# rosinality/vision-transformers-pytorch

Hardware: AMD Instinct MI355X
Metric: images/sec training (fwd+bwd+step) (higher is better)
Workload: dtype bf16; 1 GPU; swin_s 224x224 train step, batch 128/GPU, drop_path 0.3, MixLoss(eps 0.1), clip 5.0, AdamW(lr 1e-3, wd 0.05), grad_accum 1; global_batch=128, parallelism=dp1

## Files before the change

include/vtx.h:

```cpp
#ifndef VTX_H_
#define VTX_H_

#include <stddef.h>
#include <stdint.h>

#ifdef __cplusplus
extern "C" {
#endif

#define VTX_F32 0
#define VTX_BF16 1

#define VTX_OK 0
#define VTX_ERR_SHAPE (-1)
#define VTX_ERR_DTYPE (-2)
#define VTX_ERR_ALIGN (-3)
#define VTX_ERR_LAUNCH (-4)
#define VTX_ERR_WORKSPACE (-5)
#define VTX_ERR_NULL (-6)
#define VTX_ERR_JPEG (-7)

const char* vtx_strerror(int code);
#define VTX_ABI_VERSION 30
int vtx_abi_version(void);
int vtx_cu_count(void);
int vtx_debug_lds_poison(unsigned pattern, int rounds, void* stream);
int vtx_debug_mfma_peak(int iters, int waves_per_cu, void* sink, double* flops, void* stream);
int vtx_debug_spin(int microseconds, void* stream);
int vtx_sattn_waves(int L);

int vtx_option_count(void);
const char* vtx_option_name(int id);
int vtx_get_option(int id);
int vtx_set_option(int id, int value);

int vtx_layernorm_fwd(const void* x, const float* gamma, const float* beta, void* y, float* mean, float* rstd,
                      int64_t rows, int C, float eps, int dtype, int merge, int H, int W, void* stream);
int vtx_layernorm_fwd_mapped(const void* x, const float* gamma, const float* beta, void* y, float* mean, float* rstd,
                             int64_t rows, int C, float eps, int dtype, const int* perm, int T, void* stream);
int vtx_layernorm_bwd_mapped(const void* dy, const void* x, const float* mean, const float* rstd, const float* gamma,
                             const void* dres, void* dx, void* workspace, size_t ws_bytes, int64_t rows, int64_t live, int C,
                             int dtype, const int* perm, int T, void* stream);
size_t vtx_layernorm_bwd_workspace(int64_t rows, int C);
int vtx_layernorm_bwd_blocks(int64_t rows, int C);
int vtx_colreduce_multi(int n, const float* const* part, float* const* out0, float* const* out1, const int* nb,
                        const int* C, const int* ld, void* stream);
int vtx_layernorm_bwd(const void* dy, const void* x, const float* mean, const float* rstd, const float* gamma,
                      const void* dres, void* dx, float* dgamma, float* dbeta, void* workspace, size_t ws_bytes,
                      int64_t rows, int C, int dtype, int merge, int H, int W, void* stream);

int vtx_gemm(int mode, int dtype, const void* A, const void* B, void* C, int M, int N, int K, int64_t lda,
             int64_t ldb, int64_t ldc, const float* bias, const void* resid, const float* rowscale,
             int rows_per_scale, void* aux_out, const void* aux_in, int act, void* stream);
typedef struct VtxRoute {
  int family;
  int tile_m, tile_n, tile_k, stages, waves;
  int wmf, nf, ktiles;
  int mapped, act, resid, aux;
  int wide_j, tiles;
  int reserved;
  char label[96];
} VtxRoute;
#define VTX_Q_RESID 1
#define VTX_Q_AUXOUT 2
#define VTX_Q_AUXIN 4
#define VTX_Q_MAPPED 8
#define VTX_Q_BIAS 16
#define VTX_Q_ROWSCALE 32
#define VTX_Q_INPLACE 64
typedef struct VtxGemmQuery {
  int mode, dtype, M, N, K, act;
  int flags;
  int Mk, map_T;
  int rows_per_scale;
} VtxGemmQuery;
int vtx_gemm_route(const VtxGemmQuery* q, VtxRoute* out);
int vtx_wgrad_route(int dtype, int nprob, const int* N, const int* Kin, int64_t mtok, int flags, int rows_per_scale,
                    float scale_const, VtxRoute* out);
int vtx_wattn_route(int dtype, int bwd, int masked, int problems_per_head, int inverse_map, VtxRoute* out);
int vtx_gemm_glds_ok(int N, int K);

int vtx_mlp_fused_ok(int dtype, int64_t M, int C, int ff);
int vtx_mlp_fwd(int dtype, const void* ln2, const void* w1, const float* b1, const void* w2, const float* b2, const void* resid,
                const float* rowscale, int rows_per_scale, void* y, void* z, void* h, int64_t M, int C, int ff, void* stream);
int vtx_mlp_bwd(int dtype, const void* ln2, const void* dy, const void* w1, const float* b1, const void* w2, const float* rowscale,
                int rows_per_scale, void* h, void* dz, void* dln2, int64_t M, int C, int ff, void* stream);
int vtx_mlp_bwd_ln(int dtype, const void* ln2, const void* dy, const void* w1, const float* b1, const void* w2, const float* rowscale,
                   int rows_per_scale, void* h, void* dz, const void* x1, const float* mean, const float* rstd, const float* gamma,
                   void* dx1, float* part, int part_rows, int64_t M, int C, int ff, void* stream);
int vtx_dgrad_ln(int dtype, const void* dy, const void* wt, const void* x, const float* mean, const float* rstd, const float* gamma,
                 const void* dres, void* dx, float* part, int part_rows, int64_t M, int C, int K, void* stream);
int vtx_mlp_fwd_ln(int dtype, const void* x1, const float* gamma, const float* beta, float eps, void* ln2, float* mean, float* rstd,
                   const void* w1, const float* b1, const void* w2, const float* b2, const float* rowscale, int rows_per_scale, void* y,
                   int64_t M, int C, int ff, void* stream);
int vtx_ln_gemm(int dtype, const void* x, const float* gamma, const float* beta, float eps, void* ln_out, float* mean, float* rstd,
                const void* w, const float* bias, void* y, int64_t M, int C, int N, void* stream);
size_t vtx_wgrad_workspace(int64_t mtok, int N, int Kin);
int vtx_wgrad(int dtype, const void* dy, const void* x, float* dW, float* dbias, int64_t mtok, int N, int Kin,
              int64_t ld_dy, int64_t ld_x, const float* rowscale, int rows_per_scale, float scale_const,
              void* workspace, size_t ws_bytes, void* stream);
int vtx_wgrad_group_max(void);
int vtx_wgrad_group_ok(int dtype, int nprob, const int* N, const int* Kin, int64_t mtok, int has_rowscale,
                       int rows_per_scale, float scale_const);
size_t vtx_wgrad_group_workspace(int nprob, const int* N, const int* Kin, int64_t mtok);
int vtx_wgrad_group(int dtype, int nprob, const void* const* dy, const void* const* x, float* const* dW,
                    float* const* dbias, const int* N, const int* Kin, const int64_t* ld_dy, const int64_t* ld_x,
                    const float* const* rowscale, int rows_per_scale, float scale_const, int64_t mtok,
                    void* workspace, size_t ws_bytes, int ncol, const float* const* col_part, float* const* col_out0,
                    float* const* col_out1, const int* col_nb, const int* col_C, const int* col_ld, int accumulate,
                    void* stream);
int vtx_wgrad_group_mapped(int dtype, int nprob, const void* const* dy, const void* const* x, float* const* dW,
                           float* const* dbias, const int* N, const int* Kin, const int64_t* ld_dy, const int64_t* ld_x,
                           const float* const* rowscale, const int* const* perm, const int* mtok_kept, const float* scale,
                           int rows_per_scale, float scale_const, int64_t mtok, void* workspace, size_t ws_bytes, int ncol,
                           const float* const* col_part, float* const* col_out0, float* const* col_out1, const int* col_nb,
                           const int* col_C, const int* col_ld, int accumulate, void* stream);
int vtx_wgrad_group_slices(int nprob, const int* N, const int* Kin, int64_t mtok);

int vtx_relpos_bias(const float* rel_pos, const int64_t* pos, float* bias, int L, int nH, void* stream);
int vtx_attention_fwd(const void* qkv, void* o, float* lse, const float* bias, const uint8_t* mask, int B, int L,
                      int nH, int D, int swin, int H, int W, int win, int shift, int dtype, void* stream);
size_t vtx_attention_bwd_workspace(int B, int L, int nH, int swin, int H, int W, int win);
int vtx_attention_fwd_mapped(const void* qkv, void* o, float* lse, const int* perm, int Bk, int L, int nH, int D, int dtype,
                             void* stream);
int vtx_attention_bwd_mapped(const void* qkv, const void* o, const void* dout, const float* lse, void* dqkv, const int* perm,
                             int Bk, int L, int nH, int D, int dtype, void* stream);
int vtx_attention_bwd(const void* qkv, const void* o, const void* dout, const float* lse, const float* bias,
                      const uint8_t* mask, const int* csr_order, const int* csr_offsets, void* dqkv,
                      float* drel_pos, int ntab, void* workspace, size_t ws_bytes, int B, int L, int nH, int D,
                      int swin, int H, int W, int win, int shift, int dtype, void* stream);

int vtx_attention_fwd_drop(const void* qkv, void* o, float* lse, const float* bias, const uint8_t* mask, int B, int L,
                           int nH, int D, int swin, int H, int W, int win, int shift, int dtype, float drop_p, uint64_t seed,
                           const uint8_t* keep, void* stream);
int vtx_attention_bwd_drop(const void* qkv, const void* o, const void* dout, const float* lse, const float* bias,
                           const uint8_t* mask, const int* csr_order, const int* csr_offsets, void* dqkv,
                           float* drel_pos, int ntab, void* workspace, size_t ws_bytes, int B, int L, int nH, int D,
                           int swin, int H, int W, int win, int shift, int dtype, float drop_p, uint64_t seed,
                           const uint8_t* keep, void* stream);
int vtx_attn_keep_mask(uint8_t* out, int64_t nprob, int Lq, int Lk, float drop_p, uint64_t seed, void* stream);

int vtx_wattn_fwd(const void* qkv, void* o, float* lse, const float* rel_pos, const int64_t* pos,
                  const uint8_t* region, int B, int L, int nH, int H, int W, int win, int shift, int dtype,
                  void* stream);
int vtx_wattn_fwd_mapped(const void* qkv, void* o, float* lse, const float* rel_pos, const int64_t* pos,
                         const uint8_t* region, const int* perm, int Bk, int L, int nH, int H, int W, int win, int shift,
                         int dtype, void* stream);
int vtx_wattn_bwd_mapped(const void* qkv, const void* o, const void* dout, const float* lse, const float* rel_pos,
                         const int64_t* pos, const uint8_t* region, void* dqkv, void* workspace, size_t ws_bytes,
                         const int* inv_cells, int inv_count, const int* perm, int Bk, int L, int nH, int H, int W, int win,
                         int shift, int dtype, void* stream);
size_t vtx_wattn_bwd_workspace(int B, int nH, int H, int W, int win);
int vtx_wattn_bwd_parts(int B, int nH, int H, int W, int win);
int vtx_wattn_bwd_part_ld(int nH);
int vtx_wattn_bwd(const void* qkv, const void* o, const void* dout, const float* lse, const float* rel_pos,
                  const int64_t* pos, const uint8_t* region, void* dqkv, float* drel_pos, void* workspace,
                  size_t ws_bytes, const int* inv_cells, int inv_count, int B, int L, int nH, int H, int W, int win,
                  int shift, int dtype, void* stream);

#define VTX_ATTN_WINDOW 1
#define VTX_ATTN_GLOBAL 2
typedef struct VtxLayerFwd {
  int dtype, attn_kind;
  int64_t M;
  int C, ff, nH, L, B, rows_per_scale;
  int H, W, win, shift;
  float eps;
  const void* x;
  const float *ln1_w, *ln1_b, *ln2_w, *ln2_b;
  const void *wq, *wo, *w1, *w2;
  const float *bq, *bo, *b1, *b2;
  const float* rel_pos; const int64_t* pos; const uint8_t* region;
  const float *s1, *s2;
  void *ln1, *qkv, *o, *x1, *ln2, *z, *h, *y;
  float *mean1, *rstd1, *mean2, *rstd2, *lse;
  const int *perm1, *perm2;
  int Bk1, Bk2;
} VtxLayerFwd;
int vtx_layer_fwd(const VtxLayerFwd* a, void* stream);
typedef struct VtxLayerBwd {
  int dtype, attn_kind;
  int64_t M;
  int C, ff, nH, L, B, rows_per_scale;
  int H, W, win, shift;
  float scale_const;
  int accumulate, inv_count;
  const void *dy, *x, *ln1, *qkv, *o, *x1, *ln2, *z, *h;
  const float *mean1, *rstd1, *mean2, *rstd2, *lse;
  const float *ln1_w, *ln2_w;
  const void *wq, *wo, *w1, *w2, *wqt, *wot, *w1t, *w2t;
  const float* rel_pos; const int64_t* pos; const uint8_t* region; const int* inv_cells;
  const float *s1, *s2;
  void *dz, *dln2, *dx1, *dout, *dqkv, *dln1, *dx;
  void *ln1_ws, *ln2_ws, *attn_ws, *wgrad_ws;
  size_t ln_ws_bytes, attn_ws_bytes, wgrad_ws_bytes;
  float *dWq, *dbq, *dWo, *dbo, *dW1, *db1, *dW2, *db2, *dg1, *dbe1, *dg2, *dbe2, *drel;
  const int *perm1, *perm2;
  int Bk1, Bk2;
  const float* b1;
} VtxLayerBwd;
int vtx_layer_bwd(const VtxLayerBwd* a, void* stream, void* side_stream);
int vtx_layer_desc_bytes(int which);
typedef struct VtxSrLayerFwd {
  int dtype, twins;
  int64_t M;
  int C, ff, nH, L, B, rows_per_scale, H, W, r, skip, Lk, splitk;
  float eps;
  const void* x;
  const float *ln1_w, *ln1_b, *ln2_w, *ln2_b, *srn_w, *srn_b;
  const void *wq, *wkv, *wsr, *wsr_t, *wo, *w1, *w2;
  const float *bsr, *bo, *b1, *b2;
  const float *s1, *s2;
  void *ln1, *q, *patches, *patches_t, *red32, *red, *kvin, *kv, *o, *x1, *ln2, *z, *h, *y;
  float *mean1, *rstd1, *mean2, *rstd2, *means, *rstds, *lse;
  void* splitk_ws;
  size_t splitk_ws_bytes;
} VtxSrLayerFwd;
int vtx_srlayer_fwd(const VtxSrLayerFwd* a, void* stream);
typedef struct VtxSrLayerBwd {
  int dtype, twins;
  int64_t M;
  int C, ff, nH, L, B, rows_per_scale, H, W, r, skip, Lk, reserved;
  float scale_const;
  const void *dy, *x, *ln1, *q, *patches, *red, *kvin, *kv, *o, *x1, *ln2, *z, *h;
  const float *mean1, *rstd1, *mean2, *rstd2, *means, *rstds, *lse;
  const float *ln1_w, *ln2_w, *srn_w;
  const void *wq, *wkv, *wsr, *wo, *w1, *w2, *wqt, *wkvt, *wsrt, *wot, *w1t, *w2t;
  const float *s1, *s2;
  void *dz, *dln2, *dx1, *dout, *dq, *dkv, *dkvin, *dred, *dpatches, *dln1, *dx;
  void *ln1_ws, *ln2_ws, *lns_ws, *attn_ws, *wgrad_ws, *wgrad2_ws;
  size_t ln_ws_bytes, lns_ws_bytes, attn_ws_bytes, wgrad_ws_bytes, wgrad2_ws_bytes;
  float *dWq, *dWkv, *dWsr, *dbsr, *dWo, *dbo, *dW1, *db1, *dW2, *db2, *dg1, *dbe1, *dg2, *dbe2, *dgs, *dbs;
  const float* b1;
} VtxSrLayerBwd;
int vtx_srlayer_bwd(const VtxSrLayerBwd* a, void* stream, void* side_stream);
enum { VTX_T_LN_FWD = 1, VTX_T_GEMM = 2, VTX_T_WATTN_FWD = 3, VTX_T_ATTN_FWD = 4, VTX_T_LN_BWD = 5, VTX_T_WATTN_BWD = 6,
       VTX_T_ATTN_BWD = 7, VTX_T_WGRAD = 8,
       VTX_T_SRATTN_FWD = 9, VTX_T_SRATTN_BWD = 10, VTX_T_WGRAD_SR_A = 11, VTX_T_WGRAD_SR_B = 12, VTX_T_WGRAD_SPLITK = 13,
       VTX_T_GATHER = 14,
       VTX_T_MLP_FWD = 15, VTX_T_MLP_BWD = 16,
       VTX_T_DGRAD_LN = 17,
       VTX_T_LN_GEMM = 18 };
typedef struct VtxTimerRec { int tag, n, k, flags; int64_t rows; float ms; } VtxTimerRec;
int vtx_timer_start(void);
int vtx_timer_stop(VtxTimerRec* out, int cap);

int vtx_srattn_fwd(const void* q, const void* kv, void* o, float* lse, int B, int Lq, int Lk, int nH, int D, int dtype,
                   void* stream);
int vtx_srattn_scores(const void* q, const void* kv, void* score, int B, int Lq, int Lk, int nH, int D, int dtype,
                      void* stream);
size_t vtx_srattn_bwd_workspace(int B, int Lq, int Lk, int nH, int D);
int vtx_srattn_bwd(const void* q, const void* kv, const void* o, const void* dout, const float* lse, void* dq, void* dkv,
                   void* workspace, size_t ws_bytes, int B, int Lq, int Lk, int nH, int D, int dtype, void* stream);

int vtx_srattn_fwd_drop(const void* q, const void* kv, void* o, float* lse, int B, int Lq, int Lk, int nH, int D, int dtype,
                        float drop_p, uint64_t seed, const uint8_t* keep, void* stream);
int vtx_srattn_bwd_drop(const void* q, const void* kv, const void* o, const void* dout, const float* lse, void* dq, void* dkv,
                        void* workspace, size_t ws_bytes, int B, int Lq, int Lk, int nH, int D, int dtype, float drop_p,
                        uint64_t seed, const uint8_t* keep, void* stream);

int vtx_window_gather(const void* map, void* dst, int B, int H, int W, int64_t ld, int c0, int nc, int win, int halo, int dtype,
                      void* stream);
int vtx_window_scatter(const void* src, void* map, int B, int H, int W, int64_t ld, int c0, int nc, int win, int halo, int dtype,
                       void* stream);
int vtx_table_bias(const float* table, const int64_t* pos, float* bias, int64_t cells, int nH, void* stream);
int vtx_table_bias_bwd(const float* full, const int* csr_order, const int* csr_offsets, float* dtable, int64_t cells, int nH, int ntab,
                       void* stream);
int vtx_xattn_fwd(const void* q, const void* kv, void* o, float* lse, const float* bias, int B, int Lq, int Lk, int nH, int D, int dtype,
                  void* stream);
size_t vtx_xattn_bwd_workspace(int B, int Lq, int nH);
int vtx_xattn_bwd(const void* q, const void* kv, const void* o, const void* dout, const float* lse, const float* bias, void* dq,
                  void* dkv, float* dbias, void* workspace, size_t ws_bytes, int B, int Lq, int Lk, int nH, int D, int dtype,
                  void* stream);

int vtx_xattn_fwd_drop(const void* q, const void* kv, void* o, float* lse, const float* bias, int B, int Lq, int Lk, int nH, int D,
                       int dtype, float drop_p, uint64_t seed, const uint8_t* keep, void* stream);
int vtx_xattn_bwd_drop(const void* q, const void* kv, const void* o, const void* dout, const float* lse, const float* bias, void* dq,
                       void* dkv, float* dbias, void* workspace, size_t ws_bytes, int B, int Lq, int Lk, int nH, int D, int dtype,
                       float drop_p, uint64_t seed, const uint8_t* keep, void* stream);

int vtx_attn_hd_fwd(const void* q, const void* k, const void* v, int64_t ldq, int64_t ldkv, void* o, float* lse, int B, int Lq, int Lk,
                    int nH, int D, int dtype, float drop_p, uint64_t seed, const uint8_t* keep, int64_t keep_cells, void* stream);
size_t vtx_attn_hd_bwd_workspace(int B, int Lq, int nH);
int vtx_attn_hd_bwd(const void* q, const void* k, const void* v, int64_t ldq, int64_t ldkv, const void* o, const void* dout,
                    const float* lse, void* dq, void* dk, void* dv, int64_t lddq, int64_t lddkv, void* workspace, size_t ws_bytes, int B,
                    int Lq, int Lk, int nH, int D, int dtype, float drop_p, uint64_t seed, const uint8_t* keep, int64_t keep_cells,
                    void* stream);

int vtx_attn_hdw_fwd(const void* q, const void* k, const void* v, int64_t ldq, int64_t ldkv, void* o, float* lse, const float* bias,
                     const uint8_t* mask, int B, int Lq, int Lk, int nH, int D, int H, int W, int win, int shift, int dtype, float drop_p,
                     uint64_t seed, const uint8_t* keep, int64_t keep_cells, void* stream);
size_t vtx_attn_hdw_bwd_workspace(int B, int Lq, int Lk, int nH, int H, int W, int win, int has_bias);
int vtx_attn_hdw_bwd(const void* q, const void* k, const void* v, int64_t ldq, int64_t ldkv, const void* o, const void* dout,
                     const float* lse, const float* bias, const uint8_t* mask, void* dq, void* dk, void* dv, int64_t lddq, int64_t lddkv,
                     float* dbias, void* workspace, size_t ws_bytes, int B, int Lq, int Lk, int nH, int D, int H, int W, int win, int shift,
                     int dtype, float drop_p, uint64_t seed, const uint8_t* keep, int64_t keep_cells, void* stream);

int vtx_dwconv3_fwd(const void* x, const float* w, void* y, int B, int H, int W, int C, int adjoint, int dtype, void* stream);
size_t vtx_dwconv3_wgrad_workspace(int B, int H, int W, int C);
int vtx_dwconv3_wgrad(const void* x, const void* dy, float* dw, void* workspace, size_t ws_bytes, int B, int H, int W, int C,
                      int dtype, void* stream);

int vtx_twins_subsample_fwd(const void* x, void* out, void* out_t, int B, int H, int W, int C, int r, int dtype, void* stream);
int vtx_bias_cast(const float* x, const float* bias, void* out, int64_t rows, int C, int dtype, void* stream);
int vtx_twins_subsample_bwd(const void* dout, void* dx, int B, int H, int W, int C, int r, int accumulate, int dtype,
                            void* stream);

int vtx_patchify_fwd(const void* x, void* out, int B, int H, int W, int C, int p, int skip, int dtype, void* stream);
int vtx_patchify_bwd(const void* dout, void* dx, int B, int H, int W, int C, int p, int skip, int accumulate, int dtype,
                     void* stream);

int vtx_add_pos_fwd(const void* x, const float* cls, const float* pos, void* out, int B, int T, int C, int dtype,
                    void* stream);
int vtx_add_pos_bwd(const void* dout, void* dx, float* dcls, float* dpos, int B, int T, int C, int dtype, void* stream);

int vtx_l2norm_fwd(const void* x, void* y, float* nrm, int64_t rows, int C, float eps, int dtype, void* stream);
int vtx_l2norm_bwd(const void* dy, const void* y, const float* nrm, void* dx, int64_t rows, int C, float eps, int dtype,
                   void* stream);

size_t vtx_mix_plan_bytes(void);
int vtx_mix_max_rects(void);
int vtx_mix_normalize_erase(const void* x, int in_u8, const void* plan, const float* mean, const float* stdv,
                            const float* fills, void* out, int out_nhwc_bf16, int N, int C, int H, int W, void* stream);

size_t vtx_randaug_plan_bytes(void);
int vtx_randaug_max_ops(void);
int vtx_randaug_apply(const void* x, const void* plan, void* scratch, void* out, int N, int C, int H, int W, void* stream);

size_t vtx_resample_plan_bytes(void);
int vtx_resample_max_taps(void);
size_t vtx_resample_workspace_bytes(int M, int S_h, int S_w);
int vtx_resample_coeffs(int L, int S, int first, int n, void* table, void* stream);
int vtx_resized_crop(const void* buf, size_t buf_bytes, const void* table, void* ws, size_t ws_bytes, void* out, int M, int S_h,
                     int S_w, void* stream);

size_t vtx_resample_long_workspace_bytes(int L, int S_h, int S_w, int max_taps);
int vtx_resized_crop_long(const void* buf, size_t buf_bytes, const void* table, const void* idx, int L, int max_taps, void* ws,
                          size_t ws_bytes, void* out, int M, int S_h, int S_w, void* stream);

int vtx_jpeg_info(const void* data, size_t len, void* info);
size_t vtx_jpeg_plan_bytes(void);
size_t vtx_jpeg_coef_bytes(const void* info, const int* window);
size_t vtx_jpeg_plane_bytes(const void* info, const int* window);
size_t vtx_jpeg_workspace_bytes(int n, size_t plane_bytes);
int vtx_jpeg_entropy_decode(const void* data, size_t len, const int* window, void* coef, size_t coef_bytes, const long long* offs,
                            void* plan, int* reason);
int vtx_jpeg_decode(const void* coef, size_t coef_bytes, const void* plans, int n, void* ws, size_t ws_bytes, void* out,
                    size_t out_bytes, void* stream);

int vtx_jpeg_info_ex(const void* data, size_t len, void* info, int flags);
size_t vtx_jpeg_scratch_bytes(const void* info);
int vtx_jpeg_entropy_decode_ms(const void* data, size_t len, const int* window, void* coef, size_t coef_bytes, const long long* offs,
// ... 113 lines not shown
```

vision-transformers-pytorch_amd/csrc/attention_win.hip:

```cpp
#include <stdlib.h>

#include <type_traits>

#include "options.h"
#include "vtx_common.h"

#define WA_D 32
#define WA_LP 64
#define WA_STR 72
#define WA_NBIN 172
#define WA_BSTR 68
#define WA_WAVES 4
#ifndef WA_ABLATE
#define WA_ABLATE 0
#endif

struct WinGeom {
  int L, nH, hd, nW, H, W, win, shift, nWx;
  float scale;
  const int* perm;
};

struct WaTok {
  int ay[4], ax[4];
  bool val[4];
};
__device__ __forceinline__ void wa_tok_init(WaTok& k, const WinGeom& g, int c) {
#pragma unroll
  for (int t4 = 0; t4 < 4; ++t4) {
    const int tok = 16 * t4 + c;
    k.val[t4] = tok < g.L;
    const int t = k.val[t4] ? tok : 0;
    k.ay[t4] = t / g.win;
    k.ax[t4] = t - k.ay[t4] * g.win;
  }
}
__device__ __forceinline__ int wa_row(const WinGeom& g, const WaTok& k, int t4, int b, int wi, int wj) {
  int y = wi * g.win + k.ay[t4] + g.shift;
  y -= y >= g.H ? g.H : 0;
  int x = wj * g.win + k.ax[t4] + g.shift;
  x -= x >= g.W ? g.W : 0;
  return (b * g.H + y) * g.W + x;
}
template <typename T> __device__ __forceinline__ Vec8<T> wa_frag_acc(const f32x4& lo, const f32x4& hi) {
  Vec8<T> f;
#pragma unroll
  for (int j = 0; j < 4; ++j) { f.set(j, lo[j]); f.set(4 + j, hi[j]); }
  return f;
}
template <typename T> __device__ __forceinline__ Vec8<T> wa_frag_t(const T* p, int g) {
  Vec8<T> f;
  if constexpr (sizeof(T) == 2) {
    bf16x4 a = *reinterpret_cast<const bf16x4*>(p + 4 * g);
    bf16x4 b = *reinterpret_cast<const bf16x4*>(p + 16 + 4 * g);
#pragma unroll
    for (int j = 0; j < 4; ++j) { f.v[j] = a[j]; f.v[4 + j] = b[j]; }
  } else {
    f32x4 a = *reinterpret_cast<const f32x4*>(p + 4 * g);
    f32x4 b = *reinterpret_cast<const f32x4*>(p + 16 + 4 * g);
#pragma unroll
    for (int j = 0; j < 4; ++j) { f.v[j] = a[j]; f.v[4 + j] = b[j]; }
  }
  return f;
}
template <typename T> __device__ __forceinline__ void wa_store_t(T* xt, const Vec8<T> (&f)[4], int c, int g) {
#pragma unroll
  for (int t4 = 0; t4 < 4; ++t4)
#pragma unroll
    for (int e = 0; e < 8; ++e) xt[(16 * (e >> 2) + 4 * g + (e & 3)) * WA_STR + 16 * t4 + c] = f[t4].v[e];
}
template <typename T> __device__ __forceinline__ Vec8<T> wa_out8(const f32x4& a0, const f32x4& a1, float scale) {
  Vec8<T> f;
#pragma unroll
  for (int j = 0; j < 4; ++j) { f.set(j, a0[j] * scale); f.set(4 + j, a1[j] * scale); }
  return f;
}


__device__ __forceinline__ void wa_wave_sync() {
  __builtin_amdgcn_fence(__ATOMIC_RELEASE, "wavefront");
  __builtin_amdgcn_wave_barrier();
  __builtin_amdgcn_fence(__ATOMIC_ACQUIRE, "wavefront");
}

__device__ __forceinline__ bool wa_uniform(uint8_t reg, bool live) {
  const int first = __builtin_amdgcn_readfirstlane((int)reg);
  return __ballot(live && (int)reg != first) == 0ull;
}
__device__ __forceinline__ float group_max16(float v) {
  v = fmaxf(v, dpp_f<0xB1>(v));
  v = fmaxf(v, dpp_f<0x4E>(v));
  v = fmaxf(v, dpp_f<0x141>(v));
  v = fmaxf(v, dpp_f<0x140>(v));
  return v;
}

__device__ __forceinline__ void wa_build_bias(float* bias_s, float* relh, const float* __restrict__ rel_pos,
                                              const int64_t* __restrict__ pos, int L, int nH, int h, int ntab,
                                              int qrows = 64) {
  constexpr int PER = 64 * 64 / (64 * WA_WAVES);
  if (WA_ABLATE & 16) return;
  int pidx[PER];
#pragma unroll
  for (int i = 0; i < PER; ++i) {
    const int idx = threadIdx.x + i * 64 * WA_WAVES;
    const int k = idx & 63, q = idx >> 6;
    pidx[i] = (k < L && q < L) ? (int)pos[q * L + k] : -1;
  }
  if ((int)threadIdx.x < ntab) relh[threadIdx.x] = rel_pos[threadIdx.x * nH + h];
  __syncthreads();
#pragma unroll
  for (int i = 0; i < PER; ++i) {
    const int idx = threadIdx.x + i * 64 * WA_WAVES;
    const int k = idx & 63, q = idx >> 6;
    if (q < qrows) bias_s[q * WA_BSTR + k] = k >= L ? -INFINITY : (pidx[i] >= 0 ? relh[pidx[i]] : 0.f);
  }
}

template <typename T> struct WaSmem {
  static constexpr int kImg = WA_D * WA_STR * (int)sizeof(T);
  static constexpr int kBias = 64 * WA_BSTR * 4;
  static constexpr int kFwdWave = kImg + 64 + 64 * (int)sizeof(T);
  static constexpr int kBwdWave = 3 * kImg + 2 * WA_LP * 4 + WA_NBIN * 4 + 64;
  static constexpr int kFwd = kBias + WA_WAVES * kFwdWave;
  static constexpr int kBwd = kBias + WA_WAVES * kBwdWave;
};

__device__ __forceinline__ void wa_block_map(int nblk, int nH, int xcd_major, int& blk, int& h) {
  const int b = blockIdx.x;
  if (xcd_major) {
    const int xcd = b & 7, slot = b >> 3;
    h = slot % nH;
    blk = (slot / nH) * 8 + xcd;
  } else {
    blk = b % nblk;
    h = b / nblk;
  }
}

template <typename T, bool MASKED>
__global__ __launch_bounds__(64 * WA_WAVES) void wattn_fwd_kernel(const T* __restrict__ qkv, T* __restrict__ o,
                                                                  float* __restrict__ lse,
                                                                  const float* __restrict__ rel_pos,
                                                                  const int64_t* __restrict__ pos,
                                                                  const uint8_t* __restrict__ region, int nbn,
                                                                  int nblk, int xcd_major, int fast, WinGeom g) {
  extern __shared__ __attribute__((aligned(16))) unsigned char wa_smem[];
  float* bias_s = reinterpret_cast<float*>(wa_smem);
  const int wave = __builtin_amdgcn_readfirstlane(threadIdx.x >> 6);
  unsigned char* wbase = wa_smem + WaSmem<T>::kBias + wave * WaSmem<T>::kFwdWave;
  T* vt = reinterpret_cast<T*>(wbase);
  uint8_t* reg_s = wbase + WaSmem<T>::kImg;
  T* prow = reinterpret_cast<T*>(wbase + WaSmem<T>::kImg + 64);
  int blk, h;
  wa_block_map(nblk, g.nH, xcd_major, blk, h);
  const int lane = threadIdx.x & 63, c_ = lane & 15, g_ = lane >> 4;
  const int64_t ld = 3 * (int64_t)g.hd;
  wa_build_bias(bias_s, reinterpret_cast<float*>(wa_smem + WaSmem<T>::kBias), rel_pos, pos, g.L, g.nH, h,
                (2 * g.win - 1) * (2 * g.win - 1));
  __syncthreads();
  WaTok tk;
  wa_tok_init(tk, g, c_);
  const bool w7 = g.L == 49;
  const bool row48 = w7 && (fast & 1);
  if (row48) tk.ay[3] = tk.ax[3] = 6;

  for (int bn = blk * WA_WAVES + wave; bn < nbn; bn += nblk * WA_WAVES) {
    const int n = bn % g.nW, b = g.perm ? g.perm[bn / g.nW] : bn / g.nW;
    const int wi = n / g.nWx, wj = n - wi * g.nWx;
    const int prob = bn * g.nH + h;
    int row[4];
    const bool (&val)[4] = tk.val;
    Vec8<T> qf[4], kf[4], vf[4];
#pragma unroll
    for (int t4 = 0; t4 < 4; ++t4) {
      row[t4] = wa_row(g, tk, t4, b, wi, wj);
      const T* p = qkv + (int64_t)row[t4] * ld + h * WA_D + g_ * 8;
      qf[t4] = load8<T>(p);
      kf[t4] = load8<T>(p + g.hd);
      vf[t4] = load8<T>(p + 2 * g.hd);
    }
    uint8_t myreg = 0;
    if (MASKED) myreg = region[(int64_t)n * 64 + lane];
    wa_wave_sync();
    wa_store_t<T>(vt, vf, c_, g_);
    if (MASKED) reg_s[lane] = myreg;
    wa_wave_sync();

    if (WA_ABLATE & 32) {
#pragma unroll
      for (int qt = 0; qt < 4; ++qt)
        if (val[qt]) store8<T>(o + (int64_t)row[qt] * g.hd + h * WA_D + g_ * 8, qf[qt]);
      continue;
    }
    auto pv_store = [&](int qt, const Vec8<T>& p0, const Vec8<T>& p1) {
      f32x4 oacc[2] = {f32x4{0.f, 0.f, 0.f, 0.f}, f32x4{0.f, 0.f, 0.f, 0.f}};
#pragma unroll
      for (int ks = 0; ks < 2; ++ks)
#pragma unroll
        for (int dt = 0; dt < 2; ++dt) mma16(wa_frag_t<T>(vt + (dt * 16 + c_) * WA_STR + ks * 32, g_), ks ? p1 : p0, oacc[dt]);
      if (val[qt]) store8<T>(o + (int64_t)row[qt] * g.hd + h * WA_D + g_ * 8, wa_out8<T>(oacc[0], oacc[1], 1.f));
    };
    auto tiles = [&](auto mk) {
      constexpr bool MK = decltype(mk)::value;
#pragma unroll
      for (int qt = 0; qt < 4; ++qt) {
        if (qt * 16 >= g.L) break;
        if (qt == 3 && row48) {
          float sv[4], m = -INFINITY;
          const uint8_t r48 = MK ? reg_s[48] : 0;
#pragma unroll
          for (int kt = 0; kt < 4; ++kt) {
            f32x4 s = f32x4{0.f, 0.f, 0.f, 0.f};
            mma16(qf[3], kf[kt], s);
            sv[kt] = s[0] * g.scale + bias_s[48 * WA_BSTR + kt * 16 + c_];
            if (MK && reg_s[kt * 16 + c_] != r48) sv[kt] = -INFINITY;
            m = fmaxf(m, sv[kt]);
          }
          m = group_max16(m);
          float l = 0.f;
#pragma unroll
          for (int kt = 0; kt < 4; ++kt) {
            sv[kt] = __expf(sv[kt] - m);
            l += sv[kt];
          }
          l = group_sum<16>(l);
          const float inv = 1.f / l;
          if (lane == 0) lse[(int64_t)prob * g.L + 48] = m + __logf(l);
          Vec8<T> one;
#pragma unroll
          for (int kt = 0; kt < 4; ++kt) {
            one.set(0, sv[kt] * inv);
            prow[kt * 16 + c_] = one.v[0];
          }
          wa_wave_sync();
          pv_store(3, wa_frag_t<T>(prow, g_), wa_frag_t<T>(prow + 32, g_));
          break;
        }
        const int q = qt * 16 + c_;
        f32x4 st[4];
        float m = -INFINITY;
        const unsigned rq = MK ? reg_s[q] * 0x01010101u : 0u;
#pragma unroll
        for (int kt = 0; kt < 4; ++kt) {
          st[kt] = f32x4{0.f, 0.f, 0.f, 0.f};
          mma16(kf[kt], qf[qt], st[kt]);
          const f32x4 bb = *reinterpret_cast<const f32x4*>(bias_s + q * WA_BSTR + kt * 16 + g_ * 4);
          unsigned rx = 0u;
          if (MK) rx = *reinterpret_cast<const unsigned*>(reg_s + kt * 16 + g_ * 4) ^ rq;
#pragma unroll
          for (int r = 0; r < 4; ++r) {
            if (kt == 3 && r > 0 && w7) continue;
            float sv = st[kt][r] * g.scale + bb[r];
            if (MK && (rx & (0xffu << (8 * r))) != 0u) sv = -INFINITY;
            st[kt][r] = sv;
            m = fmaxf(m, sv);
          }
        }
        m = fmaxf(m, shfl_xor_f(m, 16));
        m = fmaxf(m, shfl_xor_f(m, 32));
        float l = 0.f;
#pragma unroll
        for (int kt = 0; kt < 4; ++kt)
#pragma unroll
          for (int r = 0; r < 4; ++r) {
            if (kt == 3 && r > 0 && w7) { st[kt][r] = 0.f; continue; }
            st[kt][r] = __expf(st[kt][r] - m);
            l += st[kt][r];
          }
        l += shfl_xor_f(l, 16);
        l += shfl_xor_f(l, 32);
        const float inv = 1.f / l;
        if (val[qt] && g_ == 0) lse[(int64_t)prob * g.L + q] = m + __logf(l);
        pv_store(qt, wa_frag_acc<T>(st[0] * inv, st[1] * inv), wa_frag_acc<T>(st[2] * inv, st[3] * inv));
      }
    };
    if (MASKED && !((fast & 2) && wa_uniform(myreg, lane < g.L)))
      tiles(std::true_type{});
    else
      tiles(std::false_type{});
  }
}

template <typename T, bool MASKED>
__global__ __launch_bounds__(64 * WA_WAVES, 2) void wattn_bwd_kernel(
    const T* __restrict__ qkv, const T* __restrict__ oin, const T* __restrict__ dout, const float* __restrict__ lse,
    const float* __restrict__ rel_pos, const int64_t* __restrict__ pos, const uint8_t* __restrict__ region,
    T* __restrict__ dqkv, float* __restrict__ bins_part, const int* __restrict__ inv_cells, int inv_count, int nbn,
    int nblk, int xcd_major, WinGeom g) {
  extern __shared__ __attribute__((aligned(16))) unsigned char wa_smem[];
  float* bias_s = reinterpret_cast<float*>(wa_smem);
  const int wave = __builtin_amdgcn_readfirstlane(threadIdx.x >> 6);
  unsigned char* wbase = wa_smem + WaSmem<T>::kBias + wave * WaSmem<T>::kBwdWave;
  T* kt_s = reinterpret_cast<T*>(wbase);
  T* qt_s = reinterpret_cast<T*>(wbase + WaSmem<T>::kImg);
  T* dot_s = reinterpret_cast<T*>(wbase + 2 * WaSmem<T>::kImg);
  float* dq_s = reinterpret_cast<float*>(wbase + 3 * WaSmem<T>::kImg);
  float* lse_s = dq_s + WA_LP;
  float* bins = lse_s + WA_LP;
  uint8_t* reg_s = reinterpret_cast<uint8_t*>(bins + WA_NBIN);
  int blk, h;
  wa_block_map(nblk, g.nH, xcd_major, blk, h);
  const int lane = threadIdx.x & 63, c_ = lane & 15, g_ = lane >> 4;
  const int64_t ld = 3 * (int64_t)g.hd;
  wa_build_bias(bias_s, reinterpret_cast<float*>(wa_smem + WaSmem<T>::kBias), rel_pos, pos, g.L, g.nH, h,
                (2 * g.win - 1) * (2 * g.win - 1));
  __syncthreads();
  for (int i = lane; i < WA_NBIN; i += 64) bins[i] = 0.f;
  f32x4 dsacc[4][4];
#pragma unroll
  for (int i = 0; i < 4; ++i)
#pragma unroll
    for (int j = 0; j < 4; ++j) dsacc[i][j] = f32x4{0.f, 0.f, 0.f, 0.f};
  WaTok tk;
  wa_tok_init(tk, g, c_);

  for (int bn = blk * WA_WAVES + wave; bn < nbn; bn += nblk * WA_WAVES) {
    const int n = bn % g.nW, b = g.perm ? g.perm[bn / g.nW] : bn / g.nW;
    const int wi = n / g.nWx, wj = n - wi * g.nWx;
    const int prob = bn * g.nH + h;

    int row[4];
    const bool (&val)[4] = tk.val;
    Vec8<T> qf[4], kf[4], vf[4], dof[4];
    float dsum[4], lq[4];
#pragma unroll
    for (int t4 = 0; t4 < 4; ++t4) {
      row[t4] = wa_row(g, tk, t4, b, wi, wj);
      const T* p = qkv + (int64_t)row[t4] * ld + h * WA_D + g_ * 8;
      const int64_t ro = (int64_t)row[t4] * g.hd + h * WA_D + g_ * 8;
      qf[t4] = load8<T>(p);
      kf[t4] = load8<T>(p + g.hd);
      vf[t4] = load8<T>(p + 2 * g.hd);
      dof[t4] = load8<T>(dout + ro);
      Vec8<T> of = load8<T>(oin + ro);
      const float lv = lse[(int64_t)prob * g.L + (val[t4] ? 16 * t4 + c_ : 0)];
      lq[t4] = val[t4] ? lv : INFINITY;
      float s = 0.f;
#pragma unroll
      for (int e = 0; e < 8; ++e) s += of.get(e) * dof[t4].get(e);
      s += shfl_xor_f(s, 16);
      s += shfl_xor_f(s, 32);
      dsum[t4] = s;
    }
    uint8_t myreg = 0;
    if (MASKED) myreg = region[(int64_t)n * 64 + lane];
    wa_wave_sync();
    wa_store_t<T>(kt_s, kf, c_, g_);
    wa_store_t<T>(qt_s, qf, c_, g_);
    wa_store_t<T>(dot_s, dof, c_, g_);
    if (g_ == 0) {
#pragma unroll
      for (int t4 = 0; t4 < 4; ++t4) { dq_s[16 * t4 + c_] = dsum[t4]; lse_s[16 * t4 + c_] = lq[t4]; }
    }
    if (MASKED) reg_s[lane] = myreg;
    wa_wave_sync();

    constexpr bool MK = MASKED;
#pragma unroll
    for (int qt = 0; qt < 4; ++qt) {
      if (qt * 16 >= g.L || (WA_ABLATE & 4)) break;
      const int q = qt * 16 + c_;
      const unsigned rq = MK ? reg_s[q] * 0x01010101u : 0u;
      f32x4 dqacc[2] = {f32x4{0.f, 0.f, 0.f, 0.f}, f32x4{0.f, 0.f, 0.f, 0.f}};
#pragma unroll
      for (int ks = 0; ks < 2; ++ks) {
        f32x4 dsv[2];
#pragma unroll
        for (int half = 0; half < 2; ++half) {
          const int kt = 2 * ks + half;
          f32x4 pt = f32x4{0.f, 0.f, 0.f, 0.f}, dpt = f32x4{0.f, 0.f, 0.f, 0.f};
          mma16(kf[kt], qf[qt], pt);
          mma16(vf[kt], dof[qt], dpt);
          const f32x4 bb = *reinterpret_cast<const f32x4*>(bias_s + q * WA_BSTR + kt * 16 + g_ * 4);
          unsigned rx = 0u;
          if (MK) rx = *reinterpret_cast<const unsigned*>(reg_s + kt * 16 + g_ * 4) ^ rq;
#pragma unroll
          for (int r = 0; r < 4; ++r) {
            float p = __expf(pt[r] * g.scale + bb[r] - lq[qt]);
            if (MK && (rx & (0xffu << (8 * r))) != 0u) p = 0.f;
            dsv[half][r] = p * (dpt[r] - dsum[qt]);
          }
        }
        Vec8<T> dsf = wa_frag_acc<T>(dsv[0], dsv[1]);
#pragma unroll
        for (int dt = 0; dt < 2; ++dt) mma16(wa_frag_t<T>(kt_s + (dt * 16 + c_) * WA_STR + ks * 32, g_), dsf, dqacc[dt]);
      }
      if (val[qt]) store8<T>(dqkv + (int64_t)row[qt] * ld + h * WA_D + g_ * 8, wa_out8<T>(dqacc[0], dqacc[1], g.scale));
      __builtin_amdgcn_sched_barrier(0);
    }

#pragma unroll
    for (int kt = 0; kt < 4; ++kt) {
      if (kt * 16 >= g.L || (WA_ABLATE & 8)) break;
      const int key = kt * 16 + c_;
      const unsigned rk = MK ? reg_s[key] * 0x01010101u : 0u;
      f32x4 dkacc[2] = {f32x4{0.f, 0.f, 0.f, 0.f}, f32x4{0.f, 0.f, 0.f, 0.f}};
      f32x4 dvacc[2] = {f32x4{0.f, 0.f, 0.f, 0.f}, f32x4{0.f, 0.f, 0.f, 0.f}};
#pragma unroll
      for (int qs = 0; qs < 2; ++qs) {
        f32x4 pp[2], dss[2];
#pragma unroll
        for (int half = 0; half < 2; ++half) {
          const int qt = 2 * qs + half;
          f32x4 s = f32x4{0.f, 0.f, 0.f, 0.f}, dp = f32x4{0.f, 0.f, 0.f, 0.f};
          mma16(qf[qt], kf[kt], s);
          mma16(dof[qt], vf[kt], dp);
          const int q0 = qt * 16 + g_ * 4;
          const f32x4 ls = *reinterpret_cast<const f32x4*>(lse_s + q0);
          const f32x4 dd = *reinterpret_cast<const f32x4*>(dq_s + q0);
          unsigned rx = 0u;
          if (MK) rx = *reinterpret_cast<const unsigned*>(reg_s + q0) ^ rk;
#pragma unroll
          for (int r = 0; r < 4; ++r) {
            const float bb = bias_s[(q0 + r) * WA_BSTR + key];
            float p = __expf(s[r] * g.scale + bb - ls[r]);
            if (MK && (rx & (0xffu << (8 * r))) != 0u) p = 0.f;
            pp[half][r] = p;
            dss[half][r] = p * (dp[r] - dd[r]);
          }
          dsacc[kt][qt] += dss[half];
        }
        Vec8<T> pf = wa_frag_acc<T>(pp[0], pp[1]);
        Vec8<T> dsf = wa_frag_acc<T>(dss[0], dss[1]);
#pragma unroll
        for (int dt = 0; dt < 2; ++dt) {
          mma16(wa_frag_t<T>(dot_s + (dt * 16 + c_) * WA_STR + qs * 32, g_), pf, dvacc[dt]);
          mma16(wa_frag_t<T>(qt_s + (dt * 16 + c_) * WA_STR + qs * 32, g_), dsf, dkacc[dt]);
        }
      }
      if (val[kt]) {
        T* p = dqkv + (int64_t)row[kt] * ld + h * WA_D + g_ * 8;
        store8<T>(p + g.hd, wa_out8<T>(dkacc[0], dkacc[1], g.scale));
        store8<T>(p + 2 * g.hd, wa_out8<T>(dvacc[0], dvacc[1], 1.f));
      }
      __builtin_amdgcn_sched_barrier(0);
    }
  }
  const int ntab = (2 * g.win - 1) * (2 * g.win - 1);
  if (inv_cells != nullptr && (g.L + 1) * 64 * 4 <= 3 * WaSmem<T>::kImg && !(WA_ABLATE & 1)) {
    float* ds_s = reinterpret_cast<float*>(wbase);
    wa_wave_sync();
#pragma unroll
    for (int kt = 0; kt < 4; ++kt) {
      const int key = kt * 16 + c_;
#pragma unroll
      for (int qt = 0; qt < 4; ++qt) {
#pragma unroll
        for (int r = 0; r < 4; ++r) {
          const int q = qt * 16 + g_ * 4 + r;
          if (key < g.L && q < g.L) ds_s[q * 64 + key] = dsacc[kt][qt][r];
        }
      }
    }
    if (lane == 0) ds_s[g.L * 64] = 0.f;
    wa_wave_sync();
    for (int b = lane; b < ntab; b += 64) {
      float sum = 0.f;
      const int* __restrict__ ic = inv_cells + b;
#pragma unroll 7
      for (int t = 0; t < inv_count; ++t) sum += ds_s[ic[t * ntab]];
      bins[b] = sum;
    }
  } else {
#pragma unroll
    for (int kt = 0; kt < 4; ++kt) {
      const int key = kt * 16 + c_;
#pragma unroll
      for (int qt = 0; qt < 4; ++qt) {
#pragma unroll
        for (int r = 0; r < 4; ++r) {
          const int q = qt * 16 + g_ * 4 + r;
          if (key < g.L && q < g.L && !(WA_ABLATE & 1)) atomicAdd(&bins[(int)pos[q * g.L + key]], dsacc[kt][qt][r]);
        }
      }
    }
  }
  wa_wave_sync();
  float* out = bins_part + ((int64_t)blk * WA_WAVES + wave) * WA_NBIN * g.nH + h;
  if (!(WA_ABLATE & 2))
    for (int i = lane; i < WA_NBIN; i += 64) out[(int64_t)i * g.nH] = bins[i];
}

#define WA4_PSTR 40
#ifndef WA4_OCC
#define WA4_OCC 3
#endif
#define WA4_BROWS 50
#define WA4_MSTR 72
struct Wa4Smem {
  static constexpr int kBias = WA4_BROWS * WA_BSTR * 4;
  static constexpr int kPlain = WA_LP * WA4_PSTR * 2;
  static constexpr int kMat = WA_LP * WA4_MSTR * 2;
  static constexpr int kSmall = 64;
  static constexpr int kTotal = kBias + 4 * kPlain + 2 * kMat + kSmall;
};
static_assert((WA_LP + 1) * 64 * 4 <= 4 * Wa4Smem::kPlain, "the dS spill must fit the images");
static_assert(3 * Wa4Smem::kTotal <= 160 * 1024, "three workgroups per CU");

typedef __attribute__((ext_vector_type(4))) short wa_s16x4;
typedef __attribute__((ext_vector_type(8))) short wa_s16x8;
typedef __attribute__((address_space(3))) wa_s16x4 wa_lds_s16x4;
__device__ __forceinline__ Vec8<bf16> wa4_frag_trp(const bf16* img, int t0, int dt, int lane) {
  const int p = lane & 15, g = lane >> 4;
  const int n = ((p & 3) << 3) + 4 * dt;
  wa_s16x4 v[2];
#pragma unroll
  for (int half = 0; half < 2; ++half) {
    const int r = t0 + half * 16 + g * 4 + (p >> 2);
    v[half] = __builtin_amdgcn_ds_read_tr16_b64_v4i16((wa_lds_s16x4*)(img + r * WA4_PSTR + n));
  }
  wa_s16x8 wv = __builtin_shufflevector(v[0], v[1], 0, 1, 2, 3, 4, 5, 6, 7);
  Vec8<bf16> f;
  f.v = __builtin_bit_cast(bf16x8, wv);
  return f;
}

__device__ __forceinline__ void wa_wg_sync() {
  asm volatile("s_waitcnt lgkmcnt(0)" ::: "memory");
  __builtin_amdgcn_s_barrier();
  asm volatile("" ::: "memory");
}

__device__ __forceinline__ Vec8<bf16> wa4_frag_tr(const bf16* mat, int t0, int key0, int lane) {
  const int p = lane & 15, g = lane >> 4;
  const int n = key0 + ((p & 3) << 2);
  wa_s16x4 v[2];
#pragma unroll
  for (int half = 0; half < 2; ++half) {
    const int r = t0 + half * 16 + g * 4 + (p >> 2);
    v[half] = __builtin_amdgcn_ds_read_tr16_b64_v4i16((wa_lds_s16x4*)(mat + r * WA4_MSTR + n));
  }
  wa_s16x8 wv = __builtin_shufflevector(v[0], v[1], 0, 1, 2, 3, 4, 5, 6, 7);
  Vec8<bf16> f;
  f.v = __builtin_bit_cast(bf16x8, wv);
  return f;
}

template <bool MASKED>
__global__ __launch_bounds__(64 * WA_WAVES, WA4_OCC) void wattn_bwd4_kernel(
    const bf16* __restrict__ qkv, const bf16* __restrict__ oin, const bf16* __restrict__ dout, const float* __restrict__ lse,
    const float* __restrict__ rel_pos, const int64_t* __restrict__ pos, const uint8_t* __restrict__ region,
    bf16* __restrict__ dqkv, float* __restrict__ bins_part, const int* __restrict__ inv_cells, int inv_count, int nbn,
    int nblk, int rows_total, int xcd_major, WinGeom g) {
  using T = bf16;
  extern __shared__ __attribute__((aligned(16))) unsigned char wa_smem[];
  float* bias_s = reinterpret_cast<float*>(wa_smem);
  unsigned char* base = wa_smem + Wa4Smem::kBias;
  T* pk = reinterpret_cast<T*>(base);
  T* pv = reinterpret_cast<T*>(base + Wa4Smem::kPlain);
  T* pq = reinterpret_cast<T*>(base + 2 * Wa4Smem::kPlain);
  T* pdo = reinterpret_cast<T*>(base + 3 * Wa4Smem::kPlain);
  T* pm_s = reinterpret_cast<T*>(base + 4 * Wa4Smem::kPlain);
  T* dm_s = reinterpret_cast<T*>(base + 4 * Wa4Smem::kPlain + Wa4Smem::kMat);
  uint8_t* reg_s = base + 4 * Wa4Smem::kPlain + 2 * Wa4Smem::kMat;
  const int w = __builtin_amdgcn_readfirstlane(threadIdx.x >> 6);
  const int lane = threadIdx.x & 63, c_ = lane & 15, g_ = lane >> 4;
  int blk, h;
  wa_block_map(nblk, g.nH, xcd_major, blk, h);
  const int64_t ld = 3 * (int64_t)g.hd;
  const int ntab = (2 * g.win - 1) * (2 * g.win - 1);
  wa_build_bias(bias_s, reinterpret_cast<float*>(base), rel_pos, pos, g.L, g.nH, h, ntab, WA4_BROWS);
  __syncthreads();

  const int tok = 16 * w + c_;
  const bool val = tok < g.L;
  const int tcl = val ? tok : 0;
  const int ay = tcl / g.win, ax = tcl - ay * g.win;
  const bool tile_live = 16 * w < g.L;
  const bool w7 = g.L == 49;

  f32x4 dsacc[4];
#pragma unroll
  for (int j = 0; j < 4; ++j) dsacc[j] = f32x4{0.f, 0.f, 0.f, 0.f};

  Vec8<T> nq, nk, nv, ndo, no;
  float nl = 0.f;
  int nrow = 0;
  auto request = [&](int bn) {
    const int n = bn % g.nW, b = g.perm ? g.perm[bn / g.nW] : bn / g.nW;
    const int wi = n / g.nWx, wj = n - wi * g.nWx;
    int y = wi * g.win + ay + g.shift;
    y -= y >= g.H ? g.H : 0;
    int x = wj * g.win + ax + g.shift;
    x -= x >= g.W ? g.W : 0;
    nrow = (b * g.H + y) * g.W + x;
    const T* p = qkv + (int64_t)nrow * ld + h * WA_D + g_ * 8;
    const int64_t ro = (int64_t)nrow * g.hd + h * WA_D + g_ * 8;
    nq = load8<T>(p);
    nk = load8<T>(p + g.hd);
    nv = load8<T>(p + 2 * g.hd);
    ndo = load8<T>(dout + ro);
    no = load8<T>(oin + ro);
    nl = lse[((int64_t)bn * g.nH + h) * g.L + tcl];
  };
  if (blk < nbn) request(blk);

  for (int bn = blk; bn < nbn; bn += nblk) {
    const Vec8<T> qf = nq, kf = nk, vf = nv, dof = ndo;
    const int row = nrow;
    const float lq = val ? nl : INFINITY;
    float dsum = 0.f;
#pragma unroll
    for (int e = 0; e < 8; ++e) dsum += no.get(e) * dof.get(e);
    dsum += shfl_xor_f(dsum, 16);
    dsum += shfl_xor_f(dsum, 32);
    uint8_t myreg = 0;
    if (MASKED && w == 0) myreg = region[(int64_t)(bn % g.nW) * 64 + lane];
    if (bn != blk) wa_wg_sync();
    *reinterpret_cast<Vec8<T>*>(pk + tok * WA4_PSTR + g_ * 8) = kf;
    *reinterpret_cast<Vec8<T>*>(pv + tok * WA4_PSTR + g_ * 8) = vf;
    *reinterpret_cast<Vec8<T>*>(pq + tok * WA4_PSTR + g_ * 8) = qf;
    *reinterpret_cast<Vec8<T>*>(pdo + tok * WA4_PSTR + g_ * 8) = dof;
    if (MASKED && w == 0) reg_s[lane] = myreg;
    wa_wg_sync();
    if (bn + nblk < nbn) request(bn + nblk);

    constexpr bool MK = MASKED;
    if (tile_live) {
      const int q = tok;
      const unsigned rq = MK ? reg_s[q] * 0x01010101u : 0u;
      f32x4 dqacc[2] = {f32x4{0.f, 0.f, 0.f, 0.f}, f32x4{0.f, 0.f, 0.f, 0.f}};
#pragma unroll
      for (int ks = 0; ks < 2; ++ks) {
        f32x4 dsv[2], pv2[2];
#pragma unroll
        for (int half = 0; half < 2; ++half) {
          const int kt = 2 * ks + half;
          const Vec8<T> kk = *reinterpret_cast<const Vec8<T>*>(pk + (16 * kt + c_) * WA4_PSTR + g_ * 8);
          const Vec8<T> vv = *reinterpret_cast<const Vec8<T>*>(pv + (16 * kt + c_) * WA4_PSTR + g_ * 8);
          f32x4 pt = f32x4{0.f, 0.f, 0.f, 0.f}, dpt = f32x4{0.f, 0.f, 0.f, 0.f};
          mma16(kk, qf, pt);
          mma16(vv, dof, dpt);
          const f32x4 bb = *reinterpret_cast<const f32x4*>(bias_s + tcl * WA_BSTR + kt * 16 + g_ * 4);
          unsigned rx = 0u;
          if (MK) rx = *reinterpret_cast<const unsigned*>(reg_s + kt * 16 + g_ * 4) ^ rq;
#pragma unroll
          for (int r = 0; r < 4; ++r) {
            if (kt == 3 && r > 0 && w7) { pv2[half][r] = 0.f; dsv[half][r] = 0.f; continue; }
            float p = __expf(pt[r] * g.scale + bb[r] - lq);
            if (MK && (rx & (0xffu << (8 * r))) != 0u) p = 0.f;
            pv2[half][r] = p;
            dsv[half][r] = p * (dpt[r] - dsum);
          }
          dsacc[kt] += dsv[half];
        }
        const Vec8<T> pf = wa_frag_acc<T>(pv2[0], pv2[1]);
        const Vec8<T> dsf = wa_frag_acc<T>(dsv[0], dsv[1]);
        bf16x4 plo, phi, dlo, dhi;
#pragma unroll
        for (int j = 0; j < 4; ++j) { plo[j] = pf.v[j]; phi[j] = pf.v[4 + j]; dlo[j] = dsf.v[j]; dhi[j] = dsf.v[4 + j]; }
        *reinterpret_cast<bf16x4*>(pm_s + q * WA4_MSTR + 32 * ks + 4 * g_) = plo;
        *reinterpret_cast<bf16x4*>(pm_s + q * WA4_MSTR + 32 * ks + 16 + 4 * g_) = phi;
        *reinterpret_cast<bf16x4*>(dm_s + q * WA4_MSTR + 32 * ks + 4 * g_) = dlo;
        *reinterpret_cast<bf16x4*>(dm_s + q * WA4_MSTR + 32 * ks + 16 + 4 * g_) = dhi;
#pragma unroll
        for (int dt = 0; dt < 2; ++dt) mma16(wa4_frag_trp(pk, ks * 32, dt, lane), dsf, dqacc[dt]);
      }
      if (val) store8<T>(dqkv + (int64_t)row * ld + h * WA_D + g_ * 8, wa_out8<T>(dqacc[0], dqacc[1], g.scale));
    } else {
      const bf16x4 z = {(bf16)0.f, (bf16)0.f, (bf16)0.f, (bf16)0.f};
#pragma unroll
      for (int j = 0; j < 4; ++j) {
        *reinterpret_cast<bf16x4*>(pm_s + tok * WA4_MSTR + 16 * j + 4 * g_) = z;
        *reinterpret_cast<bf16x4*>(dm_s + tok * WA4_MSTR + 16 * j + 4 * g_) = z;
      }
    }
    wa_wg_sync();
    if (tile_live) {
      f32x4 dkacc[2] = {f32x4{0.f, 0.f, 0.f, 0.f}, f32x4{0.f, 0.f, 0.f, 0.f}};
      f32x4 dvacc[2] = {f32x4{0.f, 0.f, 0.f, 0.f}, f32x4{0.f, 0.f, 0.f, 0.f}};
#pragma unroll
      for (int qs = 0; qs < 2; ++qs) {
        const Vec8<T> pf = wa4_frag_tr(pm_s, qs * 32, 16 * w, lane);
        const Vec8<T> dsf = wa4_frag_tr(dm_s, qs * 32, 16 * w, lane);
#pragma unroll
        for (int dt = 0; dt < 2; ++dt) {
          mma16(wa4_frag_trp(pdo, qs * 32, dt, lane), pf, dvacc[dt]);
          mma16(wa4_frag_trp(pq, qs * 32, dt, lane), dsf, dkacc[dt]);
        }
      }
      if (val) {
        T* p = dqkv + (int64_t)row * ld + h * WA_D + g_ * 8;
        store8<T>(p + g.hd, wa_out8<T>(dkacc[0], dkacc[1], g.scale));
        store8<T>(p + 2 * g.hd, wa_out8<T>(dvacc[0], dvacc[1], 1.f));
      }
    }
  }

  wa_wg_sync();
  float* ds_s = reinterpret_cast<float*>(base);
  {
    const int q = tok;
#pragma unroll
    for (int kt = 0; kt < 4; ++kt)
#pragma unroll
      for (int r = 0; r < 4; ++r) {
        const int key = kt * 16 + g_ * 4 + r;
        if (key < g.L && q < g.L) ds_s[q * 64 + key] = dsacc[kt][r];
      }
    if (threadIdx.x == 0) ds_s[g.L * 64] = 0.f;
  }
  wa_wg_sync();
  for (int b = threadIdx.x; b < WA_NBIN; b += 64 * WA_WAVES) {
    float sum = 0.f;
    if (b < ntab) {
      const int* __restrict__ ic = inv_cells + b;
#pragma unroll 7
      for (int t = 0; t < inv_count; ++t) sum += ds_s[ic[t * ntab]];
    }
    bins_part[((int64_t)blk * WA_NBIN + b) * g.nH + h] = sum;
    for (int r = nblk + blk; r < rows_total; r += nblk) bins_part[((int64_t)r * WA_NBIN + b) * g.nH + h] = 0.f;
  }
}

#ifndef WF4_OCC
#define WF4_OCC 5
#endif
#ifndef WF4_PF
#define WF4_PF 1
#endif
#ifndef WF4_COAL
#define WF4_COAL 0
#endif
#ifndef WF4_DB
#define WF4_DB 0
#endif
struct Wf4Smem {
  static constexpr int kBias = WA4_BROWS * WA_BSTR * 4;
  static constexpr int kPlain = WA_LP * WA4_PSTR * 2;
  static constexpr int kRow = 64 * 2;
  static constexpr int kSmall = 64;
  static constexpr int kSet = (2 + WF4_COAL) * kPlain + kSmall;
  static constexpr int kTotal = kBias + kRow + (1 + WF4_DB) * kSet;
};
static_assert(WF4_OCC * Wf4Smem::kTotal <= 160 * 1024, "WF4_OCC workgroups per CU");
static_assert(WA_NBIN * 4 <= Wf4Smem::kPlain, "the rel_pos column scratch of the table build must fit the K image");

template <bool MASKED>
__global__ __launch_bounds__(64 * WA_WAVES, WF4_OCC) void wattn_fwd4_kernel(
    const bf16* __restrict__ qkv, bf16* __restrict__ o, float* __restrict__ lse, const float* __restrict__ rel_pos,
    const int64_t* __restrict__ pos, const uint8_t* __restrict__ region, int nbn, int nblk, int xcd_major, int fast, WinGeom g) {
  using T = bf16;
  extern __shared__ __attribute__((aligned(16))) unsigned char wa_smem[];
  float* bias_s = reinterpret_cast<float*>(wa_smem);
  unsigned char* base = wa_smem + Wf4Smem::kBias;
  T* prow = reinterpret_cast<T*>(base);
  base += Wf4Smem::kRow;
  const int w = __builtin_amdgcn_readfirstlane(threadIdx.x >> 6);
  const int lane = threadIdx.x & 63, c_ = lane & 15, g_ = lane >> 4;
  const int lt = WF4_COAL ? lane >> 2 : c_, lp = WF4_COAL ? lane & 3 : g_;
  int blk, h;
  wa_block_map(nblk, g.nH, xcd_major, blk, h);
  const int64_t ld = 3 * (int64_t)g.hd;
  wa_build_bias(bias_s, reinterpret_cast<float*>(base), rel_pos, pos, g.L, g.nH, h, (2 * g.win - 1) * (2 * g.win - 1), WA4_BROWS);
  __syncthreads();
  const bool w7 = g.L == 49;
  const bool row48 = w7 && (fast & 1);
  auto tok_pack = [&](int t4) {
    const int tok = 16 * t4 + lt;
    const bool live = tok < g.L;
    const int tc = (t4 == 3 && row48) ? 48 : (live ? tok : 0);
    const int ay = tc / g.win;
    return ay | ((tc - ay * g.win) << 8) | ((int)live << 16);
  };
  const int tp0 = tok_pack(0), tp1 = tok_pack(1), tp2 = tok_pack(2), tp3 = tok_pack(3);

  struct Rows { Vec8<T> q, k, v; int row; uint8_t reg; };
  auto request = [&](int bn, int t, Rows& s) __attribute__((always_inline)) {
    const int n = bn % g.nW, b = g.perm ? g.perm[bn / g.nW] : bn / g.nW;
    const int wi = n / g.nWx, wj = n - wi * g.nWx;
    const int tp = t == 0 ? tp0 : t == 1 ? tp1 : t == 2 ? tp2 : tp3;
    const int ay = tp & 0xff, ax = (tp >> 8) & 0xff;
    int y = wi * g.win + ay + g.shift;
    y -= y >= g.H ? g.H : 0;
    int x = wj * g.win + ax + g.shift;
    x -= x >= g.W ? g.W : 0;
    s.row = (b * g.H + y) * g.W + x;
    const T* p = qkv + (int64_t)s.row * ld + h * WA_D + lp * 8;
    s.q = load8<T>(p);
    s.k = load8<T>(p + g.hd);
    s.v = load8<T>(p + 2 * g.hd);
    if (MASKED && w == 0) s.reg = region[(int64_t)n * 64 + lane];
  };
  Rows rs[WF4_PF];
#pragma unroll
  for (int u = 0; u < WF4_PF; ++u) {
    rs[u].reg = 0;
    if (blk + u * nblk < nbn) request(blk + u * nblk, (w + u) & 3, rs[u]);
  }
  for (int bn = blk, it = 0; bn < nbn;) {
#pragma unroll
  for (int u = 0; u < WF4_PF; ++u, bn += nblk, ++it) {
    if (bn >= nbn) break;
    Rows& nx = rs[u];
    const int t = (w + it) & 3;
    const Vec8<T> qg = nx.q, kf = nx.k, vf = nx.v;
    const int row = nx.row;
    const uint8_t myreg = nx.reg;
    const int tok = 16 * t + c_, ltok = 16 * t + lt;
    const bool val = tok < g.L;
    const bool gval = ((t == 0 ? tp0 : t == 1 ? tp1 : t == 2 ? tp2 : tp3) >> 16) != 0;
    const int prob = bn * g.nH + h;
    unsigned char* set = base + (WF4_DB ? (it & 1) * Wf4Smem::kSet : 0);
    T* pk = reinterpret_cast<T*>(set);
    T* pv = reinterpret_cast<T*>(set + Wf4Smem::kPlain);
    T* pq = reinterpret_cast<T*>(set + 2 * Wf4Smem::kPlain);
    uint8_t* reg_s = set + (2 + WF4_COAL) * Wf4Smem::kPlain;
    if (!WF4_DB && bn != blk) wa_wg_sync();
    *reinterpret_cast<Vec8<T>*>(pk + ltok * WA4_PSTR + lp * 8) = kf;
    *reinterpret_cast<Vec8<T>*>(pv + ltok * WA4_PSTR + lp * 8) = vf;
    if (WF4_COAL) *reinterpret_cast<Vec8<T>*>(pq + ltok * WA4_PSTR + lp * 8) = qg;
    if (MASKED && w == 0) reg_s[lane] = myreg;
    wa_wg_sync();
    if (bn + WF4_PF * nblk < nbn) request(bn + WF4_PF * nblk, (w + it + WF4_PF) & 3, nx);
    if (WA_ABLATE & 32) {
      if (gval) store8<T>(o + (int64_t)row * g.hd + h * WA_D + lp * 8, qg);
      continue;
    }
    if (16 * t >= g.L) continue;
    Vec8<T> qf = qg;
    if (WF4_COAL) qf = *reinterpret_cast<const Vec8<T>*>(pq + tok * WA4_PSTR + g_ * 8);

    auto pv_store = [&](const Vec8<T>& p0, const Vec8<T>& p1) {
      f32x4 oacc[2] = {f32x4{0.f, 0.f, 0.f, 0.f}, f32x4{0.f, 0.f, 0.f, 0.f}};
#pragma unroll
      for (int ks = 0; ks < 2; ++ks)
#pragma unroll
        for (int dt = 0; dt < 2; ++dt) mma16(wa4_frag_trp(pv, ks * 32, dt, lane), ks ? p1 : p0, oacc[dt]);
      Vec8<T> ov = wa_out8<T>(oacc[0], oacc[1], 1.f);
      if (WF4_COAL) {
        wa_wave_sync();
        *reinterpret_cast<Vec8<T>*>(pq + tok * WA4_PSTR + g_ * 8) = ov;
        wa_wave_sync();
        ov = *reinterpret_cast<const Vec8<T>*>(pq + ltok * WA4_PSTR + lp * 8);
      }
      if (gval) store8<T>(o + (int64_t)row * g.hd + h * WA_D + lp * 8, ov);
    };
    auto tile = [&](auto mk) {
      constexpr bool MK = decltype(mk)::value;
      if (t == 3 && row48) {
        float sv[4], m = -INFINITY;
        const uint8_t r48 = MK ? reg_s[48] : 0;
#pragma unroll
        for (int kt = 0; kt < 4; ++kt) {
          const Vec8<T> kk = *reinterpret_cast<const Vec8<T>*>(pk + (16 * kt + c_) * WA4_PSTR + g_ * 8);
          f32x4 s = f32x4{0.f, 0.f, 0.f, 0.f};
          mma16(qf, kk, s);
          sv[kt] = s[0] * g.scale + bias_s[48 * WA_BSTR + kt * 16 + c_];
          if (MK && reg_s[kt * 16 + c_] != r48) sv[kt] = -INFINITY;
          m = fmaxf(m, sv[kt]);
        }
        m = group_max16(m);
        float l = 0.f;
#pragma unroll
        for (int kt = 0; kt < 4; ++kt) {
          sv[kt] = __expf(sv[kt] - m);
          l += sv[kt];
        }
        l = group_sum<16>(l);
        const float inv = 1.f / l;
        if (lane == 0) lse[(int64_t)prob * g.L + 48] = m + __logf(l);
        Vec8<T> one;
#pragma unroll
        for (int kt = 0; kt < 4; ++kt) {
          one.set(0, sv[kt] * inv);
          prow[kt * 16 + c_] = one.v[0];
        }
        wa_wave_sync();
        pv_store(wa_frag_t<T>(prow, g_), wa_frag_t<T>(prow + 32, g_));
        return;
      }
      const int q = val ? tok : 0;
      f32x4 st[4];
      float m = -INFINITY;
      const unsigned rq = MK ? reg_s[tok] * 0x01010101u : 0u;
#pragma unroll
      for (int kt = 0; kt < 4; ++kt) {
        const Vec8<T> kk = *reinterpret_cast<const Vec8<T>*>(pk + (16 * kt + c_) * WA4_PSTR + g_ * 8);
        st[kt] = f32x4{0.f, 0.f, 0.f, 0.f};
        mma16(kk, qf, st[kt]);
        const f32x4 bb = *reinterpret_cast<const f32x4*>(bias_s + q * WA_BSTR + kt * 16 + g_ * 4);
        unsigned rx = 0u;
        if (MK) rx = *reinterpret_cast<const unsigned*>(reg_s + kt * 16 + g_ * 4) ^ rq;
#pragma unroll
        for (int r = 0; r < 4; ++r) {
          if (kt == 3 && r > 0 && w7) continue;
          float sv = st[kt][r] * g.scale + bb[r];
          if (MK && (rx & (0xffu << (8 * r))) != 0u) sv = -INFINITY;
          st[kt][r] = sv;
          m = fmaxf(m, sv);
        }
      }
      m = fmaxf(m, shfl_xor_f(m, 16));
      m = fmaxf(m, shfl_xor_f(m, 32));
      float l = 0.f;
#pragma unroll
      for (int kt = 0; kt < 4; ++kt)
#pragma unroll
        for (int r = 0; r < 4; ++r) {
          if (kt == 3 && r > 0 && w7) { st[kt][r] = 0.f; continue; }
          st[kt][r] = __expf(st[kt][r] - m);
          l += st[kt][r];
        }
      l += shfl_xor_f(l, 16);
      l += shfl_xor_f(l, 32);
      const float inv = 1.f / l;
      if (val && g_ == 0) lse[(int64_t)prob * g.L + tok] = m + __logf(l);
      pv_store(wa_frag_acc<T>(st[0] * inv, st[1] * inv), wa_frag_acc<T>(st[2] * inv, st[3] * inv));
    };
    bool masked = MASKED;
    if (MASKED && (fast & 2)) masked = !wa_uniform(reg_s[lane], lane < g.L);
    if (masked)
      tile(std::true_type{});
    else
      tile(std::false_type{});
  }
  }
}

static int win_geom(WinGeom& g, int L, int nH, int H, int W, int win, int shift) {
  if (win <= 0 || H % win || W % win || L != win * win || L > WA_LP) return VTX_ERR_SHAPE;
  if ((2 * win - 1) * (2 * win - 1) > WA_NBIN) return VTX_ERR_SHAPE;
  g.L = L; g.nH = nH; g.hd = nH * WA_D; g.H = H; g.W = W; g.win = win;
  g.nWx = W / win; g.nW = (H / win) * (W / win); g.shift = shift ? win / 2 : 0;
  g.scale = 1.0f / sqrtf((float)WA_D);
  g.perm = nullptr;
  return VTX_OK;
}

static int wattn_blocks(int nbn, int nH, int cap) {
  int per_head = cap / nH;
  if (per_head < WA_WAVES) per_head = WA_WAVES;
  const int ppw = (nbn + per_head - 1) / per_head;
  const int waves = (nbn + ppw - 1) / ppw;
  int blocks = (waves + WA_WAVES - 1) / WA_WAVES;
  if (blocks >= 8 && vtx_opt(VTX_OPT_WATTN_XCD_MAJOR)) blocks = (blocks + 7) / 8 * 8;
  return blocks;
}
static int wattn_xcd_major(int nblk) { return (nblk % 8 == 0 && vtx_opt(VTX_OPT_WATTN_XCD_MAJOR)) ? 1 : 0; }
static int wattn_fwd_blocks(int nbn, int nH) {
  const int cap = vtx_opt(VTX_OPT_WATTN_FWD_WAVES);
  return wattn_blocks(nbn, nH, cap > 0 ? cap : 4096);
}
static int wattn_bwd_blocks(int nbn, int nH) {
  const int cap = vtx_opt(VTX_OPT_WATTN_BWD_WAVES);
  return wattn_blocks(nbn, nH, cap > 0 ? cap : 2048);
}
static int wattn_bwd4_blocks(int nbn, int nH) {
  int per_head = 256 * WA4_OCC / nH;
  if (per_head < 1) per_head = 1;
  const int ppw = (nbn + per_head - 1) / per_head;
  int blocks = (nbn + ppw - 1) / ppw;
  if (blocks >= 8 && vtx_opt(VTX_OPT_WATTN_XCD_MAJOR)) blocks = (blocks + 7) / 8 * 8;
  return blocks;
}
static int wattn_fwd4_blocks(int nbn, int nH) {
  int per_head = 256 * WF4_OCC / nH;
  if (per_head < 1) per_head = 1;
  const int ppw = (nbn + per_head - 1) / per_head;
  int blocks = (nbn + ppw - 1) / ppw;
  if (blocks >= 8 && vtx_opt(VTX_OPT_WATTN_XCD_MAJOR)) blocks = (blocks + 7) / 8 * 8;
  return blocks;
}
static int wattn_bwd_rows(int nbn, int nH) {
  const int a = wattn_bwd_blocks(nbn, nH) * WA_WAVES, b = wattn_bwd4_blocks(nbn, nH);
  return a > b ? a : b;
}

template <typename K> static int wa_smem_attr(K kern, int bytes) {
  if (bytes > 64 * 1024 &&
      hipFuncSetAttribute((const void*)kern, hipFuncAttributeMaxDynamicSharedMemorySize, bytes) != hipSuccess)
    return VTX_ERR_LAUNCH;
  return VTX_OK;
}

struct WattnRoute { int four, masked, dtype, bwd; };
static WattnRoute wattn_route(int dtype, bool bwd, bool masked, int nbn, bool inverse_map) {
  WattnRoute r;
  r.dtype = dtype; r.bwd = bwd; r.masked = masked; r.four = 0;
  if (dtype != VTX_BF16) return r;
  if (bwd) {
    r.four = inverse_map && vtx_opt(VTX_OPT_WATTN_BWD4) != 0;
  } else {
    const int f4 = vtx_opt(VTX_OPT_WATTN_FWD4);
    r.four = f4 >= 2 || (f4 == 1 && nbn >= 4096);
  }
  return r;
}
static void wattn_route_label(const WattnRoute& r, char* buf, size_t n) {
  const char* d = r.bwd ? "bwd" : "fwd";
  const char* m = r.masked ? "true" : "false";
  if (r.four) snprintf(buf, n, "wattn_%s4_kernel<%s>", d, m);
  else snprintf(buf, n, "wattn_%s_kernel<%s, %s>", d, r.dtype == VTX_BF16 ? "__bf16" : "float", m);
}

template <typename T, bool MASKED>
static int wattn_fwd_launch(const WattnRoute& r, const void* qkv, void* o, float* lse, const float* rel_pos, const int64_t* pos,
                            const uint8_t* region, int nbn, const WinGeom& g, hipStream_t st) {
  if constexpr (sizeof(T) == 2) {
    if (r.four) {
      const int nb4 = wattn_fwd4_blocks(nbn, g.nH);
      hipLaunchKernelGGL(wattn_fwd4_kernel<MASKED>, dim3(nb4 * g.nH), dim3(64 * WA_WAVES), Wf4Smem::kTotal, st,
                         (const bf16*)qkv, (bf16*)o, lse, rel_pos, pos, region, nbn, nb4, wattn_xcd_major(nb4),
                         vtx_opt(VTX_OPT_WATTN_FAST), g);
      return vtx_check_launch();
    }
  }
  auto kern = wattn_fwd_kernel<T, MASKED>;
  int rc = wa_smem_attr(kern, WaSmem<T>::kFwd);
  if (rc) return rc;
  const int nblk = wattn_fwd_blocks(nbn, g.nH);
  hipLaunchKernelGGL(kern, dim3(nblk * g.nH), dim3(64 * WA_WAVES), WaSmem<T>::kFwd, st,
                     (const T*)qkv, (T*)o, lse, rel_pos, pos, region, nbn, nblk, wattn_xcd_major(nblk), vtx_opt(VTX_OPT_WATTN_FAST), g);
  return vtx_check_launch();
}
static int wattn_fwd_routed(int dtype, const void* qkv, void* o, float* lse, const float* rel_pos, const int64_t* pos,
                            const uint8_t* region, int nbn, const WinGeom& g, hipStream_t st) {
  const WattnRoute r = wattn_route(dtype, false, region != nullptr, nbn, false);
  if (dtype == VTX_BF16)
    return r.masked ? wattn_fwd_launch<bf16, true>(r, qkv, o, lse, rel_pos, pos, region, nbn, g, st)
                    : wattn_fwd_launch<bf16, false>(r, qkv, o, lse, rel_pos, pos, region, nbn, g, st);
  if (dtype == VTX_F32)
    return r.masked ? wattn_fwd_launch<float, true>(r, qkv, o, lse, rel_pos, pos, region, nbn, g, st)
                    : wattn_fwd_launch<float, false>(r, qkv, o, lse, rel_pos, pos, region, nbn, g, st);
  return VTX_ERR_DTYPE;
}

template <typename T, bool MASKED>
static int wattn_bwd_launch(const WattnRoute& r, const void* qkv, const void* o, const void* dout, const float* lse, const float* rel_pos,
                            const int64_t* pos, const uint8_t* region, void* dqkv, float* part, const int* inv_cells,
                            int inv_count, int nbn, const WinGeom& g, hipStream_t st) {
  const int rows = wattn_bwd_rows(nbn, g.nH);
  if constexpr (sizeof(T) == 2) {
    if (r.four) {
      auto kern4 = wattn_bwd4_kernel<MASKED>;
      int rc4 = wa_smem_attr(kern4, Wa4Smem::kTotal);
      if (rc4) return rc4;
      const int nb4 = wattn_bwd4_blocks(nbn, g.nH);
      hipLaunchKernelGGL(kern4, dim3(nb4 * g.nH), dim3(64 * WA_WAVES), Wa4Smem::kTotal, st,
                         (const bf16*)qkv, (const bf16*)o, (const bf16*)dout, lse, rel_pos, pos, region, (bf16*)dqkv, part,
                         inv_cells, inv_count, nbn, nb4, rows, wattn_xcd_major(nb4), g);
      return vtx_check_launch();
    }
  }
  auto kern = wattn_bwd_kernel<T, MASKED>;
  int rc = wa_smem_attr(kern, WaSmem<T>::kBwd);
  if (rc) return rc;
  const int nblk = wattn_bwd_blocks(nbn, g.nH);
  if (rows > nblk * WA_WAVES &&
      hipMemsetAsync(part + (size_t)nblk * WA_WAVES * WA_NBIN * g.nH, 0,
                     (size_t)(rows - nblk * WA_WAVES) * WA_NBIN * g.nH * sizeof(float), st) != hipSuccess)
    return VTX_ERR_LAUNCH;
  hipLaunchKernelGGL(kern, dim3(nblk * g.nH), dim3(64 * WA_WAVES), WaSmem<T>::kBwd, st,
                     (const T*)qkv, (const T*)o, (const T*)dout, lse, rel_pos, pos, region, (T*)dqkv, part, inv_cells,
                     inv_count, nbn, nblk, wattn_xcd_major(nblk), g);
  return vtx_check_launch();
}

static int wattn_bwd_routed(int dtype, const void* qkv, const void* o, const void* dout, const float* lse, const float* rel_pos,
                            const int64_t* pos, const uint8_t* region, void* dqkv, float* part, const int* inv_cells,
                            int inv_count, int nbn, const WinGeom& g, hipStream_t st) {
  const WattnRoute r = wattn_route(dtype, true, region != nullptr, nbn, inv_cells != nullptr);
  if (dtype == VTX_BF16)
    return r.masked ? wattn_bwd_launch<bf16, true>(r, qkv, o, dout, lse, rel_pos, pos, region, dqkv, part, inv_cells, inv_count, nbn, g, st)
                    : wattn_bwd_launch<bf16, false>(r, qkv, o, dout, lse, rel_pos, pos, region, dqkv, part, inv_cells, inv_count, nbn, g, st);
  if (dtype == VTX_F32)
    return r.masked ? wattn_bwd_launch<float, true>(r, qkv, o, dout, lse, rel_pos, pos, region, dqkv, part, inv_cells, inv_count, nbn, g, st)
                    : wattn_bwd_launch<float, false>(r, qkv, o, dout, lse, rel_pos, pos, region, dqkv, part, inv_cells, inv_count, nbn, g, st);
  return VTX_ERR_DTYPE;
}

extern "C" {

int vtx_wattn_fwd(const void* qkv, void* o, float* lse, const float* rel_pos, const int64_t* pos,
                  const uint8_t* region, int B, int L, int nH, int H, int W, int win, int shift, int dtype,
                  void* stream) {
  if (!qkv || !o || !lse || !rel_pos || !pos) return VTX_ERR_NULL;
  WinGeom g;
  int rc = win_geom(g, L, nH, H, W, win, shift);
  if (rc) return rc;
  const int nbn = B * g.nW;
  if (nbn <= 0) return VTX_OK;
  hipStream_t st = (hipStream_t)stream;
  return wattn_fwd_routed(dtype, qkv, o, lse, rel_pos, pos, region, nbn, g, st);
}

int vtx_wattn_fwd_mapped(const void* qkv, void* o, float* lse, const float* rel_pos, const int64_t* pos,
                         const uint8_t* region, const int* perm, int Bk, int L, int nH, int H, int W, int win, int shift,
                         int dtype, void* stream) {
  if (!qkv || !o || !lse || !rel_pos || !pos || !perm) return VTX_ERR_NULL;
  WinGeom g;
  int rc = win_geom(g, L, nH, H, W, win, shift);
  if (rc) return rc;
  g.perm = perm;
  const int nbn = Bk * g.nW;
  if (nbn <= 0) return VTX_OK;
  hipStream_t st = (hipStream_t)stream;
  return wattn_fwd_routed(dtype, qkv, o, lse, rel_pos, pos, region, nbn, g, st);
}

int vtx_wattn_bwd_parts(int B, int nH, int H, int W, int win) {
  if (win <= 0 || H % win || W % win) return 0;
  return wattn_bwd_rows(B * (H / win) * (W / win), nH);
}
int vtx_wattn_bwd_part_ld(int nH) { return WA_NBIN * nH; }

size_t vtx_wattn_bwd_workspace(int B, int nH, int H, int W, int win) {
  const int nbn = B * (H / win) * (W / win);
  return (size_t)wattn_bwd_rows(nbn, nH) * nH * WA_NBIN * sizeof(float);
}

int vtx_wattn_bwd(const void* qkv, const void* o, const void* dout, const float* lse, const float* rel_pos,
                  const int64_t* pos, const uint8_t* region, void* dqkv, float* drel_pos, void* workspace,
                  size_t ws_bytes, const int* inv_cells, int inv_count, int B, int L, int nH, int H, int W, int win,
                  int shift, int dtype, void* stream) {
  if (!qkv || !o || !dout || !lse || !rel_pos || !pos || !dqkv || !workspace) return VTX_ERR_NULL;
  WinGeom g;
  int rc = win_geom(g, L, nH, H, W, win, shift);
  if (rc) return rc;
  const int nbn = B * g.nW;
  if (nbn <= 0) return VTX_OK;
  if (ws_bytes < vtx_wattn_bwd_workspace(B, nH, H, W, win)) return VTX_ERR_WORKSPACE;
  if (inv_cells != nullptr && (inv_count <= 0 || inv_count > L * L)) return VTX_ERR_SHAPE;
  hipStream_t st = (hipStream_t)stream;
  float* part = (float*)workspace;
  rc = wattn_bwd_routed(dtype, qkv, o, dout, lse, rel_pos, pos, region, dqkv, part, inv_cells, inv_count, nbn, g, st);
  if (rc || drel_pos == nullptr) return rc;
  const int ntab = (2 * win - 1) * (2 * win - 1);
  const int nwaves = wattn_bwd_rows(nbn, nH);
  hipLaunchKernelGGL(colreduce_kernel, colreduce_grid(ntab * nH), dim3(1024), 0, st, (const float*)part, drel_pos,
                     (float*)nullptr, nwaves, ntab * nH, WA_NBIN * nH);
  return vtx_check_launch();
}

int vtx_wattn_bwd_mapped(const void* qkv, const void* o, const void* dout, const float* lse, const float* rel_pos,
                         const int64_t* pos, const uint8_t* region, void* dqkv, void* workspace, size_t ws_bytes,
                         const int* inv_cells, int inv_count, const int* perm, int Bk, int L, int nH, int H, int W, int win,
                         int shift, int dtype, void* stream) {
  if (!qkv || !o || !dout || !lse || !rel_pos || !pos || !dqkv || !workspace || !perm) return VTX_ERR_NULL;
  WinGeom g;
  int rc = win_geom(g, L, nH, H, W, win, shift);
  if (rc) return rc;
  g.perm = perm;
  const int nbn = Bk * g.nW;
  if (nbn <= 0) return VTX_ERR_SHAPE;
  if (ws_bytes < vtx_wattn_bwd_workspace(Bk, nH, H, W, win)) return VTX_ERR_WORKSPACE;
  if (inv_cells != nullptr && (inv_count <= 0 || inv_count > L * L)) return VTX_ERR_SHAPE;
  hipStream_t st = (hipStream_t)stream;
  float* part = (float*)workspace;
  return wattn_bwd_routed(dtype, qkv, o, dout, lse, rel_pos, pos, region, dqkv, part, inv_cells, inv_count, nbn, g, st);
}

int vtx_wattn_route(int dtype, int bwd, int masked, int problems_per_head, int inverse_map, VtxRoute* out) {
  if (!out) return VTX_ERR_NULL;
  if (dtype != VTX_BF16 && dtype != VTX_F32) return VTX_ERR_DTYPE;
  const WattnRoute r = wattn_route(dtype, bwd != 0, masked != 0, problems_per_head, inverse_map != 0);
  *out = VtxRoute{};
  out->family = r.four ? 2 : 1;
  out->waves = r.four ? 4 : 1;
  wattn_route_label(r, out->label, sizeof(out->label));
  return VTX_OK;
}

}
```

vision-transformers-pytorch_amd/csrc/cast.hip:

```cpp
#include "vtx_common.h"

struct CastDesc {
  const float* src;
  int64_t off;
  int rows, cols;
  int tile0;
  int tiles_c;
};

__global__ __launch_bounds__(256) void cast_weights_kernel(const CastDesc* __restrict__ desc, int nmat,
                                                          bf16* __restrict__ dst, bf16* __restrict__ dst_t) {
  __shared__ float tile[64][65];
  const int t = blockIdx.x;
  int lo = 0, hi = nmat - 1;
  while (lo < hi) {
    const int mid = (lo + hi + 1) >> 1;
    if (desc[mid].tile0 <= t) lo = mid; else hi = mid - 1;
  }
  const CastDesc d = desc[lo];
  const int lt = t - d.tile0;
  const int r0 = (lt / d.tiles_c) * 64, c0 = (lt % d.tiles_c) * 64;
  const int tx = threadIdx.x & 63, ty = threadIdx.x >> 6;
  bf16* out = dst + d.off;
  bf16* out_t = dst_t + d.off;
#pragma unroll 4
  for (int i = 0; i < 16; ++i) {
    const int r = r0 + ty + 4 * i, c = c0 + tx;
    float v = 0.f;
    if (r < d.rows && c < d.cols) {
      v = d.src[(int64_t)r * d.cols + c];
      out[(int64_t)r * d.cols + c] = from_f32<bf16>(v);
    }
    tile[ty + 4 * i][tx] = v;
  }
  __syncthreads();
#pragma unroll 4
  for (int i = 0; i < 16; ++i) {
    const int c = c0 + ty + 4 * i, r = r0 + tx;
    if (r < d.rows && c < d.cols) out_t[(int64_t)c * d.rows + r] = from_f32<bf16>(tile[tx][ty + 4 * i]);
  }
}

extern "C" {

size_t vtx_cast_desc_bytes(void) { return sizeof(CastDesc); }

int vtx_cast_weights(const void* desc, int nmat, int ntiles, void* dst, void* dst_t, void* stream) {
  if (!desc || !dst || !dst_t) return VTX_ERR_NULL;
  if (nmat <= 0 || ntiles <= 0) return VTX_OK;
  hipLaunchKernelGGL(cast_weights_kernel, dim3(ntiles), dim3(256), 0, (hipStream_t)stream, (const CastDesc*)desc, nmat,
                     (bf16*)dst, (bf16*)dst_t);
  return vtx_check_launch();
}

}
```

vision-transformers-pytorch_amd/csrc/layer.hip:

```cpp
#include <hip/hip_runtime.h>

#include <vector>

#include "gemm_common.h"

namespace {

struct EventRing {
  hipEvent_t ev[64];
  int n = 0, next = 0;
  hipEvent_t get() {
    if (n < 64) {
      if (hipEventCreateWithFlags(&ev[n], hipEventDisableTiming) != hipSuccess) return nullptr;
      return ev[n++];
    }
    hipEvent_t e = ev[next];
    next = (next + 1) & 63;
    return e;
  }
};
thread_local EventRing g_events;

struct TimerEntry { int tag, n, k, flags; int64_t rows; hipEvent_t e0, e1; };
std::vector<TimerEntry>* g_timer = nullptr;
int g_timer_base = 0;
struct TimerScope {
  TimerEntry e; hipStream_t st; bool on;
  TimerScope(int tag, int64_t rows, int n, int k, int flags, void* stream) : st((hipStream_t)stream), on(g_timer != nullptr) {
    if (!on) return;
    e.tag = tag; e.rows = rows; e.n = n; e.k = k; e.flags = flags | g_timer_base;
    on = hipEventCreate(&e.e0) == hipSuccess && hipEventCreate(&e.e1) == hipSuccess && hipEventRecord(e.e0, st) == hipSuccess;
  }
  ~TimerScope() {
    if (on && hipEventRecord(e.e1, st) == hipSuccess) g_timer->push_back(e);
  }
};
#define TCALL(tag, rows, n, k, flags, st, expr) ([&]() -> int { TimerScope ts_(tag, rows, n, k, flags, st); return (expr); }())
enum { F_RESID = 1, F_AUXOUT = 2, F_AUXIN = 4, F_MAPPED = 8, F_MASKED = 16, F_BF16 = 32, F_TWINS = 64 };

int layer_dgrad(int dtype, const void* dy, const void* w, const void* wt, void* dx, int64_t M, int n_in, int k_out,
                const void* resid, const float* rowscale, int rps, const void* aux_in, int act, void* st) {
  if (dtype == VTX_BF16 && wt != nullptr && gemm_glds_ok(n_in, k_out))
    return vtx_gemm(0, dtype, dy, wt, dx, (int)M, n_in, k_out, k_out, k_out, n_in, nullptr, resid, rowscale, rps, nullptr,
                    aux_in, act, st);
  return vtx_gemm(1, dtype, dy, w, dx, (int)M, n_in, k_out, k_out, n_in, n_in, nullptr, resid, rowscale, rps, nullptr,
                  aux_in, act, st);
}

int layer_gemm_mapped(const void* A, const void* W, void* Cc, int M, int Mk, int N, int K, const float* bias, const void* resid,
                      const float* rowscale, int T, void* aux_out, const void* aux_in, int act, const int* perm, void* st) {
  GemmArgs a;
  a.A = A; a.B = W; a.C = Cc; a.M = M; a.N = N; a.K = K; a.lda = K; a.ldb = K; a.ldc = N;
  a.bias = bias; a.resid = resid; a.rowscale = rowscale; a.rows_per_scale = T; a.aux_out = aux_out; a.aux_in = aux_in;
  a.act = act; a.kscale = nullptr; a.k_per_scale = 1; a.kscale_const = 0.f; a.kchunk = ((K + 127) / 128) * 128;
  a.ksum_out = nullptr; a.perm = perm; a.map_T = T; a.Mk = Mk; a.map_magic = vtx_div_magic(T);
  if (!A || !W || !Cc || !perm) return VTX_ERR_NULL;
  if ((act == 2 || act == 4) && !aux_in) return VTX_ERR_NULL;
  int rc = gemm_mapped_validate(a);
  if (rc) return rc;
  GemmRoute r;
  rc = gemm_route(a, 0, VTX_BF16, r);
  return rc ? rc : gemm_route_launch(a, r, 1, (hipStream_t)st);
}

}

extern "C" {

int vtx_layer_desc_bytes(int which) {
  switch (which) {
    case 0: return (int)sizeof(VtxLayerFwd);
    case 1: return (int)sizeof(VtxLayerBwd);
    case 2: return (int)sizeof(VtxSrLayerFwd);
    case 3: return (int)sizeof(VtxSrLayerBwd);
    case 4: return (int)sizeof(VtxRoute);
    case 5: return (int)sizeof(VtxGemmQuery);
    default: return 0;
  }
}

int vtx_timer_start(void) {
  if (g_timer == nullptr) g_timer = new std::vector<TimerEntry>();
  g_timer->clear();
  return VTX_OK;
}
int vtx_timer_stop(VtxTimerRec* out, int cap) {
  if (g_timer == nullptr) return 0;
  int n = 0;
  for (TimerEntry& e : *g_timer) {
    float ms = 0.f;
    if (hipEventSynchronize(e.e1) == hipSuccess && hipEventElapsedTime(&ms, e.e0, e.e1) == hipSuccess && out && n < cap) {
      out[n].tag = e.tag; out[n].n = e.n; out[n].k = e.k; out[n].flags = e.flags; out[n].rows = e.rows; out[n].ms = ms;
      ++n;
    }
    hipEventDestroy(e.e0); hipEventDestroy(e.e1);
  }
  delete g_timer;
  g_timer = nullptr;
  return n;
}

int vtx_layer_fwd(const VtxLayerFwd* a, void* stream) {
  if (!a || !a->x || !a->y || !a->ln1 || !a->qkv || !a->o || !a->x1 || !a->ln2 || !a->h) return VTX_ERR_NULL;
  if (a->M <= 0 || a->M > 0x7fffffff || a->C <= 0 || a->ff <= 0 || a->nH <= 0) return VTX_ERR_SHAPE;
  const int dt = a->dtype, M = (int)a->M, C = a->C, ff = a->ff;
  g_timer_base = (dt == VTX_BF16 ? F_BF16 : 0) | ((C / a->nH) << 8);
  if (a->perm1 != nullptr || a->perm2 != nullptr) {
    const int T = a->rows_per_scale;
    if (!a->perm1 || !a->perm2 || dt != VTX_BF16 || T <= 0 || M != a->B * T ||
        a->Bk1 <= 0 || a->Bk1 > a->B || a->Bk2 <= 0 || a->Bk2 > a->B)
      return VTX_ERR_SHAPE;
    const int M1 = a->Bk1 * T, M2 = a->Bk2 * T;
    int rc = TCALL(VTX_T_LN_FWD, M1, C, 0, F_MAPPED, stream, vtx_layernorm_fwd_mapped(a->x, a->ln1_w, a->ln1_b, a->ln1, a->mean1, a->rstd1, M1, C, a->eps, dt, a->perm1, T, stream));
    if (rc) return rc;
    rc = TCALL(VTX_T_GEMM, M1, 3 * C, C, F_MAPPED, stream, layer_gemm_mapped(a->ln1, a->wq, a->qkv, M1, M1, 3 * C, C, a->bq, nullptr, nullptr, T, nullptr, nullptr, 0, a->perm1, stream));
    if (rc) return rc;
    if (a->attn_kind == VTX_ATTN_WINDOW)
      rc = TCALL(VTX_T_WATTN_FWD, M1, a->nH, a->L, F_MAPPED | (a->region ? F_MASKED : 0), stream,
                 vtx_wattn_fwd_mapped(a->qkv, a->o, a->lse, a->rel_pos, a->pos, a->region, a->perm1, a->Bk1, a->L, a->nH, a->H, a->W,
                                      a->win, a->shift, dt, stream));
    else
      rc = TCALL(VTX_T_ATTN_FWD, M1, a->nH, a->L, F_MAPPED, stream,
                 vtx_attention_fwd_mapped(a->qkv, a->o, a->lse, a->perm1, a->Bk1, a->L, a->nH, C / a->nH, dt, stream));
    if (rc) return rc;
    rc = TCALL(VTX_T_GEMM, M1, C, C, F_MAPPED | F_RESID, stream, layer_gemm_mapped(a->o, a->wo, a->x1, M, M1, C, C, a->bo, a->x, a->s1, T, nullptr, nullptr, 0, a->perm1, stream));
    if (rc) return rc;
    rc = TCALL(VTX_T_LN_FWD, M2, C, 0, F_MAPPED, stream, vtx_layernorm_fwd_mapped(a->x1, a->ln2_w, a->ln2_b, a->ln2, a->mean2, a->rstd2, M2, C, a->eps, dt, a->perm2, T, stream));
    if (rc) return rc;
    rc = TCALL(VTX_T_GEMM, M2, ff, C, F_MAPPED | (a->z ? F_AUXOUT : 0), stream, layer_gemm_mapped(a->ln2, a->w1, a->h, M2, M2, ff, C, a->b1, nullptr, nullptr, T, a->z, nullptr, 1, a->perm2, stream));
    if (rc) return rc;
    return TCALL(VTX_T_GEMM, M2, C, ff, F_MAPPED | F_RESID, stream, layer_gemm_mapped(a->h, a->w2, a->y, M, M2, C, ff, a->b2, a->x1, a->s2, T, nullptr, nullptr, 0, a->perm2, stream));
  }
  int rc;
  if (ln_gemm_ok(dt, M, C, 3 * C)) {
    rc = TCALL(VTX_T_LN_GEMM, M, 3 * C, C, 0, stream,
               ln_gemm_launch(a->x, a->ln1_w, a->ln1_b, a->eps, a->ln1, a->mean1, a->rstd1, a->wq, a->bq, a->qkv, M, C, 3 * C, (hipStream_t)stream));
    if (rc) return rc;
  } else {
    rc = TCALL(VTX_T_LN_FWD, M, C, 0, 0, stream, vtx_layernorm_fwd(a->x, a->ln1_w, a->ln1_b, a->ln1, a->mean1, a->rstd1, a->M, C, a->eps, dt, 0, 0, 0, stream));
    if (rc) return rc;
    rc = TCALL(VTX_T_GEMM, M, 3 * C, C, 0, stream, vtx_gemm(0, dt, a->ln1, a->wq, a->qkv, M, 3 * C, C, C, C, 3 * C, a->bq, nullptr, nullptr, 1, nullptr, nullptr, 0, stream));
    if (rc) return rc;
  }
  if (a->attn_kind == VTX_ATTN_WINDOW)
    rc = TCALL(VTX_T_WATTN_FWD, M, a->nH, a->L, a->region ? F_MASKED : 0, stream,
               vtx_wattn_fwd(a->qkv, a->o, a->lse, a->rel_pos, a->pos, a->region, a->B, a->L, a->nH, a->H, a->W, a->win, a->shift, dt, stream));
  else if (a->attn_kind == VTX_ATTN_GLOBAL)
    rc = TCALL(VTX_T_ATTN_FWD, M, a->nH, a->L, 0, stream,
               vtx_attention_fwd(a->qkv, a->o, a->lse, nullptr, nullptr, a->B, a->L, a->nH, C / a->nH, 0, 0, 0, 0, 0, dt, stream));
  else
    return VTX_ERR_SHAPE;
  if (rc) return rc;
  rc = TCALL(VTX_T_GEMM, M, C, C, F_RESID, stream, vtx_gemm(0, dt, a->o, a->wo, a->x1, M, C, C, C, C, C, a->bo, a->x, a->s1, a->rows_per_scale, nullptr, nullptr, 0, stream));
  if (rc) return rc;
  if (mlp_fused_lnf_ok(dt, M, C, ff))
    return TCALL(VTX_T_MLP_FWD, M, C, ff, F_RESID | F_AUXOUT, stream,
                 mlp_fused_fwd_ln(a->x1, a->ln2_w, a->ln2_b, a->eps, a->ln2, a->mean2, a->rstd2, a->w1, a->b1, a->w2, a->b2, a->s2, a->rows_per_scale,
                                  a->y, M, C, ff, (hipStream_t)stream));
  rc = TCALL(VTX_T_LN_FWD, M, C, 0, 0, stream, vtx_layernorm_fwd(a->x1, a->ln2_w, a->ln2_b, a->ln2, a->mean2, a->rstd2, a->M, C, a->eps, dt, 0, 0, 0, stream));
  if (rc) return rc;
  if (mlp_fused_ok(dt, M, C, ff))
    return TCALL(VTX_T_MLP_FWD, M, C, ff, F_RESID, stream,
                 mlp_fused_fwd(a->ln2, a->w1, a->b1, a->w2, a->b2, a->x1, a->s2, a->rows_per_scale, a->y, nullptr, nullptr, M, C, ff, (hipStream_t)stream));
  rc = TCALL(VTX_T_GEMM, M, ff, C, a->z ? F_AUXOUT : 0, stream, vtx_gemm(0, dt, a->ln2, a->w1, a->h, M, ff, C, C, C, ff, a->b1, nullptr, nullptr, 1, a->z, nullptr, 1, stream));
  if (rc) return rc;
  return TCALL(VTX_T_GEMM, M, C, ff, F_RESID, stream,
               vtx_gemm(0, dt, a->h, a->w2, a->y, M, C, ff, ff, ff, C, a->b2, a->x1, a->s2, a->rows_per_scale, nullptr, nullptr, 0, stream));
}

int vtx_layer_bwd(const VtxLayerBwd* a, void* stream, void* side_stream) {
  if (!a || !a->dy || !a->dx || !a->x || !a->z || !a->dz || !a->dln2 || !a->dx1 || !a->dout || !a->dqkv || !a->dln1)
    return VTX_ERR_NULL;
  if (a->M <= 0 || a->M > 0x7fffffff || a->C <= 0 || a->ff <= 0 || a->nH <= 0) return VTX_ERR_SHAPE;
  const int dt = a->dtype, C = a->C, ff = a->ff, rps = a->rows_per_scale;
  const int64_t M = a->M;
  const bool mapped = a->perm1 != nullptr || a->perm2 != nullptr;
  g_timer_base = (dt == VTX_BF16 ? F_BF16 : 0) | ((C / a->nH) << 8);
  if (mapped) {
    const int T = rps;
    if (!a->perm1 || !a->perm2 || dt != VTX_BF16 || T <= 0 || M != (int64_t)a->B * T ||
        a->Bk1 <= 0 || a->Bk1 > a->B || a->Bk2 <= 0 || a->Bk2 > a->B || !a->w2t || !a->w1t || !a->wot || !a->wqt ||
        !a->s1 || !a->s2)
      return VTX_ERR_SHAPE;
    const int M1 = a->Bk1 * T, M2 = a->Bk2 * T;
    int rc = TCALL(VTX_T_GEMM, M2, ff, C, F_MAPPED | F_AUXIN, stream, layer_gemm_mapped(a->dy, a->w2t, a->dz, M2, M2, ff, C, nullptr, nullptr, a->s2, T, nullptr, a->z, 2, a->perm2, stream));
    if (rc) return rc;
    rc = TCALL(VTX_T_GEMM, M2, C, ff, F_MAPPED, stream, layer_gemm_mapped(a->dz, a->w1t, a->dln2, M2, M2, C, ff, nullptr, nullptr, nullptr, T, nullptr, nullptr, 0, a->perm2, stream));
    if (rc) return rc;
    rc = TCALL(VTX_T_LN_BWD, M, C, 0, F_MAPPED, stream,
               vtx_layernorm_bwd_mapped(a->dln2, a->x1, a->mean2, a->rstd2, a->ln2_w, a->dy, a->dx1, a->ln2_ws, a->ln_ws_bytes, M, M2, C, dt,
                                        a->perm2, T, stream));
    if (rc) return rc;
    rc = TCALL(VTX_T_GEMM, M1, C, C, F_MAPPED, stream, layer_gemm_mapped(a->dx1, a->wot, a->dout, M1, M1, C, C, nullptr, nullptr, a->s1, T, nullptr, nullptr, 0, a->perm1, stream));
    if (rc) return rc;
    if (a->attn_kind == VTX_ATTN_WINDOW)
      rc = TCALL(VTX_T_WATTN_BWD, M1, a->nH, a->L, F_MAPPED | (a->region ? F_MASKED : 0), stream,
                 vtx_wattn_bwd_mapped(a->qkv, a->o, a->dout, a->lse, a->rel_pos, a->pos, a->region, a->dqkv, a->attn_ws, a->attn_ws_bytes,
                                      a->inv_cells, a->inv_count, a->perm1, a->Bk1, a->L, a->nH, a->H, a->W, a->win, a->shift, dt, stream));
    else
      rc = TCALL(VTX_T_ATTN_BWD, M1, a->nH, a->L, F_MAPPED, stream,
                 vtx_attention_bwd_mapped(a->qkv, a->o, a->dout, a->lse, a->dqkv, a->perm1, a->Bk1, a->L, a->nH, C / a->nH, dt, stream));
    if (rc) return rc;
    rc = TCALL(VTX_T_GEMM, M1, C, 3 * C, F_MAPPED, stream, layer_gemm_mapped(a->dqkv, a->wqt, a->dln1, M1, M1, C, 3 * C, nullptr, nullptr, nullptr, T, nullptr, nullptr, 0, a->perm1, stream));
    if (rc) return rc;
    rc = TCALL(VTX_T_LN_BWD, M, C, 0, F_MAPPED, stream,
               vtx_layernorm_bwd_mapped(a->dln1, a->x, a->mean1, a->rstd1, a->ln1_w, a->dx1, a->dx, a->ln1_ws, a->ln_ws_bytes, M, M1, C, dt,
                                        a->perm1, T, stream));
    if (rc) return rc;
  }
  if (!mapped) {
    int rc;
    bool ln2_folded = false;
    if (mlp_fused_ok(dt, M, C, ff)) {
      if (!a->h || !a->b1) return VTX_ERR_NULL;
      if (mlp_fused_ln_ok(dt, M, C, ff)) {
        if (a->ln_ws_bytes < vtx_layernorm_bwd_workspace(M, C)) return VTX_ERR_WORKSPACE;
        rc = TCALL(VTX_T_MLP_BWD, M, C, ff, F_RESID, stream,
                   mlp_fused_bwd_ln(a->ln2, a->dy, a->w1, a->b1, a->w2, a->s2, rps, const_cast<void*>(a->h), a->dz, a->x1, a->mean2, a->rstd2,
                                    a->ln2_w, a->dx1, (float*)a->ln2_ws, vtx_layernorm_bwd_blocks(M, C), M, C, ff, (hipStream_t)stream));
        if (rc) return rc;
        ln2_folded = true;
      } else {
        rc = TCALL(VTX_T_MLP_BWD, M, C, ff, 0, stream,
                   mlp_fused_bwd(a->ln2, a->dy, a->w1, a->b1, a->w2, a->s2, rps, const_cast<void*>(a->h), a->dz, a->dln2, M, C, ff, (hipStream_t)stream));
        if (rc) return rc;
      }
    } else {
      rc = TCALL(VTX_T_GEMM, M, ff, C, F_AUXIN, stream, layer_dgrad(dt, a->dy, a->w2, a->w2t, a->dz, M, ff, C, nullptr, a->s2, rps, a->z, 2, stream));
      if (rc) return rc;
      rc = TCALL(VTX_T_GEMM, M, C, ff, 0, stream, layer_dgrad(dt, a->dz, a->w1, a->w1t, a->dln2, M, C, ff, nullptr, nullptr, 1, nullptr, 0, stream));
      if (rc) return rc;
    }
    if (!ln2_folded) {
      rc = TCALL(VTX_T_LN_BWD, M, C, 0, 0, stream,
                 vtx_layernorm_bwd(a->dln2, a->x1, a->mean2, a->rstd2, a->ln2_w, a->dy, a->dx1, nullptr, nullptr, a->ln2_ws, a->ln_ws_bytes,
                                   M, C, dt, 0, 0, 0, stream));
      if (rc) return rc;
    }
    rc = TCALL(VTX_T_GEMM, M, C, C, 0, stream, layer_dgrad(dt, a->dx1, a->wo, a->wot, a->dout, M, C, C, nullptr, a->s1, rps, nullptr, 0, stream));
    if (rc) return rc;
    if (a->attn_kind == VTX_ATTN_WINDOW)
      rc = TCALL(VTX_T_WATTN_BWD, M, a->nH, a->L, a->region ? F_MASKED : 0, stream,
                 vtx_wattn_bwd(a->qkv, a->o, a->dout, a->lse, a->rel_pos, a->pos, a->region, a->dqkv, nullptr, a->attn_ws, a->attn_ws_bytes,
                               a->inv_cells, a->inv_count, a->B, a->L, a->nH, a->H, a->W, a->win, a->shift, dt, stream));
    else if (a->attn_kind == VTX_ATTN_GLOBAL)
      rc = TCALL(VTX_T_ATTN_BWD, M, a->nH, a->L, 0, stream,
                 vtx_attention_bwd(a->qkv, a->o, a->dout, a->lse, nullptr, nullptr, nullptr, nullptr, a->dqkv, nullptr, 0, a->attn_ws,
                                   a->attn_ws_bytes, a->B, a->L, a->nH, C / a->nH, 0, 0, 0, 0, 0, dt, stream));
    else
      return VTX_ERR_SHAPE;
    if (rc) return rc;
    if (a->wqt != nullptr && dgrad_ln_ok(dt, M, C, 3 * C)) {
      if (a->ln_ws_bytes < vtx_layernorm_bwd_workspace(M, C)) return VTX_ERR_WORKSPACE;
      rc = TCALL(VTX_T_DGRAD_LN, M, C, 3 * C, 0, stream,
                 dgrad_ln_launch(a->dqkv, a->wqt, a->x, a->mean1, a->rstd1, a->ln1_w, a->dx1, a->dx, (float*)a->ln1_ws, vtx_layernorm_bwd_blocks(M, C),
                                 M, C, 3 * C, (hipStream_t)stream));
    } else {
      rc = TCALL(VTX_T_GEMM, M, C, 3 * C, 0, stream, layer_dgrad(dt, a->dqkv, a->wq, a->wqt, a->dln1, M, C, 3 * C, nullptr, nullptr, 1, nullptr, 0, stream));
      if (rc) return rc;
      rc = TCALL(VTX_T_LN_BWD, M, C, 0, 0, stream,
                 vtx_layernorm_bwd(a->dln1, a->x, a->mean1, a->rstd1, a->ln1_w, a->dx1, a->dx, nullptr, nullptr, a->ln1_ws, a->ln_ws_bytes,
                                   M, C, dt, 0, 0, 0, stream));
    }
    if (rc) return rc;
  }
  void* ws = stream;
  if (side_stream != nullptr && side_stream != stream) {
    hipEvent_t e = g_events.get();
    if (!e || hipEventRecord(e, (hipStream_t)stream) != hipSuccess ||
        hipStreamWaitEvent((hipStream_t)side_stream, e, 0) != hipSuccess)
      return VTX_ERR_LAUNCH;
    ws = side_stream;
  }
  const void* dys[4] = {a->dy, a->dz, a->dx1, a->dqkv};
  const void* xs[4] = {a->h, a->ln2, a->o, a->ln1};
  float* dWs[4] = {a->dW2, a->dW1, a->dWo, a->dWq};
  float* dbs[4] = {a->db2, a->db1, a->dbo, a->dbq};
  const int Ns[4] = {C, ff, C, 3 * C}, Ks[4] = {ff, C, C, C};
  const int64_t ldy[4] = {C, ff, C, 3 * C}, ldx[4] = {ff, C, C, C};
  const float* rs[4] = {mapped ? nullptr : a->s2, nullptr, mapped ? nullptr : a->s1, nullptr};
  const int* perms[4] = {a->perm2, a->perm2, a->perm1, a->perm1};
  const int kept[4] = {a->Bk2 * rps, a->Bk2 * rps, a->Bk1 * rps, a->Bk1 * rps};
  const float scl[4] = {a->scale_const, 1.f, a->scale_const, 1.f};
  const int ncol = a->attn_kind == VTX_ATTN_WINDOW ? 3 : 2;
  const float* cpart[4] = {(const float*)a->ln2_ws, (const float*)a->ln1_ws, (const float*)a->attn_ws, nullptr};
  float* cout0[4] = {a->dg2, a->dg1, a->drel, nullptr};
  float* cout1[4] = {a->dbe2, a->dbe1, nullptr, nullptr};
  const int ntab = (2 * a->win - 1) * (2 * a->win - 1);
  const int cnb[4] = {vtx_layernorm_bwd_blocks(M, C), vtx_layernorm_bwd_blocks(M, C),
                      ncol == 3 ? vtx_wattn_bwd_parts(mapped ? a->Bk1 : a->B, a->nH, a->H, a->W, a->win) : 0, 0};
  const int cC[4] = {C, C, ncol == 3 ? ntab * a->nH : 0, 0};
  const int cld[4] = {2 * C, 2 * C, ncol == 3 ? vtx_wattn_bwd_part_ld(a->nH) : 0, 0};
  return TCALL(VTX_T_WGRAD, mapped ? (int64_t)(kept[0] > kept[2] ? kept[0] : kept[2]) : M, C, ff, mapped ? F_MAPPED : 0, ws,
               vtx_wgrad_group_mapped(dt, 4, dys, xs, dWs, dbs, Ns, Ks, ldy, ldx, rs, mapped ? perms : nullptr, kept, scl, rps,
                                      a->scale_const, M, a->wgrad_ws, a->wgrad_ws_bytes, ncol, cpart, cout0, cout1, cnb, cC, cld,
                                      a->accumulate, ws));
}

int vtx_srlayer_fwd(const VtxSrLayerFwd* a, void* stream) {
  if (!a || !a->x || !a->y || !a->ln1 || !a->q || !a->kv || !a->o || !a->x1 || !a->ln2 || !a->h) return VTX_ERR_NULL;
  if (a->M <= 0 || a->M > 0x7fffffff || a->C <= 0 || a->ff <= 0 || a->nH <= 0 || a->B <= 0 || a->L <= 0 || a->Lk <= 0 || a->r < 1)
    return VTX_ERR_SHAPE;
  const int dt = a->dtype, M = (int)a->M, C = a->C, ff = a->ff, r = a->r;
  g_timer_base = (dt == VTX_BF16 ? F_BF16 : 0) | ((C / a->nH) << 8);
  int rc;
  if (ln_gemm_ok(dt, M, C, C)) {
    rc = TCALL(VTX_T_LN_GEMM, M, C, C, 0, stream,
               ln_gemm_launch(a->x, a->ln1_w, a->ln1_b, a->eps, a->ln1, a->mean1, a->rstd1, a->wq, nullptr, a->q, M, C, C, (hipStream_t)stream));
    if (rc) return rc;
  } else {
    rc = TCALL(VTX_T_LN_FWD, M, C, 0, 0, stream, vtx_layernorm_fwd(a->x, a->ln1_w, a->ln1_b, a->ln1, a->mean1, a->rstd1, a->M, C, a->eps, dt, 0, 0, 0, stream));
    if (rc) return rc;
    rc = TCALL(VTX_T_GEMM, M, C, C, 0, stream, vtx_gemm(0, dt, a->ln1, a->wq, a->q, M, C, C, C, C, C, nullptr, nullptr, nullptr, 1, nullptr, nullptr, 0, stream));
    if (rc) return rc;
  }
  const void* kvin = a->ln1;
  const int rows = a->B * a->Lk;
  if (r > 1) {
    if (!a->patches || !a->red || !a->wsr) return VTX_ERR_NULL;
    const int K = r * r * C;
    if (a->twins) rc = TCALL(VTX_T_GATHER, rows, K, 0, F_TWINS, stream, vtx_twins_subsample_fwd(a->ln1, a->patches, a->splitk ? a->patches_t : nullptr, a->B, a->H, a->W, C, r, dt, stream));
    else rc = TCALL(VTX_T_GATHER, rows, K, 0, 0, stream, vtx_patchify_fwd(a->ln1, a->patches, a->B, a->H, a->W, C, r, a->skip, dt, stream));
    if (rc) return rc;
    if (a->splitk) {
      if (!a->twins || !a->patches_t || !a->wsr_t || !a->red32 || !a->splitk_ws) return VTX_ERR_NULL;
      rc = TCALL(VTX_T_WGRAD_SPLITK, K, rows, C, 0, stream,
                 vtx_wgrad(dt, a->patches_t, a->wsr_t, (float*)a->red32, nullptr, K, rows, C, rows, C, nullptr, 1, 0.f, a->splitk_ws,
                           a->splitk_ws_bytes, stream));
      if (rc) return rc;
      rc = vtx_bias_cast((const float*)a->red32, a->bsr, a->red, rows, C, dt, stream);
    } else {
      rc = TCALL(VTX_T_GEMM, rows, C, K, 0, stream, vtx_gemm(0, dt, a->patches, a->wsr, a->red, rows, C, K, K, K, C, a->bsr, nullptr, nullptr, 1, nullptr, nullptr, 0, stream));
    }
    if (rc) return rc;
    kvin = a->red;
    if (a->srn_w != nullptr) {
      if (!a->kvin || !a->means || !a->rstds) return VTX_ERR_NULL;
      rc = TCALL(VTX_T_LN_FWD, rows, C, 0, 0, stream, vtx_layernorm_fwd(a->red, a->srn_w, a->srn_b, a->kvin, a->means, a->rstds, rows, C, a->eps, dt, 0, 0, 0, stream));
      if (rc) return rc;
      kvin = a->kvin;
    }
  }
  rc = TCALL(VTX_T_GEMM, rows, 2 * C, C, 0, stream, vtx_gemm(0, dt, kvin, a->wkv, a->kv, rows, 2 * C, C, C, C, 2 * C, nullptr, nullptr, nullptr, 1, nullptr, nullptr, 0, stream));
  if (rc) return rc;
  rc = TCALL(VTX_T_SRATTN_FWD, M, a->nH, a->Lk, 0, stream, vtx_srattn_fwd(a->q, a->kv, a->o, a->lse, a->B, a->L, a->Lk, a->nH, C / a->nH, dt, stream));
  if (rc) return rc;
  rc = TCALL(VTX_T_GEMM, M, C, C, F_RESID, stream, vtx_gemm(0, dt, a->o, a->wo, a->x1, M, C, C, C, C, C, a->bo, a->x, a->s1, a->rows_per_scale, nullptr, nullptr, 0, stream));
  if (rc) return rc;
  if (mlp_fused_lnf_ok(dt, M, C, ff))
    return TCALL(VTX_T_MLP_FWD, M, C, ff, F_RESID | F_AUXOUT, stream,
                 mlp_fused_fwd_ln(a->x1, a->ln2_w, a->ln2_b, a->eps, a->ln2, a->mean2, a->rstd2, a->w1, a->b1, a->w2, a->b2, a->s2, a->rows_per_scale,
                                  a->y, M, C, ff, (hipStream_t)stream));
  rc = TCALL(VTX_T_LN_FWD, M, C, 0, 0, stream, vtx_layernorm_fwd(a->x1, a->ln2_w, a->ln2_b, a->ln2, a->mean2, a->rstd2, a->M, C, a->eps, dt, 0, 0, 0, stream));
  if (rc) return rc;
  if (mlp_fused_ok(dt, M, C, ff))
    return TCALL(VTX_T_MLP_FWD, M, C, ff, F_RESID, stream,
                 mlp_fused_fwd(a->ln2, a->w1, a->b1, a->w2, a->b2, a->x1, a->s2, a->rows_per_scale, a->y, nullptr, nullptr, M, C, ff, (hipStream_t)stream));
  rc = TCALL(VTX_T_GEMM, M, ff, C, a->z ? F_AUXOUT : 0, stream, vtx_gemm(0, dt, a->ln2, a->w1, a->h, M, ff, C, C, C, ff, a->b1, nullptr, nullptr, 1, a->z, nullptr, 1, stream));
  if (rc) return rc;
  return TCALL(VTX_T_GEMM, M, C, ff, F_RESID, stream,
               vtx_gemm(0, dt, a->h, a->w2, a->y, M, C, ff, ff, ff, C, a->b2, a->x1, a->s2, a->rows_per_scale, nullptr, nullptr, 0, stream));
}

int vtx_srlayer_bwd(const VtxSrLayerBwd* a, void* stream, void* side_stream) {
  if (!a || !a->dy || !a->dx || !a->x || !a->z || !a->dz || !a->dln2 || !a->dx1 || !a->dout || !a->dq || !a->dkv || !a->dkvin || !a->dln1)
    return VTX_ERR_NULL;
  if (a->M <= 0 || a->M > 0x7fffffff || a->C <= 0 || a->ff <= 0 || a->nH <= 0 || a->r < 1) return VTX_ERR_SHAPE;
  const int dt = a->dtype, C = a->C, ff = a->ff, rps = a->rows_per_scale, r = a->r;
  const int64_t M = a->M;
  const int rows = a->B * a->Lk;
  g_timer_base = (dt == VTX_BF16 ? F_BF16 : 0) | ((C / a->nH) << 8);
  int rc;
  bool ln2_folded = false;
  if (mlp_fused_ok(dt, M, C, ff)) {
    if (!a->h || !a->b1) return VTX_ERR_NULL;
    if (mlp_fused_ln_ok(dt, M, C, ff)) {
      if (a->ln_ws_bytes < vtx_layernorm_bwd_workspace(M, C)) return VTX_ERR_WORKSPACE;
      rc = TCALL(VTX_T_MLP_BWD, M, C, ff, F_RESID, stream,
                 mlp_fused_bwd_ln(a->ln2, a->dy, a->w1, a->b1, a->w2, a->s2, rps, const_cast<void*>(a->h), a->dz, a->x1, a->mean2, a->rstd2,
                                  a->ln2_w, a->dx1, (float*)a->ln2_ws, vtx_layernorm_bwd_blocks(M, C), M, C, ff, (hipStream_t)stream));
      if (rc) return rc;
      ln2_folded = true;
    } else {
      rc = TCALL(VTX_T_MLP_BWD, M, C, ff, 0, stream,
                 mlp_fused_bwd(a->ln2, a->dy, a->w1, a->b1, a->w2, a->s2, rps, const_cast<void*>(a->h), a->dz, a->dln2, M, C, ff, (hipStream_t)stream));
      if (rc) return rc;
    }
  } else {
    rc = TCALL(VTX_T_GEMM, M, ff, C, F_AUXIN, stream, layer_dgrad(dt, a->dy, a->w2, a->w2t, a->dz, M, ff, C, nullptr, a->s2, rps, a->z, 2, stream));
    if (rc) return rc;
    rc = TCALL(VTX_T_GEMM, M, C, ff, 0, stream, layer_dgrad(dt, a->dz, a->w1, a->w1t, a->dln2, M, C, ff, nullptr, nullptr, 1, nullptr, 0, stream));
    if (rc) return rc;
  }
  if (!ln2_folded) {
    rc = TCALL(VTX_T_LN_BWD, M, C, 0, 0, stream,
               vtx_layernorm_bwd(a->dln2, a->x1, a->mean2, a->rstd2, a->ln2_w, a->dy, a->dx1, nullptr, nullptr, a->ln2_ws, a->ln_ws_bytes, M, C, dt, 0, 0, 0, stream));
// ... 80 lines not shown
```

vision-transformers-pytorch_amd/vtx/attention.py:

```python
import ctypes

import torch

from . import _lib, options
from ._lib import VtxError


L32_MAX = 160
SHORT_MAX = 224
L64_TABLE_MAX = 64


def attn_hd_supported(D):
    return isinstance(D, int) and 8 <= D <= 128 and D % 8 == 0


def attn_hd_pad(D):
    return 32 if D <= 32 else (64 if D <= 64 else (96 if D <= 96 else 128))


def wattn_supported(D, win):
    return D == 32 and win <= 7


# ... 228 lines not shown
    _dev(q, kv)
    if q.dtype != kv.dtype or q.numel() != B * Lq * hd or kv.numel() != B * Lk * 2 * hd:
        raise VtxError(f"vtx: attn_hd shape mismatch (q {tuple(q.shape)}, kv {tuple(kv.shape)}, {n_head} heads of {D})")
    t = kv.view(B * Lk, 2 * hd)
    return q.view(B * Lq, hd), t[:, :hd], t[:, hd:], hd, 2 * hd


def attn_hd_fwd(q, kv, B, Lq, Lk, n_head, D, drop=None):
    qv, kk, vv, ldq, ldkv = _attn_hd_views(q, kv, B, Lq, Lk, n_head, D)
    o = torch.empty((B * Lq, n_head * D), dtype=q.dtype, device=q.device)
    lse = torch.empty(B * n_head * Lq, dtype=torch.float32, device=q.device)
    _launch("vtx_attn_hd_fwd", (_p(qv), _p(kk), _p(vv), ldq, ldkv, _p(o), _p(lse), B, Lq, Lk, n_head, D, _dt(q)), drop,
            f"hdattn_fwd_kernel<{_tn(q)}, {attn_hd_pad(D)}>", _pair_geom(q, B, Lq, Lk, n_head, D, False), drop_fields=True)
    return o, lse


def attn_hd_bwd(q, kv, o, dout, lse, B, Lq, Lk, n_head, D, drop=None):
    qv, kk, vv, ldq, ldkv = _attn_hd_views(q, kv, B, Lq, Lk, n_head, D)
    _dev(o, dout, lse)
    _f32(lse, "lse")
    hd = n_head * D
    if o.dtype != q.dtype or dout.dtype != q.dtype or o.numel() != B * Lq * hd or dout.numel() != B * Lq * hd or \
            lse.numel() != B * n_head * Lq:
        raise VtxError("vtx: attn_hd backward operands do not match the forward's (o, dout [B*Lq, h*D] of q's dtype, lse [B*h*Lq])")
    dq = torch.empty_like(q)
    dkv = torch.empty_like(kv) if kv is not None else None
    dqv, dkk, dvv, _, _ = _attn_hd_views(dq, dkv, B, Lq, Lk, n_head, D)
    wsb = _lib.load().vtx_attn_hd_bwd_workspace(B, Lq, n_head)
    ws = torch.empty(wsb, dtype=torch.uint8, device=q.device)
    _launch("vtx_attn_hd_bwd", (_p(qv), _p(kk), _p(vv), ldq, ldkv, _p(o), _p(dout), _p(lse), _p(dqv), _p(dkk), _p(dvv), ldq, ldkv,
                                _p(ws), wsb, B, Lq, Lk, n_head, D, _dt(q)), drop,
            f"hdattn_bwd_*_kernel<{_tn(q)}, {attn_hd_pad(D)}>", _pair_geom(q, B, Lq, Lk, n_head, D, True), drop_fields=True)
    return dq if kv is None else (dq, dkv)


def _attn_hdw_args(q, kv, B, Lq, Lk, n_head, D, swin, bias, mask):
    H, W, win, shift = swin if swin is not None else (0, 0, 0, 0)
    nprob = B
    if swin is not None:
        if kv is not None or win <= 0 or H % win or W % win or Lq != win * win or Lk != Lq:
            raise VtxError(f"vtx: attn_hdw window geometry mismatch ({H} x {W} map, window {win}, {Lq} x {Lk} tokens)")
        nW = (H // win) * (W // win)
        nprob = B * nW
        qv, kk, vv, ldq, ldkv = _attn_hd_views(q, None, nprob, Lq, Lk, n_head, D)
    else:
        if mask is not None:
            raise VtxError("vtx: attn_hdw takes a mask only with a window (it is indexed by the window)")
        qv, kk, vv, ldq, ldkv = _attn_hd_views(q, kv, B, Lq, Lk, n_head, D)
    _dev(bias, mask)
    if bias is not None:
        _f32(bias, "bias")
        if bias.numel() != n_head * Lq * Lk or not bias.is_contiguous():
            raise VtxError(f"vtx: attn_hdw bias must be a contiguous [{n_head}, {Lq}, {Lk}] fp32 tensor")
    if mask is not None:
        msk = mask.view(torch.uint8) if mask.dtype == torch.bool else mask
        if msk.dtype != torch.uint8 or not msk.is_contiguous() or msk.numel() != (nprob // B) * Lq * Lk:
            raise VtxError(f"vtx: attn_hdw mask must be a contiguous [{nprob // B}, {Lq}, {Lk}] bool / uint8 tensor")
        mask = msk
    return qv, kk, vv, ldq, ldkv, nprob, (H, W, win, int(bool(shift))), mask


def attn_hdw_fwd(q, kv, B, Lq, Lk, n_head, D, swin=None, bias=None, mask=None, drop=None):
    qv, kk, vv, ldq, ldkv, nprob, (H, W, win, shift), mask = _attn_hdw_args(q, kv, B, Lq, Lk, n_head, D, swin, bias, mask)
    o = torch.empty((nprob * Lq, n_head * D), dtype=q.dtype, device=q.device)
    lse = torch.empty(nprob * n_head * Lq, dtype=torch.float32, device=q.device)
    _launch("vtx_attn_hdw_fwd", (_p(qv), _p(kk), _p(vv), ldq, ldkv, _p(o), _p(lse), _p(bias), _p(mask), B, Lq, Lk, n_head, D, H, W, win,
                                 shift, _dt(q)), drop,
            f"hdattn_fwd_kernel<{_tn(q)}, {attn_hd_pad(D)}, true>", _pair_geom(q, nprob, Lq, Lk, n_head, D, False), drop_fields=True)
    return o, lse


def attn_hdw_bwd(q, kv, o, dout, lse, B, Lq, Lk, n_head, D, swin=None, bias=None, mask=None, drop=None):
    qv, kk, vv, ldq, ldkv, nprob, (H, W, win, shift), mask = _attn_hdw_args(q, kv, B, Lq, Lk, n_head, D, swin, bias, mask)
    _dev(o, dout, lse)
    _f32(lse, "lse")
    hd = n_head * D
    if o.dtype != q.dtype or dout.dtype != q.dtype or o.numel() != nprob * Lq * hd or dout.numel() != nprob * Lq * hd or \
            lse.numel() != nprob * n_head * Lq or not o.is_contiguous() or not dout.is_contiguous():
        raise VtxError("vtx: attn_hdw backward operands do not match the forward's (o, dout [rows, h*D] of q's dtype, lse [problems*h*Lq])")
    dq = torch.empty_like(q)
    dkv = torch.empty_like(kv) if kv is not None else None
    dqv, dkk, dvv, _, _ = _attn_hd_views(dq, dkv, nprob if kv is None else B, Lq, Lk, n_head, D)
    dbias = torch.empty((n_head, Lq, Lk), dtype=torch.float32, device=q.device) if bias is not None else None
    wsb = _lib.load().vtx_attn_hdw_bwd_workspace(B, Lq, Lk, n_head, H, W, win, int(bias is not None))
    ws = torch.empty(wsb, dtype=torch.uint8, device=q.device)
    _launch("vtx_attn_hdw_bwd", (_p(qv), _p(kk), _p(vv), ldq, ldkv, _p(o), _p(dout), _p(lse), _p(bias), _p(mask), _p(dqv), _p(dkk), _p(dvv),
                                 ldq, ldkv, _p(dbias), _p(ws), wsb, B, Lq, Lk, n_head, D, H, W, win, shift, _dt(q)), drop,
            f"hdattn_bwd_*_kernel<{_tn(q)}, {attn_hd_pad(D)}, true>",
            _pair_geom(q, nprob, Lq, Lk, n_head, D, True, 14 if bias is not None else 10), drop_fields=True)
    return (dq, dbias) if kv is None else (dq, dkv, dbias)


def relpos_bias(rel_pos, pos, n_head):
    _dev(rel_pos, pos)
    _f32(rel_pos, "rel_pos")
    if pos.dtype != torch.int64:
        raise VtxError("vtx: pos must be int64 (the reference's buffer dtype)")
    L = pos.shape[0]
    bias = torch.empty((n_head, L, L), dtype=torch.float32, device=rel_pos.device)
    _lib.check(_lib.load().vtx_relpos_bias(_p(rel_pos), _p(pos), _p(bias), L, n_head, _stream()), "vtx_relpos_bias")
    return bias


def pos_csr(pos, ntab):
    flat = pos.reshape(-1).cpu()
    order = torch.argsort(flat, stable=True).to(torch.int32)
    counts = torch.bincount(flat, minlength=ntab)
    offsets = torch.zeros(ntab + 1, dtype=torch.int32)
    offsets[1:] = torch.cumsum(counts, 0).to(torch.int32)
    return order, offsets


def _packed_geom(qkv, nprob, L, n_head, D, bwd):
    rows = qkv.numel() // (3 * n_head * D)
    return nprob, L, L, D, rows, rows, n_head * D, qkv.element_size(), bwd, 10 if bwd else 4


def attention_fwd(qkv, B, L, n_head, D, swin=None, bias=None, mask=None, drop=None):
    _dev(qkv, bias, mask)
    H, W, win, shift = swin if swin is not None else (0, 0, 0, 0)
    rows = qkv.numel() // (3 * n_head * D)
    nW = (H // win) * (W // win) if swin is not None else 1
    if rows != B * nW * L:
        raise VtxError("vtx: attention rows mismatch")
    o = torch.empty(qkv.shape[:-1] + (n_head * D,), dtype=qkv.dtype, device=qkv.device)
    lse = torch.empty(B * nW * n_head * L, dtype=torch.float32, device=qkv.device)
    _launch("vtx_attention_fwd", (_p(qkv), _p(o), _p(lse), _p(bias), _p(mask), B, L, n_head, D, int(swin is not None), H, W, win,
                                  int(bool(shift)), _dt(qkv)), drop,
            lambda: generic_label(qkv.dtype, D, L, swin is not None, bias is not None, mask is not None, drop is not None, False),
            _packed_geom(qkv, B * nW * n_head, L, n_head, D, False))
    return o, lse


def attention_bwd(qkv, o, dout, lse, B, L, n_head, D, swin=None, bias=None, mask=None, csr=None, ntab=0, drop=None):
    _dev(qkv, o, dout, lse, bias, mask)
    H, W, win, shift = swin if swin is not None else (0, 0, 0, 0)
    dqkv = torch.empty_like(qkv)
    drel, ws, wsb, order, offsets = None, None, 0, None, None
    if bias is not None:
        order, offsets = csr
        _dev(order, offsets)
        drel = torch.empty((ntab, n_head), dtype=torch.float32, device=qkv.device)
    if bias is not None or (swin is None and L > SHORT_MAX):
        wsb = _lib.load().vtx_attention_bwd_workspace(B, L, n_head, int(swin is not None), H, W, max(win, 1))
        ws = torch.empty(wsb, dtype=torch.uint8, device=qkv.device)
    rows = qkv.numel() // (3 * n_head * D)
    _launch("vtx_attention_bwd", (_p(qkv), _p(o), _p(dout), _p(lse), _p(bias), _p(mask), _p(order), _p(offsets), _p(dqkv), _p(drel), ntab,
                                  _p(ws), wsb, B, L, n_head, D, int(swin is not None), H, W, win, int(bool(shift)), _dt(qkv)), drop,
            lambda: generic_label(qkv.dtype, D, L, swin is not None, bias is not None, mask is not None, drop is not None, True),
            _packed_geom(qkv, rows // L * n_head, L, n_head, D, True))
    return dqkv, drel


def wattn_fwd(qkv, rel_pos, pos, region, B, L, n_head, swin):
    _dev(qkv, rel_pos, pos, region)
    _f32(rel_pos, "rel_pos")
    if pos.dtype != torch.int64:
        raise VtxError("vtx: pos must be int64 (the reference's buffer dtype)")
    H, W, win, shift = swin
    o = torch.empty(qkv.shape[:-1] + (n_head * 32,), dtype=qkv.dtype, device=qkv.device)
    nW = (H // win) * (W // win)
    lse = torch.empty(B * nW * n_head * L, dtype=torch.float32, device=qkv.device)
    _launch("vtx_wattn_fwd", (_p(qkv), _p(o), _p(lse), _p(rel_pos), _p(pos), _p(region), B, L, n_head, H, W, win, int(bool(shift)),
                              _dt(qkv)), None, lambda: wattn_fwd_kernel_name(qkv.dtype, region is not None, B * nW),
            (B * nW * n_head, L, L, 32, B * nW * L, B * nW * L, n_head * 32, qkv.element_size(), False, 4))
    return o, lse


_POS_INVERSE = {}


def _pos_inverse(pos, ntab):
    key = (pos.data_ptr(), pos.device, tuple(pos.shape), ntab)
    hit = _POS_INVERSE.get(key)
    if hit is None or hit[0]() is None:
        import weakref
        from . import tables
        for k in [k for k, v in _POS_INVERSE.items() if v[0]() is None]:
            del _POS_INVERSE[k]
        cells, count = tables.pos_inverse(pos, ntab)
        hit = (weakref.ref(pos), cells.to(pos.device), count)
        _POS_INVERSE[key] = hit
    return hit[1], hit[2]


def wattn_bwd(qkv, o, dout, lse, rel_pos, pos, region, B, L, n_head, swin, ntab, defer=False, use_inverse=True):
    _dev(qkv, o, dout, lse, rel_pos, pos, region)
    lib = _lib.load()
    inv_cells, inv_count = _pos_inverse(pos, ntab) if use_inverse else (None, 0)
    H, W, win, shift = swin
    dqkv = torch.empty_like(qkv)
    drel = None if defer else torch.empty((ntab, n_head), dtype=torch.float32, device=qkv.device)
    wsb = lib.vtx_wattn_bwd_workspace(B, n_head, H, W, win)
    ws = torch.empty(wsb, dtype=torch.uint8, device=qkv.device)
    nW = (H // win) * (W // win)
    _launch("vtx_wattn_bwd", (_p(qkv), _p(o), _p(dout), _p(lse), _p(rel_pos), _p(pos), _p(region), _p(dqkv), _p(drel), _p(ws), wsb,
                              _p(inv_cells), inv_count, B, L, n_head, H, W, win, int(bool(shift)), _dt(qkv)), None,
            lambda: wattn_bwd_kernel_name(qkv.dtype, region is not None, use_inverse),
            (B * nW * n_head, L, L, 32, B * nW * L, B * nW * L, n_head * 32, qkv.element_size(), True, 10))
    if defer:
        return dqkv, Partials(ws, lib.vtx_wattn_bwd_parts(B, n_head, H, W, win), ntab * n_head, lib.vtx_wattn_bwd_part_ld(n_head), False)
    return dqkv, drel


from . import ops
from .ops import Partials, _dev, _dt, _f32, _p, _stream
```

vision-transformers-pytorch_amd/vtx/functional.py:

```python
import contextlib
import ctypes
import os
import struct
import threading
import warnings

import torch
from torch.autograd import Function

from . import _lib, attention, ops, options
from .ops import ACT_DGELU, ACT_DSILU, ACT_GELU, ACT_SILU, VtxError


def compute_dtype(x):
    if torch.is_autocast_enabled("cuda"):
        dt = torch.get_autocast_dtype("cuda")
        if dt == torch.bfloat16:
            return torch.bfloat16
        raise VtxError(f"vtx: autocast dtype {dt} unsupported on the MI355X path (use torch.bfloat16)")
    if x.dtype in (torch.float32, torch.bfloat16):
        return x.dtype
    raise VtxError(f"vtx: unsupported activation dtype {x.dtype}")


_tls = threading.local()


class WeightPlan:

    def __init__(self, module):
        self.params = []
        for m in module.modules():
            w = m._parameters.get("weight") if isinstance(m, (torch.nn.Linear, torch.nn.Conv2d)) else None
            if w is not None and w.dtype == torch.float32 and w.is_cuda:
                self.params.append(w)
        self.key, self.desc, self.offs, self.total, self.ntiles = None, None, None, 0, 0

    def _prepare(self):
        key = tuple((p.data_ptr(), p.device) for p in self.params)
        if key == self.key:
            return
        offs, recs, off, tile0 = [], [], 0, 0
        for p in self.params:
            rows, cols = p.shape[0], p.numel() // p.shape[0]
            tr, tc = (rows + 63) // 64, (cols + 63) // 64
            recs.append(struct.pack("<QqiiiI", p.data_ptr(), off, rows, cols, tile0, tc))
            offs.append(off)
            off += (rows * cols + 63) // 64 * 64
            tile0 += tr * tc
        assert struct.calcsize("<QqiiiI") == ops.cast_desc_bytes()
        dev = self.params[0].device
        self.desc = torch.frombuffer(bytearray(b"".join(recs)), dtype=torch.uint8).to(dev)
        self.key, self.offs, self.total, self.ntiles = key, offs, off, tile0

    def cast_all(self):
        if not self.params:
            return {}
        self._prepare()
        dev = self.params[0].device
        flat = torch.empty(self.total, dtype=torch.bfloat16, device=dev)
        flat_t = torch.empty(self.total, dtype=torch.bfloat16, device=dev)
        ops.cast_weights(self.desc, len(self.params), self.ntiles, flat, flat_t)
        out = {}
        for p, off in zip(self.params, self.offs):
            n, rows = p.numel(), p.shape[0]
            out[id(p)] = (flat[off:off + n].view(p.shape), flat_t[off:off + n].view(n // rows, rows))
        return out


@contextlib.contextmanager
def weight_scope(module, x):
    if getattr(_tls, "scope", None) is not None or not x.is_cuda or compute_dtype(x) != torch.bfloat16:
        yield
        return
    plan = module.__dict__.get("_vtx_weight_plan")
    if plan is not None:
        plan[3][0] += 1
        mods = plan[2] if plan[3][0] % 32 else list(module.modules())
    else:
        mods = list(module.modules())
    ids = [(id(m), id(m._parameters.get("weight"))) for m in mods]
    if plan is None or plan[0] != ids:
        plan = (ids, WeightPlan(module), mods, [0])
        module.__dict__["_vtx_weight_plan"] = plan
    _tls.scope = plan[1].cast_all()
    try:
        yield
    finally:
        _tls.scope = None


def wcast(p, dtype):
    if p.dtype == dtype:
        return (p.detach(), None)
    sc = getattr(_tls, "scope", None)
    if sc is not None:
        ent = sc.get(id(p))
        if ent is not None and ent[0].dtype == dtype:
            return ent
    return (p.detach().to(dtype), None)


_DGRAD_SPLITK = os.environ.get("VTX_DGRAD_SPLITK", "1") != "0"


def dgrad(dy, wp, T, **epi):
    w, wt = wp
    w2 = w.view(w.shape[0], -1)
    if (_DGRAD_SPLITK and T == torch.bfloat16 and not epi and dy.dim() == 2 and w2.shape[0] >= 16384 and w2.shape[1] % 8 == 0 and
            w2.shape[1] >= 64 and dy.shape[0] % 8 == 0 and dy.shape[0] >= 64 and
            ((dy.shape[0] + 63) // 64) * ((w2.shape[1] + 127) // 128) < 128):
        dx32, _ = ops.wgrad(dy.t().contiguous(), w2 if w2.is_contiguous() else w2.contiguous(), want_bias=False)
        return ops.bias_cast(dx32, None, T)
    if T == torch.bfloat16 and ops.glds_ok(w2.shape[1], w2.shape[0]):
        if wt is None:
            wt = w2.t().contiguous()
        return ops.gemm(dy, wt, 0, **epi)
    return ops.gemm(dy, w2, 1, **epi)


def _c(t):
    return t if t.is_contiguous() else t.contiguous()


def _img(x):
    return x if ops.is_nhwc_bf16(x) else _c(x)


_SIDE_ENABLED = os.environ.get("VTX_SIDE_WGRAD", "1") != "0"
_SIDE_FENCE_MODE = os.environ.get("VTX_SIDE_FENCE", "0")
_TWINS_SPLITK = os.environ.get("VTX_TWINS_SPLITK", "1") != "0"
_DEFER_REDUCE = os.environ.get("VTX_DEFER_REDUCE", "1") != "0"
_deferred = False


_SIDE_PROBE = os.environ.get("VTX_SIDE_PROBE", "1") != "0"
side_stream_report = {}


def _concurrent_stream(device, candidates=8, spin_us=150):
    cur = torch.cuda.current_stream(device)
    lib = _lib.load()
    seen = []
    first = None
    alone = float(spin_us)
    for rep in range(2):
        e0, e1 = torch.cuda.Event(enable_timing=True), torch.cuda.Event(enable_timing=True)
        e0.record(cur)
        _lib.check(lib.vtx_debug_spin(spin_us, cur.cuda_stream), "vtx_debug_spin")
        e1.record(cur)
        e1.synchronize()
        alone = e0.elapsed_time(e1) * 1e3
    for k in range(candidates):
        st = torch.cuda.Stream(device=device)
        first = first or st
        best = None
        for rep in range(2):
            e0, e1 = torch.cuda.Event(enable_timing=True), torch.cuda.Event(enable_timing=True)
            e0.record(cur)
            st.wait_event(e0)
            _lib.check(lib.vtx_debug_spin(spin_us, cur.cuda_stream), "vtx_debug_spin")
            _lib.check(lib.vtx_debug_spin(spin_us, st.cuda_stream), "vtx_debug_spin")
            cur.wait_stream(st)
            e1.record(cur)
            e1.synchronize()
            best = e0.elapsed_time(e1) * 1e3
        seen.append(round(best, 1))
        if best < 1.6 * alone:
            side_stream_report[str(device)] = dict(chosen=k, pair_us=seen, spin_us=spin_us, alone_us=round(alone, 1), concurrent=True)
            return st
    side_stream_report[str(device)] = dict(chosen=0, pair_us=seen, spin_us=spin_us, alone_us=round(alone, 1), concurrent=False)
    warnings.warn(f"vtx: none of {candidates} candidate streams runs concurrently with the compute stream (two {spin_us}-us spin kernels took "
                  f"{seen} us): the side-stream weight gradients will serialise", RuntimeWarning)
    return first


class _SideState:
    def __init__(self, device):
        self.stream = _concurrent_stream(device) if _SIDE_PROBE else torch.cuda.Stream(device=device)
        self.pending = False
        self.keep = []


_side_states = {}


@contextlib.contextmanager
def deferred_wgrad(enabled=True):
    global _deferred
    prev, _deferred = _deferred, bool(enabled) and _SIDE_ENABLED
    try:
        yield
    finally:
        _deferred = prev
        side_join()


def side_stream_after_current(dev):
    st = _side_states.get(dev)
    if st is None or not st.pending:
        return None
    st.stream.wait_stream(torch.cuda.current_stream(dev))
    return st.stream


def side_fence(dev, merge=False):
    st = _side_states.get(dev)
    if st is not None and st.pending and (_SIDE_FENCE_MODE == "1" or (_SIDE_FENCE_MODE == "merge" and merge)):
        torch.cuda.current_stream(dev).wait_stream(st.stream)


def side_join():
    for dev, st in _side_states.items():
        if st.pending:
            torch.cuda.current_stream(dev).wait_stream(st.stream)
            st.pending = False
            st.keep.clear()


_shared_grads = None


@contextlib.contextmanager
def shared_param_backward(enabled=True):
    global _shared_grads
    prev, _shared_grads = _shared_grads, ({} if enabled else None)
    try:
        yield
    finally:
        _shared_grads = prev


_grad_sink_providers = []


def register_grad_sink_provider(obj):
    import weakref
    _grad_sink_providers.append(weakref.ref(obj))


def grad_sink(param):
    if not _grad_sink_providers or param is None or param.grad is not None:
# ... 329 lines not shown
    bias = ops.relpos_bias(rel_pos.detach(), meta.pos, meta.n_head) if rel_pos is not None else None
    if route == "hdw":
        o, lse = ops.attn_hdw_fwd(qkv, None, B, meta.L, meta.L, meta.n_head, meta.dim_head, swin=meta.swin, bias=bias, mask=meta.mask,
                                  drop=drop)
        return o.view(qkv.shape[:-1] + (meta.n_head * meta.dim_head,)), lse, bias
    o, lse = ops.attention_fwd(qkv, B, meta.L, meta.n_head, meta.dim_head, swin=meta.swin, bias=bias, mask=meta.mask, drop=drop)
    return o, lse, bias


def _attn_backward(qkv, o, do, lse, aux, meta, route, rel_pos=None, defer=False, drop=None):
    B = qkv.shape[0]
    if route == "hd":
        return ops.attn_hd_bwd(qkv, None, o, do, lse, B, meta.L, meta.L, meta.n_head, meta.dim_head, drop=drop), None
    if route == "hdw":
        dqkv, dbias = ops.attn_hdw_bwd(qkv, None, o, do, lse, B, meta.L, meta.L, meta.n_head, meta.dim_head, swin=meta.swin, bias=aux,
                                       mask=meta.mask, drop=drop)
        return dqkv, (ops.table_bias_bwd(dbias, meta.csr, meta.ntab, meta.n_head) if aux is not None else None)
    if route == "window":
        return ops.wattn_bwd(qkv, o, do, lse, rel_pos.detach(), meta.pos, meta.region, B, meta.L, meta.n_head,
                             meta.swin, meta.ntab, defer=defer)
    return ops.attention_bwd(qkv, o, do, lse, B, meta.L, meta.n_head, meta.dim_head, swin=meta.swin, bias=aux,
                             mask=meta.mask, csr=meta.csr, ntab=meta.ntab, drop=drop)


class AttentionCoreFn(Function):

    @staticmethod
    def forward(ctx, qkv, rel_pos, meta, drop=None):
        qkv = _c(qkv)
        ctx.route = _route(rel_pos, meta, drop)
        o, lse, aux = _attn_forward(qkv, rel_pos, meta, ctx.route, drop)
        ctx.save_for_backward(qkv, o, lse, aux, rel_pos)
        ctx.meta, ctx.drop = meta, drop
        return o

    @staticmethod
    def backward(ctx, do):
        side_fence(do.device)
        qkv, o, lse, aux, rel_pos = ctx.saved_tensors
        dqkv, drel = _attn_backward(qkv, o, _c(do), lse, aux, ctx.meta, ctx.route, rel_pos, drop=ctx.drop)
        return dqkv, drel, None, None


class HaloMeta:

    def __init__(self, n_head, dim_head, window, halo, pos, csr, ntab):
        self.n_head, self.dim_head, self.window, self.halo = n_head, dim_head, window, halo
        self.pos, self.csr, self.ntab = pos, csr, ntab


class HaloAttentionFn(Function):

    @staticmethod
    def forward(ctx, qkv, rel_pos, meta, drop=None):
        qkv = _c(qkv)
        B, H, W, C3 = qkv.shape
        hd = C3 // 3
        w, a, nH = meta.window, meta.halo, meta.n_head
        nW, Lq, Lk = (H // w) * (W // w), w * w, (w + 2 * a) ** 2
        q = ops.window_gather(qkv, B, H, W, 0, hd, w, 0)
        kv = ops.window_gather(qkv, B, H, W, hd, 2 * hd, w, a)
        bias = ops.table_bias(rel_pos.detach(), meta.pos, nH)
        ctx.route = attention.route_pair(meta.dim_head, True)
        if ctx.route == "hdw":
            o, lse = ops.attn_hdw_fwd(q.view(B * nW * Lq, hd), kv.view(B * nW * Lk, 2 * hd), B * nW, Lq, Lk, nH, meta.dim_head, bias=bias,
                                      drop=drop)
        else:
            o, lse = ops.xattn_fwd(q.view(B * nW * Lq, hd), kv.view(B * nW * Lk, 2 * hd), B * nW, Lq, Lk, nH, bias, drop=drop)
        out = torch.empty((B, H, W, hd), dtype=qkv.dtype, device=qkv.device)
        ops.window_scatter(o, out, B, H, W, 0, hd, w, 0)
        ctx.save_for_backward(q, kv, o, lse, bias)
        ctx.meta, ctx.geom, ctx.drop = meta, (B, H, W, hd, nW, Lq, Lk), drop
        return out

    @staticmethod
    def backward(ctx, dout):
        side_fence(dout.device)
        q, kv, o, lse, bias = ctx.saved_tensors
        meta = ctx.meta
        B, H, W, hd, nW, Lq, Lk = ctx.geom
        w, a, nH = meta.window, meta.halo, meta.n_head
        do = ops.window_gather(_c(dout), B, H, W, 0, hd, w, 0)
        if ctx.route == "hdw":
            dq, dkv, dbias = ops.attn_hdw_bwd(q.view(B * nW * Lq, hd), kv.view(B * nW * Lk, 2 * hd), o, do.view(B * nW * Lq, hd), lse,
                                              B * nW, Lq, Lk, nH, meta.dim_head, bias=bias, drop=ctx.drop)
        else:
            dq, dkv, dbias = ops.xattn_bwd(q.view(B * nW * Lq, hd), kv.view(B * nW * Lk, 2 * hd), o, do.view(B * nW * Lq, hd), lse,
                                           B * nW, Lq, Lk, nH, bias, drop=ctx.drop)
        dqkv = torch.empty((B, H, W, 3 * hd), dtype=q.dtype, device=q.device)
        ops.window_scatter(dq, dqkv, B, H, W, 0, hd, w, 0)
        ops.window_scatter(dkv, dqkv, B, H, W, hd, 2 * hd, w, a)
        drel = ops.table_bias_bwd(dbias, meta.csr, meta.ntab, nH)
        return dqkv, drel, None, None


class TransformerLayerFn(Function):

    @staticmethod
    def forward(ctx, x, ln1_w, ln1_b, qkv_w, qkv_b, rel_pos, proj_w, proj_b, ln2_w, ln2_b, fc1_w, fc1_b, fc2_w,
                fc2_b, s1, s2, dp_c, meta):
        x = _c(x)
        T = x.dtype
        B, C = x.shape[0], x.shape[-1]
        rps = (x.numel() // C) // B
        ctx.pids = tuple(map(id, (ln1_w, ln1_b, qkv_w, qkv_b, proj_w, proj_b, ln2_w, ln2_b, fc1_w, fc1_b, fc2_w, fc2_b)))
        ctx.meta, ctx.rps, ctx.dp_c = meta, rps, float(dp_c)
        kind = _layer_kind(x, rel_pos, meta)
        if kind and (qkv_w.shape[0] != 3 * C or proj_w.shape[1] != C or meta.n_head * meta.dim_head != C or qkv_b is None or
                     proj_b is None or fc1_b is None or fc2_b is None):
            kind = 0
        pl = None
        if kind:
            pl = _layer_plan(kind, meta, B, x.numel() // C, C, fc1_w.shape[0], T, any(ctx.needs_input_grad),
                             s1 is not None or s2 is not None, rps, float(dp_c))
            if not pl.ok:
                kind = 0
        ctx.kind = kind
        if kind:
            return TransformerLayerFn._forward_one_call(ctx, kind, pl, x, ln1_w, ln1_b, qkv_w, qkv_b, rel_pos, proj_w, proj_b,
                                                        ln2_w, ln2_b, fc1_w, fc1_b, fc2_w, fc2_b, s1, s2, meta)
        ln1, mean1, rstd1 = ops.layernorm_fwd(x, ln1_w.detach(), ln1_b.detach(), meta.eps)
        wq, wo, w1, w2 = ctx.wp = (wcast(qkv_w, T), wcast(proj_w, T), wcast(fc1_w, T), wcast(fc2_w, T))
        qkv = ops.gemm(ln1, wq[0], 0, bias=qkv_b.detach())
        ctx.route = _route(rel_pos, meta)
        o, lse, bias = _attn_forward(qkv, rel_pos, meta, ctx.route)
        x1 = ops.gemm(o, wo[0], 0, bias=proj_b.detach(), resid=x, rowscale=s1, rows_per_scale=rps)
        ln2, mean2, rstd2 = ops.layernorm_fwd(x1, ln2_w.detach(), ln2_b.detach(), meta.eps)
        h, z = _act_gemm(ctx, ln2, w1[0], fc1_b.detach(), ACT_SILU)
        y = ops.gemm(h, w2[0], 0, bias=fc2_b.detach(), resid=x1, rowscale=s2, rows_per_scale=rps)
        ctx.save_for_backward(x, ln1_w, qkv_w, proj_w, ln2_w, fc1_w, fc2_w, mean1, rstd1, ln1, qkv, o, lse, x1,
                              mean2, rstd2, ln2, z, h, bias, s1, s2, rel_pos)
        return y

    @staticmethod
    def _forward_one_call(ctx, kind, pl, x, ln1_w, ln1_b, qkv_w, qkv_b, rel_pos, proj_w, proj_b, ln2_w, ln2_b, fc1_w, fc1_b,
                          fc2_w, fc2_b, s1, s2, meta):
        T = x.dtype
        B, C = x.shape[0], x.shape[-1]
        M, ff = x.numel() // C, fc1_w.shape[0]
        _check_layer_inputs(x, T, ln1_w, ln1_b, qkv_b, proj_b, ln2_w, ln2_b, fc1_b, fc2_b, s1, s2)
        want_z = any(ctx.needs_input_grad)
        wq, wo, w1, w2 = ctx.wp = (wcast(qkv_w, T), wcast(proj_w, T), wcast(fc1_w, T), wcast(fc2_w, T))
        buf = torch.empty(pl.f_bytes, dtype=torch.uint8, device=x.device)
        y = torch.empty_like(x)
        base, fo = buf.data_ptr(), pl.f_off
        d = _copy_desc(pl.fwd)
        d.rows_per_scale = ctx.rps
        d.x, d.y = x.data_ptr(), y.data_ptr()
        d.ln1_w, d.ln1_b, d.ln2_w, d.ln2_b = ln1_w.data_ptr(), ln1_b.data_ptr(), ln2_w.data_ptr(), ln2_b.data_ptr()
        d.wq, d.wo, d.w1, d.w2 = wq[0].data_ptr(), wo[0].data_ptr(), w1[0].data_ptr(), w2[0].data_ptr()
        d.bq, d.bo, d.b1, d.b2 = qkv_b.data_ptr(), proj_b.data_ptr(), fc1_b.data_ptr(), fc2_b.data_ptr()
        if kind == _lib.ATTN_WINDOW:
            d.rel_pos, d.pos, d.region = rel_pos.data_ptr(), meta.pos.data_ptr(), _dp(meta.region)
        d.s1, d.s2 = _dp(s1), _dp(s2)
        ctx.perms = _layer_perms(kind, T, C, ff, s1, s2, meta.dim_head, meta.L, M // B)
        if ctx.perms is not None and any(w[1] is None for w in (wq, wo, w1, w2)):
            ctx.perms = None
        if ctx.perms is not None:
            (p1, d.Bk1), (p2, d.Bk2) = ctx.perms
            d.perm1, d.perm2 = p1.data_ptr(), p2.data_ptr()
        d.ln1, d.qkv, d.o, d.x1, d.ln2, d.h = (base + fo["ln1"], base + fo["qkv"], base + fo["o"], base + fo["x1"],
                                               base + fo["ln2"], base + fo["h"])
        d.z = base + fo["z"] if want_z else None
        d.mean1, d.rstd1, d.mean2, d.rstd2, d.lse = (base + fo["mean1"], base + fo["rstd1"], base + fo["mean2"],
                                                     base + fo["rstd2"], base + fo["lse"])
        _lib.check(_lib.load().vtx_layer_fwd(ctypes.byref(d), ops._stream()), "vtx_layer_fwd")
        ctx.save_for_backward(x, buf, ln1_w, qkv_w, proj_w, ln2_w, fc1_w, fc2_w, s1, s2, rel_pos, fc1_b)
        ctx.plan = pl
        return y

    @staticmethod
    def _backward_one_call(ctx, dy):
        x, buf, ln1_w, qkv_w, proj_w, ln2_w, fc1_w, fc2_w, s1, s2, rel_pos, fc1_b = ctx.saved_tensors
        pl, m, kind = ctx.plan, ctx.meta, ctx.kind
        if pl.f_off["z"] is None:
            raise VtxError("vtx: this layer's forward ran without a graph (no pre-activation was kept)")
        dy = _c(dy)
        dev = x.device
        C = x.shape[-1]
        ff = fc1_w.shape[0]
        wq, wo, w1, w2 = ctx.wp
        scratch = torch.empty(pl.b_bytes, dtype=torch.uint8, device=dev)
        dx = torch.empty_like(x)
        f32 = dict(dtype=torch.float32, device=dev)
        shared = _shared_grads if rel_pos is None else None
        acc = None
        if shared is not None:
            first = [shared.get(pid) for pid in ctx.pids]
            if all(a is not None for a in first) and pl.slices >= 2:
                acc = first
        outs = None
        if acc is None:
            sinks = [grad_sink(p) for p in (qkv_w, proj_w, fc1_w, fc2_w)] if _grad_sink_providers else (None,) * 4
            dWq, dWo, dW1, dW2 = [sk if sk is not None else torch.empty(p.shape, **f32)
                                  for sk, p in zip(sinks, (qkv_w, proj_w, fc1_w, fc2_w))]
            nrel = pl.ntab * m.n_head
            small = torch.empty(9 * C + ff + nrel, **f32).split((C, C, 3 * C, C, C, C, ff, C) + ((nrel,) if nrel else ()))
            dg1, dbe1, dbq, dbo, dg2, dbe2, db1, db2 = small[:8]
            drel = small[8].view(pl.ntab, m.n_head) if nrel else None
            outs = (dg1, dbe1, dWq, dbq, dWo, dbo, dg2, dbe2, dW1, db1, dW2, db2)
            gp = [t.data_ptr() for t in outs]
        else:
            gp, drel = acc, None
        base, fo, sb, bo = buf.data_ptr(), pl.f_off, scratch.data_ptr(), pl.b_off
        d = _copy_desc(pl.bwd)
        d.rows_per_scale, d.scale_const, d.accumulate = ctx.rps, ctx.dp_c, int(acc is not None)
        d.dy, d.x, d.dx = dy.data_ptr(), x.data_ptr(), dx.data_ptr()
        (d.ln1, d.qkv, d.o, d.x1, d.ln2, d.z, d.h) = (base + fo["ln1"], base + fo["qkv"], base + fo["o"], base + fo["x1"],
                                                      base + fo["ln2"], base + fo["z"], base + fo["h"])
        d.mean1, d.rstd1, d.mean2, d.rstd2, d.lse = (base + fo["mean1"], base + fo["rstd1"], base + fo["mean2"],
                                                     base + fo["rstd2"], base + fo["lse"])
        d.ln1_w, d.ln2_w = ln1_w.data_ptr(), ln2_w.data_ptr()
        d.b1 = fc1_b.data_ptr()
        d.wq, d.wo, d.w1, d.w2 = (wq[0].data_ptr(), wo[0].data_ptr(), w1[0].data_ptr(), w2[0].data_ptr())
        d.wqt, d.wot, d.w1t, d.w2t = _dp(wq[1]), _dp(wo[1]), _dp(w1[1]), _dp(w2[1])
        if kind == _lib.ATTN_WINDOW:
            inv_cells, inv_count = ops._pos_inverse(m.pos, m.ntab)
            d.rel_pos, d.pos, d.region = rel_pos.data_ptr(), m.pos.data_ptr(), _dp(m.region)
            d.inv_cells, d.inv_count = inv_cells.data_ptr(), inv_count
            d.drel = drel.data_ptr()
        d.s1, d.s2 = _dp(s1), _dp(s2)
        if ctx.perms is not None:
            (p1, d.Bk1), (p2, d.Bk2) = ctx.perms
            d.perm1, d.perm2 = p1.data_ptr(), p2.data_ptr()
        d.dz, d.dln2, d.dx1, d.dout, d.dqkv, d.dln1 = (sb + bo["dz"], sb + bo["dln2"], sb + bo["dx1"], sb + bo["dout"],
                                                       sb + bo["dqkv"], sb + bo["dln1"])
        d.ln1_ws, d.ln2_ws, d.wgrad_ws = sb + bo["ln1_ws"], sb + bo["ln2_ws"], sb + bo["wgrad_ws"]
        d.attn_ws = sb + bo["attn_ws"] if bo["attn_ws"] is not None else None
        (d.dg1, d.dbe1, d.dWq, d.dbq, d.dWo, d.dbo, d.dg2, d.dbe2, d.dW1, d.db1, d.dW2, d.db2) = gp
        side = None
        if _deferred and not ops.timing():
            st = _side_states.get(dev)
            if st is None:
                st = _side_states[dev] = _SideState(dev)
            side = st.stream.cuda_stream
            st.keep.append((scratch, buf, dy, x, s1, s2, ctx.wp, ctx.perms))
            st.pending = True
        _lib.check(_lib.load().vtx_layer_bwd(ctypes.byref(d), ops._stream(), side), "vtx_layer_bwd")
        if acc is not None:
            return (dx,) + (None,) * 17
        if shared is not None and not any(pid in shared for pid in ctx.pids):
            for pid, a in zip(ctx.pids, gp):
                shared[pid] = a
        return (dx, dg1, dbe1, dWq, dbq, drel, dWo, dbo, dg2, dbe2, dW1, db1, dW2, db2, None, None, None, None)

    @staticmethod
    def backward(ctx, dy):
        if ctx.kind:
            return TransformerLayerFn._backward_one_call(ctx, dy)
        (x, ln1_w, qkv_w, proj_w, ln2_w, fc1_w, fc2_w, mean1, rstd1, ln1, qkv, o, lse, x1, mean2, rstd2, ln2, z, h,
         bias, s1, s2, rel_pos) = ctx.saved_tensors
        m, rps, dp_c = ctx.meta, ctx.rps, ctx.dp_c
        wq, wo, w1, w2 = ctx.wp
        T = x.dtype
        dy = _c(dy)
        B = x.shape[0]
        dz = dgrad(dy, w2, T, act=ACT_DSILU, aux_in=z, rowscale=s2, rows_per_scale=rps)
        dln2 = dgrad(dz, w1, T)
        if _DEFER_REDUCE:
            dx1, part2 = ops.layernorm_bwd(dln2, x1, mean2, rstd2, ln2_w.detach(), dres=dy, defer=True)
        else:
            dx1, dg2, dbe2 = ops.layernorm_bwd(dln2, x1, mean2, rstd2, ln2_w.detach(), dres=dy)
        do = dgrad(dx1, wo, T, rowscale=s1, rows_per_scale=rps)
        dqkv, drel = _attn_backward(qkv, o, do, lse, bias, m, ctx.route, rel_pos, defer=_DEFER_REDUCE)
        dln1 = dgrad(dqkv, wq, T)
        if _DEFER_REDUCE:
            dx, part1 = ops.layernorm_bwd(dln1, x, mean1, rstd1, ln1_w.detach(), dres=dx1, defer=True)
            parts = [part2, part1] + ([drel] if isinstance(drel, ops.Partials) else [])
        else:
            dx, dg1, dbe1 = ops.layernorm_bwd(dln1, x, mean1, rstd1, ln1_w.detach(), dres=dx1)
            parts = None
        jobs = [(dy, h, True, s2), (dz, ln2, True, None), (dx1, o, True, s1), (dqkv, ln1, True, None)]
        shared = _shared_grads if (parts is not None and len(parts) == 2 and rel_pos is None) else None
        if shared is not None:
            first = [shared.get(pid) for pid in ctx.pids]
            if all(a is not None for a in first) and ops.wgrad_group_ok(jobs, rps, dp_c) and ops.wgrad_group_slices(jobs) >= 2:
                g1, b1, wq, bq, wo, bo, g2, b2, w1, bb1, w2, bb2 = first
                layer_wgrads(jobs, rps, dp_c, colparts=parts, accumulate=((w2, w1, wo, wq), (bb2, bb1, bo, bq), [(g2, b2), (g1, b1)]))
                return (dx,) + (None,) * 17
        res = layer_wgrads(jobs, rps, dp_c, params=(fc2_w, fc1_w, proj_w, qkv_w), colparts=parts)
        if parts is not None:
            res, red = res
            (dg2, dbe2), (dg1, dbe1) = red[0], red[1]
            if isinstance(drel, ops.Partials):
                drel = red[2][0].view(m.ntab, m.n_head)
        (dW2, db2), (dW1, db1), (dWo, dbo), (dWq, dbq) = res
        if shared is not None and not any(pid in shared for pid in ctx.pids):
            for pid, t in zip(ctx.pids, (dg1, dbe1, dWq, dbq, dWo, dbo, dg2, dbe2, dW1, db1, dW2, db2)):
                shared[pid] = t.data_ptr()
        return (dx, dg1, dbe1, dWq, dbq, drel, dWo, dbo, dg2, dbe2, dW1, db1, dW2, db2, None, None, None, None)


class PatchMergeFn(Function):

    @staticmethod
    def forward(ctx, x, ln_w, ln_b, w, eps):
        x = _c(x)
        H, W = x.shape[1], x.shape[2]
        ln, mean, rstd = ops.layernorm_fwd(x, ln_w.detach(), ln_b.detach(), eps, merge_hw=(H, W))
        ctx.wp = wcast(w, x.dtype)
        y = ops.gemm(ln, ctx.wp[0], 0)
        ctx.save_for_backward(x, ln_w, w, ln, mean, rstd)
        return y

    @staticmethod
    def backward(ctx, dy):
        x, ln_w, w, ln, mean, rstd = ctx.saved_tensors
        dy = _c(dy)
        dW, _ = ops.wgrad(dy, ln, want_bias=False)
        dln = dgrad(dy, ctx.wp, x.dtype)
        side_fence(dy.device, merge=True)
        dx, dg, db = ops.layernorm_bwd(dln, x, mean, rstd, ln_w.detach(), merge_hw=(x.shape[1], x.shape[2]))
        return dx, dg, db, dW, None


class SwinPatchEmbedFn(Function):

    @staticmethod
    def forward(ctx, x_nchw, w, b, ln_w, ln_b, patch, eps, dtype):
        patches = ops.patch_gather(_img(x_nchw), patch, 0, dtype)
        t = ops.gemm(patches, wcast(w, dtype)[0], 0, bias=b.detach())
        y, mean, rstd = ops.layernorm_fwd(t, ln_w.detach(), ln_b.detach(), eps)
        ctx.save_for_backward(patches, t, mean, rstd, ln_w)
        return y

    @staticmethod
    def backward(ctx, dy):
        side_fence(dy.device)
        patches, t, mean, rstd, ln_w = ctx.saved_tensors
        dt, dg, db = ops.layernorm_bwd(_c(dy), t, mean, rstd, ln_w.detach())
        dW, dbias = ops.wgrad(dt, patches)
        return None, dW, dbias, dg, db, None, None, None


class VitPatchEmbedFn(Function):

    @staticmethod
    def forward(ctx, x_nchw, w, b, dtype):
        C, Cin, p, _ = w.shape
        patches = ops.patch_gather(_img(x_nchw), p, 1, dtype)
        B, gh, gw, K = patches.shape
        y = ops.gemm(patches.view(B, gh * gw, K), wcast(w, dtype)[0].view(C, K), 0, bias=b.detach())
        ctx.save_for_backward(patches)
        ctx.wshape = w.shape
        return y

    @staticmethod
    def backward(ctx, dy):
        side_fence(dy.device)
        (patches,) = ctx.saved_tensors
        dW, db = ops.wgrad(_c(dy), patches)
        return None, dW.view(ctx.wshape), db, None


class VitAssembleFn(Function):

    @staticmethod
    def forward(ctx, patches, cls_token, pos_embed):
        L, C = pos_embed.shape[-2], pos_embed.shape[-1]
        out = ops.vit_assemble_fwd(_c(patches), _c(cls_token.detach().reshape(C)),
                                   _c(pos_embed.detach().reshape(L, C)))
        ctx.shapes = (cls_token.shape, pos_embed.shape)
        return out

    @staticmethod
    def backward(ctx, dx):
        side_fence(dx.device)
        dpatches, dcls, dpos = ops.vit_assemble_bwd(_c(dx))
        return dpatches, dcls.view(ctx.shapes[0]), dpos.view(ctx.shapes[1])


class TokenMeanFn(Function):
# ... 483 lines not shown
```

Measured before the change: 8917 images/sec.

## Precompute per-head window-attention bias tables once per step in the weight-cast kernel

Adds a dense per-head 64x68 float bias table that the weight-cast kernel builds once per step from rel_pos and pos, with -inf padding for masked columns. The window-attention forward and backward kernels then copy this table into shared memory with vector loads, replacing the per-block gather through pos and rel_pos. The backward kernels also move the bias build after the first prefetch request so the build overlaps global loads. The cost is extra memory traffic for the tables and more plumbing through descriptors, the cast kernel and the Python scope.

```diff
diff --git a/include/vtx.h b/include/vtx.h
--- a/include/vtx.h
+++ b/include/vtx.h
@@ -157,6 +157,7 @@
                   const int64_t* pos, const uint8_t* region, void* dqkv, float* drel_pos, void* workspace,
                   size_t ws_bytes, const int* inv_cells, int inv_count, int B, int L, int nH, int H, int W, int win,
                   int shift, int dtype, void* stream);
+#define VTX_WATTN_TABLE_FLOATS 4352
 
 #define VTX_ATTN_WINDOW 1
 #define VTX_ATTN_GLOBAL 2
@@ -176,6 +177,7 @@
   float *mean1, *rstd1, *mean2, *rstd2, *lse;
   const int *perm1, *perm2;
   int Bk1, Bk2;
+  const float* bias_tab;
 } VtxLayerFwd;
 int vtx_layer_fwd(const VtxLayerFwd* a, void* stream);
 typedef struct VtxLayerBwd {
@@ -198,6 +200,7 @@
   const int *perm1, *perm2;
   int Bk1, Bk2;
   const float* b1;
+  const float* bias_tab;
 } VtxLayerBwd;
 int vtx_layer_bwd(const VtxLayerBwd* a, void* stream, void* side_stream);
 int vtx_layer_desc_bytes(int which);
diff --git a/vision-transformers-pytorch_amd/csrc/attention_win.hip b/vision-transformers-pytorch_amd/csrc/attention_win.hip
--- a/vision-transformers-pytorch_amd/csrc/attention_win.hip
+++ b/vision-transformers-pytorch_amd/csrc/attention_win.hip
@@ -19,6 +19,7 @@
   int L, nH, hd, nW, H, W, win, shift, nWx;
   float scale;
   const int* perm;
+  const float* tab;
 };
 
 struct WaTok {
@@ -96,10 +97,28 @@
 }
 
 __device__ __forceinline__ void wa_build_bias(float* bias_s, float* relh, const float* __restrict__ rel_pos,
-                                              const int64_t* __restrict__ pos, int L, int nH, int h, int ntab,
-                                              int qrows = 64) {
+                                              const int64_t* __restrict__ pos, const float* __restrict__ tab, int L, int nH,
+                                              int h, int ntab, int qrows = 64) {
   constexpr int PER = 64 * 64 / (64 * WA_WAVES);
   if (WA_ABLATE & 16) return;
+  if (tab != nullptr) {
+    constexpr int NV = (64 * WA_BSTR / 4 + 64 * WA_WAVES - 1) / (64 * WA_WAVES);
+    const f32x4* __restrict__ src = reinterpret_cast<const f32x4*>(tab + (int64_t)h * 64 * WA_BSTR);
+    f32x4* dst = reinterpret_cast<f32x4*>(bias_s);
+    const int nvec = qrows * (WA_BSTR / 4);
+    f32x4 v[NV];
+#pragma unroll
+    for (int i = 0; i < NV; ++i) {
+      const int idx = threadIdx.x + i * 64 * WA_WAVES;
+      if (idx < nvec) v[i] = src[idx];
+    }
+#pragma unroll
+    for (int i = 0; i < NV; ++i) {
+      const int idx = threadIdx.x + i * 64 * WA_WAVES;
+      if (idx < nvec) dst[idx] = v[i];
+    }
+    return;
+  }
   int pidx[PER];
 #pragma unroll
   for (int i = 0; i < PER; ++i) {
@@ -156,7 +175,7 @@
   wa_block_map(nblk, g.nH, xcd_major, blk, h);
   const int lane = threadIdx.x & 63, c_ = lane & 15, g_ = lane >> 4;
   const int64_t ld = 3 * (int64_t)g.hd;
-  wa_build_bias(bias_s, reinterpret_cast<float*>(wa_smem + WaSmem<T>::kBias), rel_pos, pos, g.L, g.nH, h,
+  wa_build_bias(bias_s, reinterpret_cast<float*>(wa_smem + WaSmem<T>::kBias), rel_pos, pos, g.tab, g.L, g.nH, h,
                 (2 * g.win - 1) * (2 * g.win - 1));
   __syncthreads();
   WaTok tk;
@@ -303,7 +322,7 @@
   wa_block_map(nblk, g.nH, xcd_major, blk, h);
   const int lane = threadIdx.x & 63, c_ = lane & 15, g_ = lane >> 4;
   const int64_t ld = 3 * (int64_t)g.hd;
-  wa_build_bias(bias_s, reinterpret_cast<float*>(wa_smem + WaSmem<T>::kBias), rel_pos, pos, g.L, g.nH, h,
+  wa_build_bias(bias_s, reinterpret_cast<float*>(wa_smem + WaSmem<T>::kBias), rel_pos, pos, g.tab, g.L, g.nH, h,
                 (2 * g.win - 1) * (2 * g.win - 1));
   __syncthreads();
   for (int i = lane; i < WA_NBIN; i += 64) bins[i] = 0.f;
@@ -560,9 +579,6 @@
   wa_block_map(nblk, g.nH, xcd_major, blk, h);
   const int64_t ld = 3 * (int64_t)g.hd;
   const int ntab = (2 * g.win - 1) * (2 * g.win - 1);
-  wa_build_bias(bias_s, reinterpret_cast<float*>(base), rel_pos, pos, g.L, g.nH, h, ntab, WA4_BROWS);
-  __syncthreads();
-
   const int tok = 16 * w + c_;
   const bool val = tok < g.L;
   const int tcl = val ? tok : 0;
@@ -595,6 +611,8 @@
     nl = lse[((int64_t)bn * g.nH + h) * g.L + tcl];
   };
   if (blk < nbn) request(blk);
+  wa_build_bias(bias_s, reinterpret_cast<float*>(base), rel_pos, pos, g.tab, g.L, g.nH, h, ntab, WA4_BROWS);
+  __syncthreads();
 
   for (int bn = blk; bn < nbn; bn += nblk) {
     const Vec8<T> qf = nq, kf = nk, vf = nv, dof = ndo;
@@ -753,8 +771,6 @@
   int blk, h;
   wa_block_map(nblk, g.nH, xcd_major, blk, h);
   const int64_t ld = 3 * (int64_t)g.hd;
-  wa_build_bias(bias_s, reinterpret_cast<float*>(base), rel_pos, pos, g.L, g.nH, h, (2 * g.win - 1) * (2 * g.win - 1), WA4_BROWS);
-  __syncthreads();
   const bool w7 = g.L == 49;
   const bool row48 = w7 && (fast & 1);
   auto tok_pack = [&](int t4) {
@@ -789,6 +805,8 @@
     rs[u].reg = 0;
     if (blk + u * nblk < nbn) request(blk + u * nblk, (w + u) & 3, rs[u]);
   }
+  wa_build_bias(bias_s, reinterpret_cast<float*>(base), rel_pos, pos, g.tab, g.L, g.nH, h, (2 * g.win - 1) * (2 * g.win - 1), WA4_BROWS);
+  __syncthreads();
   for (int bn = blk, it = 0; bn < nbn;) {
 #pragma unroll
   for (int u = 0; u < WF4_PF; ++u, bn += nblk, ++it) {
@@ -926,8 +944,11 @@
   g.nWx = W / win; g.nW = (H / win) * (W / win); g.shift = shift ? win / 2 : 0;
   g.scale = 1.0f / sqrtf((float)WA_D);
   g.perm = nullptr;
+  g.tab = nullptr;
   return VTX_OK;
 }
+
+static_assert(64 * WA_BSTR == VTX_WATTN_TABLE_FLOATS, "include/vtx.h states the table size");
 
 static int wattn_blocks(int nbn, int nH, int cap) {
   int per_head = cap / nH;
@@ -1071,56 +1092,32 @@
   return VTX_ERR_DTYPE;
 }
 
-extern "C" {
-
-int vtx_wattn_fwd(const void* qkv, void* o, float* lse, const float* rel_pos, const int64_t* pos,
-                  const uint8_t* region, int B, int L, int nH, int H, int W, int win, int shift, int dtype,
-                  void* stream) {
-  if (!qkv || !o || !lse || !rel_pos || !pos) return VTX_ERR_NULL;
+static int wattn_fwd_entry(const void* qkv, void* o, float* lse, const float* rel_pos, const int64_t* pos, const uint8_t* region,
+                           const int* perm, int B, int L, int nH, int H, int W, int win, int shift, int dtype, void* stream) {
+  if (!qkv || !o || !lse || !rel_pos) return VTX_ERR_NULL;
   WinGeom g;
   int rc = win_geom(g, L, nH, H, W, win, shift);
   if (rc) return rc;
+  g.perm = perm;
+  g.tab = pos ? nullptr : rel_pos;
   const int nbn = B * g.nW;
   if (nbn <= 0) return VTX_OK;
   hipStream_t st = (hipStream_t)stream;
   return wattn_fwd_routed(dtype, qkv, o, lse, rel_pos, pos, region, nbn, g, st);
 }
-
-int vtx_wattn_fwd_mapped(const void* qkv, void* o, float* lse, const float* rel_pos, const int64_t* pos,
-                         const uint8_t* region, const int* perm, int Bk, int L, int nH, int H, int W, int win, int shift,
-                         int dtype, void* stream) {
-  if (!qkv || !o || !lse || !rel_pos || !pos || !perm) return VTX_ERR_NULL;
+static int wattn_bwd_entry(const void* qkv, const void* o, const void* dout, const float* lse, const float* rel_pos, const int64_t* pos,
+                           const uint8_t* region, void* dqkv, float* drel_pos, void* workspace, size_t ws_bytes, const int* inv_cells,
+                           int inv_count, const int* perm, int B, int L, int nH, int H, int W, int win, int shift, int dtype,
+                           void* stream) {
+  if (!qkv || !o || !dout || !lse || !rel_pos || !dqkv || !workspace) return VTX_ERR_NULL;
+  if (!pos && !inv_cells) return VTX_ERR_NULL;
   WinGeom g;
   int rc = win_geom(g, L, nH, H, W, win, shift);
   if (rc) return rc;
   g.perm = perm;
-  const int nbn = Bk * g.nW;
-  if (nbn <= 0) return VTX_OK;
-  hipStream_t st = (hipStream_t)stream;
-  return wattn_fwd_routed(dtype, qkv, o, lse, rel_pos, pos, region, nbn, g, st);
-}
-
-int vtx_wattn_bwd_parts(int B, int nH, int H, int W, int win) {
-  if (win <= 0 || H % win || W % win) return 0;
-  return wattn_bwd_rows(B * (H / win) * (W / win), nH);
-}
-int vtx_wattn_bwd_part_ld(int nH) { return WA_NBIN * nH; }
-
-size_t vtx_wattn_bwd_workspace(int B, int nH, int H, int W, int win) {
-  const int nbn = B * (H / win) * (W / win);
-  return (size_t)wattn_bwd_rows(nbn, nH) * nH * WA_NBIN * sizeof(float);
-}
-
-int vtx_wattn_bwd(const void* qkv, const void* o, const void* dout, const float* lse, const float* rel_pos,
-                  const int64_t* pos, const uint8_t* region, void* dqkv, float* drel_pos, void* workspace,
-                  size_t ws_bytes, const int* inv_cells, int inv_count, int B, int L, int nH, int H, int W, int win,
-                  int shift, int dtype, void* stream) {
-  if (!qkv || !o || !dout || !lse || !rel_pos || !pos || !dqkv || !workspace) return VTX_ERR_NULL;
-  WinGeom g;
-  int rc = win_geom(g, L, nH, H, W, win, shift);
-  if (rc) return rc;
+  g.tab = pos ? nullptr : rel_pos;
   const int nbn = B * g.nW;
-  if (nbn <= 0) return VTX_OK;
+  if (nbn <= 0) return perm ? VTX_ERR_SHAPE : VTX_OK;
   if (ws_bytes < vtx_wattn_bwd_workspace(B, nH, H, W, win)) return VTX_ERR_WORKSPACE;
   if (inv_cells != nullptr && (inv_count <= 0 || inv_count > L * L)) return VTX_ERR_SHAPE;
   hipStream_t st = (hipStream_t)stream;
@@ -1134,22 +1131,47 @@
   return vtx_check_launch();
 }
 
+extern "C" {
+
+int vtx_wattn_fwd(const void* qkv, void* o, float* lse, const float* rel_pos, const int64_t* pos,
+                  const uint8_t* region, int B, int L, int nH, int H, int W, int win, int shift, int dtype,
+                  void* stream) {
+  return wattn_fwd_entry(qkv, o, lse, rel_pos, pos, region, nullptr, B, L, nH, H, W, win, shift, dtype, stream);
+}
+
+int vtx_wattn_fwd_mapped(const void* qkv, void* o, float* lse, const float* rel_pos, const int64_t* pos,
+                         const uint8_t* region, const int* perm, int Bk, int L, int nH, int H, int W, int win, int shift,
+                         int dtype, void* stream) {
+  if (!perm) return VTX_ERR_NULL;
+  return wattn_fwd_entry(qkv, o, lse, rel_pos, pos, region, perm, Bk, L, nH, H, W, win, shift, dtype, stream);
+}
+
+int vtx_wattn_bwd_parts(int B, int nH, int H, int W, int win) {
+  if (win <= 0 || H % win || W % win) return 0;
+  return wattn_bwd_rows(B * (H / win) * (W / win), nH);
+}
+int vtx_wattn_bwd_part_ld(int nH) { return WA_NBIN * nH; }
+
+size_t vtx_wattn_bwd_workspace(int B, int nH, int H, int W, int win) {
+  const int nbn = B * (H / win) * (W / win);
+  return (size_t)wattn_bwd_rows(nbn, nH) * nH * WA_NBIN * sizeof(float);
+}
+
+int vtx_wattn_bwd(const void* qkv, const void* o, const void* dout, const float* lse, const float* rel_pos,
+                  const int64_t* pos, const uint8_t* region, void* dqkv, float* drel_pos, void* workspace,
+                  size_t ws_bytes, const int* inv_cells, int inv_count, int B, int L, int nH, int H, int W, int win,
+                  int shift, int dtype, void* stream) {
+  return wattn_bwd_entry(qkv, o, dout, lse, rel_pos, pos, region, dqkv, drel_pos, workspace, ws_bytes, inv_cells, inv_count, nullptr,
+                         B, L, nH, H, W, win, shift, dtype, stream);
+}
+
 int vtx_wattn_bwd_mapped(const void* qkv, const void* o, const void* dout, const float* lse, const float* rel_pos,
                          const int64_t* pos, const uint8_t* region, void* dqkv, void* workspace, size_t ws_bytes,
                          const int* inv_cells, int inv_count, const int* perm, int Bk, int L, int nH, int H, int W, int win,
                          int shift, int dtype, void* stream) {
-  if (!qkv || !o || !dout || !lse || !rel_pos || !pos || !dqkv || !workspace || !perm) return VTX_ERR_NULL;
-  WinGeom g;
-  int rc = win_geom(g, L, nH, H, W, win, shift);
-  if (rc) return rc;
-  g.perm = perm;
-  const int nbn = Bk * g.nW;
-  if (nbn <= 0) return VTX_ERR_SHAPE;
-  if (ws_bytes < vtx_wattn_bwd_workspace(Bk, nH, H, W, win)) return VTX_ERR_WORKSPACE;
-  if (inv_cells != nullptr && (inv_count <= 0 || inv_count > L * L)) return VTX_ERR_SHAPE;
-  hipStream_t st = (hipStream_t)stream;
-  float* part = (float*)workspace;
-  return wattn_bwd_routed(dtype, qkv, o, dout, lse, rel_pos, pos, region, dqkv, part, inv_cells, inv_count, nbn, g, st);
+  if (!perm) return VTX_ERR_NULL;
+  return wattn_bwd_entry(qkv, o, dout, lse, rel_pos, pos, region, dqkv, nullptr, workspace, ws_bytes, inv_cells, inv_count, perm,
+                         Bk, L, nH, H, W, win, shift, dtype, stream);
 }
 
 int vtx_wattn_route(int dtype, int bwd, int masked, int problems_per_head, int inverse_map, VtxRoute* out) {
diff --git a/vision-transformers-pytorch_amd/csrc/cast.hip b/vision-transformers-pytorch_amd/csrc/cast.hip
--- a/vision-transformers-pytorch_amd/csrc/cast.hip
+++ b/vision-transformers-pytorch_amd/csrc/cast.hip
@@ -6,10 +6,32 @@
   int rows, cols;
   int tile0;
   int tiles_c;
+  const int64_t* pos;
 };
 
+#define CAST_TSTR (VTX_WATTN_TABLE_FLOATS / 64)
+
+__device__ __forceinline__ void cast_bias_table(const CastDesc& d, int h, float* relh, float* __restrict__ tab) {
+  const int L = -d.rows, nH = d.cols, ntab = d.tiles_c;
+  if ((int)threadIdx.x < ntab) relh[threadIdx.x] = d.src[threadIdx.x * nH + h];
+  __syncthreads();
+  float* dst = tab + d.off + (int64_t)h * VTX_WATTN_TABLE_FLOATS;
+  for (int idx = threadIdx.x; idx < VTX_WATTN_TABLE_FLOATS; idx += 256) {
+    const int q = idx / CAST_TSTR, k = idx - q * CAST_TSTR;
+    float v = 0.f;
+    if (k >= L) {
+      if (k < 64) v = -INFINITY;
+    } else if (q < L) {
+      const int p = (int)d.pos[q * L + k];
+      if (p >= 0 && p < ntab) v = relh[p];
+    }
+    dst[idx] = v;
+  }
+}
+
 __global__ __launch_bounds__(256) void cast_weights_kernel(const CastDesc* __restrict__ desc, int nmat,
-                                                          bf16* __restrict__ dst, bf16* __restrict__ dst_t) {
+                                                          bf16* __restrict__ dst, bf16* __restrict__ dst_t,
+                                                          float* __restrict__ tab) {
   __shared__ float tile[64][65];
   const int t = blockIdx.x;
   int lo = 0, hi = nmat - 1;
@@ -19,6 +41,10 @@
   }
   const CastDesc d = desc[lo];
   const int lt = t - d.tile0;
+  if (d.rows < 0) {
+    if (lt < d.cols) cast_bias_table(d, lt, &tile[0][0], tab);
+    return;
+  }
   const int r0 = (lt / d.tiles_c) * 64, c0 = (lt % d.tiles_c) * 64;
   const int tx = threadIdx.x & 63, ty = threadIdx.x >> 6;
   bf16* out = dst + d.off;
@@ -49,7 +75,7 @@
   if (!desc || !dst || !dst_t) return VTX_ERR_NULL;
   if (nmat <= 0 || ntiles <= 0) return VTX_OK;
   hipLaunchKernelGGL(cast_weights_kernel, dim3(ntiles), dim3(256), 0, (hipStream_t)stream, (const CastDesc*)desc, nmat,
-                     (bf16*)dst, (bf16*)dst_t);
+                     (bf16*)dst, (bf16*)dst_t, (float*)dst);
   return vtx_check_launch();
 }
 
diff --git a/vision-transformers-pytorch_amd/csrc/layer.hip b/vision-transformers-pytorch_amd/csrc/layer.hip
--- a/vision-transformers-pytorch_amd/csrc/layer.hip
+++ b/vision-transformers-pytorch_amd/csrc/layer.hip
@@ -117,7 +117,7 @@
     if (rc) return rc;
     if (a->attn_kind == VTX_ATTN_WINDOW)
       rc = TCALL(VTX_T_WATTN_FWD, M1, a->nH, a->L, F_MAPPED | (a->region ? F_MASKED : 0), stream,
-                 vtx_wattn_fwd_mapped(a->qkv, a->o, a->lse, a->rel_pos, a->pos, a->region, a->perm1, a->Bk1, a->L, a->nH, a->H, a->W,
+                 vtx_wattn_fwd_mapped(a->qkv, a->o, a->lse, a->bias_tab ? a->bias_tab : a->rel_pos, a->bias_tab ? nullptr : a->pos, a->region, a->perm1, a->Bk1, a->L, a->nH, a->H, a->W,
                                       a->win, a->shift, dt, stream));
     else
       rc = TCALL(VTX_T_ATTN_FWD, M1, a->nH, a->L, F_MAPPED, stream,
@@ -144,7 +144,7 @@
   }
   if (a->attn_kind == VTX_ATTN_WINDOW)
     rc = TCALL(VTX_T_WATTN_FWD, M, a->nH, a->L, a->region ? F_MASKED : 0, stream,
-               vtx_wattn_fwd(a->qkv, a->o, a->lse, a->rel_pos, a->pos, a->region, a->B, a->L, a->nH, a->H, a->W, a->win, a->shift, dt, stream));
+               vtx_wattn_fwd(a->qkv, a->o, a->lse, a->bias_tab ? a->bias_tab : a->rel_pos, a->bias_tab ? nullptr : a->pos, a->region, a->B, a->L, a->nH, a->H, a->W, a->win, a->shift, dt, stream));
   else if (a->attn_kind == VTX_ATTN_GLOBAL)
     rc = TCALL(VTX_T_ATTN_FWD, M, a->nH, a->L, 0, stream,
                vtx_attention_fwd(a->qkv, a->o, a->lse, nullptr, nullptr, a->B, a->L, a->nH, C / a->nH, 0, 0, 0, 0, 0, dt, stream));
@@ -175,6 +175,7 @@
   const int dt = a->dtype, C = a->C, ff = a->ff, rps = a->rows_per_scale;
   const int64_t M = a->M;
   const bool mapped = a->perm1 != nullptr || a->perm2 != nullptr;
+  const float* tab = a->inv_cells ? a->bias_tab : nullptr;
   g_timer_base = (dt == VTX_BF16 ? F_BF16 : 0) | ((C / a->nH) << 8);
   if (mapped) {
     const int T = rps;
@@ -195,7 +196,7 @@
     if (rc) return rc;
     if (a->attn_kind == VTX_ATTN_WINDOW)
       rc = TCALL(VTX_T_WATTN_BWD, M1, a->nH, a->L, F_MAPPED | (a->region ? F_MASKED : 0), stream,
-                 vtx_wattn_bwd_mapped(a->qkv, a->o, a->dout, a->lse, a->rel_pos, a->pos, a->region, a->dqkv, a->attn_ws, a->attn_ws_bytes,
+                 vtx_wattn_bwd_mapped(a->qkv, a->o, a->dout, a->lse, tab ? tab : a->rel_pos, tab ? nullptr : a->pos, a->region, a->dqkv, a->attn_ws, a->attn_ws_bytes,
                                       a->inv_cells, a->inv_count, a->perm1, a->Bk1, a->L, a->nH, a->H, a->W, a->win, a->shift, dt, stream));
     else
       rc = TCALL(VTX_T_ATTN_BWD, M1, a->nH, a->L, F_MAPPED, stream,
@@ -241,7 +242,7 @@
     if (rc) return rc;
     if (a->attn_kind == VTX_ATTN_WINDOW)
       rc = TCALL(VTX_T_WATTN_BWD, M, a->nH, a->L, a->region ? F_MASKED : 0, stream,
-                 vtx_wattn_bwd(a->qkv, a->o, a->dout, a->lse, a->rel_pos, a->pos, a->region, a->dqkv, nullptr, a->attn_ws, a->attn_ws_bytes,
+                 vtx_wattn_bwd(a->qkv, a->o, a->dout, a->lse, tab ? tab : a->rel_pos, tab ? nullptr : a->pos, a->region, a->dqkv, nullptr, a->attn_ws, a->attn_ws_bytes,
                                a->inv_cells, a->inv_count, a->B, a->L, a->nH, a->H, a->W, a->win, a->shift, dt, stream));
     else if (a->attn_kind == VTX_ATTN_GLOBAL)
       rc = TCALL(VTX_T_ATTN_BWD, M, a->nH, a->L, 0, stream,
diff --git a/vision-transformers-pytorch_amd/vtx/attention.py b/vision-transformers-pytorch_amd/vtx/attention.py
--- a/vision-transformers-pytorch_amd/vtx/attention.py
+++ b/vision-transformers-pytorch_amd/vtx/attention.py
@@ -404,8 +404,18 @@
     return dqkv, drel
 
 
-def wattn_fwd(qkv, rel_pos, pos, region, B, L, n_head, swin):
-    _dev(qkv, rel_pos, pos, region)
+def _bias_operands(rel_pos, pos, table, n_head):
+    if table is None:
+        return _p(rel_pos), _p(pos)
+    _dev(table)
+    _f32(table, "bias tables")
+    if table.numel() != n_head * _lib.WATTN_TABLE_FLOATS or not table.is_contiguous():
+        raise VtxError(f"vtx: bias tables must be {n_head} x {_lib.WATTN_TABLE_FLOATS} contiguous floats")
+    return _p(table), None
+
+
+def wattn_fwd(qkv, rel_pos, pos, region, B, L, n_head, swin, table=None, perm=None):
+    _dev(qkv, rel_pos, pos, region, perm)
     _f32(rel_pos, "rel_pos")
     if pos.dtype != torch.int64:
         raise VtxError("vtx: pos must be int64 (the reference's buffer dtype)")
@@ -413,8 +423,11 @@
     o = torch.empty(qkv.shape[:-1] + (n_head * 32,), dtype=qkv.dtype, device=qkv.device)
     nW = (H // win) * (W // win)
     lse = torch.empty(B * nW * n_head * L, dtype=torch.float32, device=qkv.device)
-    _launch("vtx_wattn_fwd", (_p(qkv), _p(o), _p(lse), _p(rel_pos), _p(pos), _p(region), B, L, n_head, H, W, win, int(bool(shift)),
-                              _dt(qkv)), None, lambda: wattn_fwd_kernel_name(qkv.dtype, region is not None, B * nW),
+    rp, ps = _bias_operands(rel_pos, pos, table, n_head)
+    head = (_p(qkv), _p(o), _p(lse), rp, ps, _p(region))
+    tail = (L, n_head, H, W, win, int(bool(shift)), _dt(qkv))
+    _launch(*(("vtx_wattn_fwd", head + (B,) + tail) if perm is None else ("vtx_wattn_fwd_mapped", head + (_p(perm), B) + tail)), None,
+            lambda: wattn_fwd_kernel_name(qkv.dtype, region is not None, B * nW),
             (B * nW * n_head, L, L, 32, B * nW * L, B * nW * L, n_head * 32, qkv.element_size(), False, 4))
     return o, lse
 
@@ -436,8 +449,12 @@
     return hit[1], hit[2]
 
 
-def wattn_bwd(qkv, o, dout, lse, rel_pos, pos, region, B, L, n_head, swin, ntab, defer=False, use_inverse=True):
-    _dev(qkv, o, dout, lse, rel_pos, pos, region)
+def wattn_bwd(qkv, o, dout, lse, rel_pos, pos, region, B, L, n_head, swin, ntab, defer=False, use_inverse=True, table=None, perm=None):
+    _dev(qkv, o, dout, lse, rel_pos, pos, region, perm)
+    if perm is not None and not defer:
+        raise VtxError("vtx: a mapped window-attention backward leaves its rel_pos-gradient partials to the caller (defer=True)")
+    if table is not None and not use_inverse:
+        raise VtxError("vtx: the scatter path of the rel_pos gradient reads pos; bias tables need the inverse map")
     lib = _lib.load()
     inv_cells, inv_count = _pos_inverse(pos, ntab) if use_inverse else (None, 0)
     H, W, win, shift = swin
@@ -446,8 +463,11 @@
     wsb = lib.vtx_wattn_bwd_workspace(B, n_head, H, W, win)
     ws = torch.empty(wsb, dtype=torch.uint8, device=qkv.device)
     nW = (H // win) * (W // win)
-    _launch("vtx_wattn_bwd", (_p(qkv), _p(o), _p(dout), _p(lse), _p(rel_pos), _p(pos), _p(region), _p(dqkv), _p(drel), _p(ws), wsb,
-                              _p(inv_cells), inv_count, B, L, n_head, H, W, win, int(bool(shift)), _dt(qkv)), None,
+    rp, ps = _bias_operands(rel_pos, pos, table, n_head)
+    head = (_p(qkv), _p(o), _p(dout), _p(lse), rp, ps, _p(region), _p(dqkv))
+    tail = (L, n_head, H, W, win, int(bool(shift)), _dt(qkv))
+    _launch(*(("vtx_wattn_bwd", head + (_p(drel), _p(ws), wsb, _p(inv_cells), inv_count, B) + tail) if perm is None else
+              ("vtx_wattn_bwd_mapped", head + (_p(ws), wsb, _p(inv_cells), inv_count, _p(perm), B) + tail)), None,
             lambda: wattn_bwd_kernel_name(qkv.dtype, region is not None, use_inverse),
             (B * nW * n_head, L, L, 32, B * nW * L, B * nW * L, n_head * 32, qkv.element_size(), True, 10))
     if defer:
diff --git a/vision-transformers-pytorch_amd/vtx/functional.py b/vision-transformers-pytorch_amd/vtx/functional.py
--- a/vision-transformers-pytorch_amd/vtx/functional.py
+++ b/vision-transformers-pytorch_amd/vtx/functional.py
@@ -30,41 +30,58 @@
 
     def __init__(self, module):
         self.params = []
+        self.tables = []
         for m in module.modules():
             w = m._parameters.get("weight") if isinstance(m, (torch.nn.Linear, torch.nn.Conv2d)) else None
             if w is not None and w.dtype == torch.float32 and w.is_cuda:
                 self.params.append(w)
+            rp, pos = m._modules.get("rel_pos"), m._buffers.get("pos")
+            if isinstance(rp, torch.nn.Embedding) and pos is not None and _bias_table_ok(rp.weight, pos):
+                self.tables.append((rp.weight, pos))
         self.key, self.desc, self.offs, self.total, self.ntiles = None, None, None, 0, 0
+        self.tab_offs, self.tab_floats = [], 0
 
     def _prepare(self):
-        key = tuple((p.data_ptr(), p.device) for p in self.params)
+        key = tuple((p.data_ptr(), p.device) for p in self.params) + tuple((r.data_ptr(), q.data_ptr()) for r, q in self.tables)
         if key == self.key:
             return
         offs, recs, off, tile0 = [], [], 0, 0
         for p in self.params:
             rows, cols = p.shape[0], p.numel() // p.shape[0]
             tr, tc = (rows + 63) // 64, (cols + 63) // 64
-            recs.append(struct.pack("<QqiiiI", p.data_ptr(), off, rows, cols, tile0, tc))
+            recs.append(struct.pack("<QqiiiIQ", p.data_ptr(), off, rows, cols, tile0, tc, 0))
             offs.append(off)
             off += (rows * cols + 63) // 64 * 64
             tile0 += tr * tc
-        assert struct.calcsize("<QqiiiI") == ops.cast_desc_bytes()
-        dev = self.params[0].device
+        tab_offs, toff = [], 0
+        for rel, pos in self.tables:
+            ntab, nH = rel.shape
+            recs.append(struct.pack("<QqiiiIQ", rel.data_ptr(), off // 2 + toff, -pos.shape[0], nH, tile0, ntab, pos.data_ptr()))
+            tab_offs.append(toff)
+            toff += nH * _lib.WATTN_TABLE_FLOATS
+            tile0 += nH
+        assert struct.calcsize("<QqiiiIQ") == ops.cast_desc_bytes()
+        dev = (self.params[0] if self.params else self.tables[0][0]).device
         self.desc = torch.frombuffer(bytearray(b"".join(recs)), dtype=torch.uint8).to(dev)
         self.key, self.offs, self.total, self.ntiles = key, offs, off, tile0
+        self.tab_offs, self.tab_floats = tab_offs, toff
 
     def cast_all(self):
-        if not self.params:
+        if not self.params and not self.tables:
             return {}
         self._prepare()
-        dev = self.params[0].device
-        flat = torch.empty(self.total, dtype=torch.bfloat16, device=dev)
-        flat_t = torch.empty(self.total, dtype=torch.bfloat16, device=dev)
-        ops.cast_weights(self.desc, len(self.params), self.ntiles, flat, flat_t)
+        dev = (self.params[0] if self.params else self.tables[0][0]).device
+        flat = torch.empty(self.total + 2 * self.tab_floats, dtype=torch.bfloat16, device=dev)
+        flat_t = torch.empty(max(self.total, 64), dtype=torch.bfloat16, device=dev)
+        ops.cast_weights(self.desc, len(self.params) + len(self.tables), self.ntiles, flat, flat_t)
         out = {}
         for p, off in zip(self.params, self.offs):
             n, rows = p.numel(), p.shape[0]
             out[id(p)] = (flat[off:off + n].view(p.shape), flat_t[off:off + n].view(n // rows, rows))
+        if self.tables:
+            tabs = flat[self.total:].view(torch.float32)
+            for (rel, pos), off in zip(self.tables, self.tab_offs):
+                out[("bias_tab", id(rel))] = (tabs[off:off + rel.shape[1] * _lib.WATTN_TABLE_FLOATS], pos.data_ptr())
         return out
 
 
@@ -88,6 +105,18 @@
         yield
     finally:
         _tls.scope = None
+
+
+def _bias_table_ok(rel, pos):
+    return (rel.dtype == torch.float32 and rel.is_cuda and rel.dim() == 2 and pos.dtype == torch.int64 and
+            pos.is_cuda and pos.dim() == 2 and pos.shape[0] == pos.shape[1] <= 64 and rel.shape[0] <= 172 and pos.is_contiguous() and
+            rel.is_contiguous())
+
+
+def bias_tables(rel_pos, pos):
+    sc = getattr(_tls, "scope", None)
+    ent = sc.get(("bias_tab", id(rel_pos))) if sc is not None and rel_pos is not None else None
+    return ent[0] if ent is not None and ent[1] == pos.data_ptr() else None
 
 
 def wcast(p, dtype):
@@ -723,6 +752,8 @@
         d.bq, d.bo, d.b1, d.b2 = qkv_b.data_ptr(), proj_b.data_ptr(), fc1_b.data_ptr(), fc2_b.data_ptr()
         if kind == _lib.ATTN_WINDOW:
             d.rel_pos, d.pos, d.region = rel_pos.data_ptr(), meta.pos.data_ptr(), _dp(meta.region)
+            ctx.bias_tab = bias_tables(rel_pos, meta.pos)
+            d.bias_tab = _dp(ctx.bias_tab)
         d.s1, d.s2 = _dp(s1), _dp(s2)
         ctx.perms = _layer_perms(kind, T, C, ff, s1, s2, meta.dim_head, meta.L, M // B)
         if ctx.perms is not None and any(w[1] is None for w in (wq, wo, w1, w2)):
@@ -789,6 +820,7 @@
             inv_cells, inv_count = ops._pos_inverse(m.pos, m.ntab)
             d.rel_pos, d.pos, d.region = rel_pos.data_ptr(), m.pos.data_ptr(), _dp(m.region)
             d.inv_cells, d.inv_count = inv_cells.data_ptr(), inv_count
+            d.bias_tab = _dp(ctx.bias_tab)
             d.drel = drel.data_ptr()
         d.s1, d.s2 = _dp(s1), _dp(s2)
         if ctx.perms is not None:
```

Result: no change. 8936 images/sec, median of 2 (+0.2%).
